# nihalsid/single-view-3d-reconstruction

Hardware: AMD Instinct MI355X
Metric: query-points/sec fwd+bwd (128^3 grid, 50k pts) (higher is better)
Workload: dtype f32

## Files before the change

### include/svr_hip.h

```cpp
#ifndef SVR_HIP_H
#define SVR_HIP_H

#include <stdint.h>

#ifdef __cplusplus
extern "C" {
#endif

#define SVR_OK 0
#define SVR_E_BADARG (-1)
#define SVR_E_BADSHAPE (-2)
#define SVR_E_ALIGN (-3)
#define SVR_E_UNSUPPORTED (-4)
#define SVR_E_IO (-5)
#define SVR_E_NOTFOUND (-6)

#define SVR_MAX_LEVELS 6

int svr_version(void);
const char *svr_last_error(void);

typedef struct svr_pull_plan {
  const uint32_t *keys;
  const void *recs;
// ... 22 lines not shown
  int32_t flags;
} svr_gather_desc;

#define SVR_GATHER_WIDE_OFFSETS 1
#define SVR_GATHER_DETERMINISTIC 2

int64_t svr_sizeof_level(void);
int64_t svr_sizeof_gather_desc(void);

int svr_points_voxel_order(const float *points, int32_t *order, int32_t B, int32_t N, int32_t D, int32_t H,
                           int32_t W, int32_t align_corners, void *workspace, void *stream);
int64_t svr_points_morton_order_workspace(int32_t B, int32_t N);
int svr_points_morton_order(const float *points, int32_t *order, float *sorted_points ,
                            int32_t B, int32_t N, void *workspace, void *stream);

int64_t svr_gather_pull_plan_workspace(int32_t B, int32_t N);
int64_t svr_gather_pull_plan_workspace_cells(int32_t B, int32_t D, int32_t H, int32_t W);
int svr_gather_pull_plan(const float *points, int32_t B, int32_t N, int32_t D, int32_t H, int32_t W, int32_t C,
                         int32_t col, int32_t row_stride, int32_t align_corners, float displacement,
                         uint32_t *keys, void *recs, int32_t *heads, int32_t *items , int32_t *stats ,
                         void *workspace, void *stream);

int svr_gather_item_order(const float *points, int32_t B, int32_t N, int32_t D, int32_t H, int32_t W,
                          int32_t align_corners, float displacement, int32_t with_j ,
                          int32_t *items, void *workspace, void *stream);
int svr_gather_item_order_xblock(const float *points, int32_t B, int32_t N, int32_t D, int32_t H, int32_t W,
                                 int32_t align_corners, float displacement, int32_t block, int32_t *items,
                                 void *workspace, void *stream);
int svr_gather_project_bwd(const float *points, const float *dh, int64_t lddh, int32_t B, int32_t N, int32_t D, int32_t H,
                           int32_t W, int32_t align_corners, float displacement, const int32_t *items, float *dP,
                           void *stream);

int64_t svr_gather_project_plan_workspace(int32_t B, int32_t N);
int64_t svr_gather_project_slots(int32_t B, int32_t N, int32_t D, int32_t H, int32_t W);
int svr_gather_project_plan(const float *points, int32_t B, int32_t N, int32_t D, int32_t H, int32_t W, int32_t align_corners,
                            float displacement, int32_t *items, uint32_t *keys, int32_t *sidx, int32_t *first_slot,
                            void *workspace, void *stream);
int svr_gather_project_bwd2(const float *points, const float *dh, int64_t lddh, int32_t B, int32_t N, int32_t D, int32_t H,
                            int32_t W, int32_t align_corners, float displacement, const int32_t *items, const int32_t *sidx,
                            const int32_t *first_slot, float *partials, float *dP, void *stream);

int svr_gather_trilinear_fwd(const svr_gather_desc *d, const float *points ,
                             float *features, void *stream);
int32_t svr_gather_fc0_supported(const svr_gather_desc *d);
int64_t svr_gather_fc0_workspace(const svr_gather_desc *d, int32_t n_out);
int svr_gather_fc0_fwd(const svr_gather_desc *d, const float *points, const float *W, int64_t ldw, const float *bias, float *Y,
                       int64_t ldy, int32_t n_out, float *features, int64_t ldf, const int32_t *keep_cols, uint32_t keep_levels,
                       int32_t epilogue, void *workspace, void *stream);
int svr_gather_fc0_prepare(const svr_gather_desc *d, const float *W, int64_t ldw, int32_t n_out, float *features, int64_t ldf,
                           const int32_t *keep_cols, uint32_t keep_levels, void *workspace, void *stream);
int svr_gather_fc0_run(const svr_gather_desc *d, const float *points, const float *bias, float *Y, int64_t ldy, int32_t n_out,
                       float *features, int64_t ldf, const int32_t *keep_cols, uint32_t keep_levels, int32_t epilogue,
                       void *workspace, void *stream);
int svr_gather_fc0_bf16_prepare(const svr_gather_desc *d, const float *W, int64_t ldw, int32_t n_out, void *workspace,
                                void *stream);
int svr_gather_fc0_bf16_run(const svr_gather_desc *d, const float *points, const float *bias, uint16_t *Y, int64_t ldy,
                            int32_t n_out, int32_t epilogue, void *workspace, void *stream);
int svr_gather_trilinear_bwd(const svr_gather_desc *d, const float *points, const float *gfeatures,
                             float *gpoints, void *stream);
int svr_gather_corner_indices(const svr_gather_desc *d, int32_t level, const float *points,
                              int32_t *out, void *stream);

int svr_cast_f32_to_bf16(const float *in, uint16_t *out, int64_t n, void *stream);
int svr_gather_trilinear_fwd_bf16(const svr_gather_desc *d, const float *points, uint16_t *features, void *stream);
int svr_linear_fwd_bf16(const uint16_t *X, int64_t ldx, const uint16_t *W, int64_t ldw, const float *bias, uint16_t *Y,
                        int64_t ldy, int64_t M, int64_t N, int64_t K, int epilogue, void *stream);
int svr_fc_out_fwd_bf16(const uint16_t *H, int64_t ldh, const float *w, const float *b, float *logits,
                        const int32_t *row_map, int64_t M, int64_t K, void *stream);

#define SVR_EPI_NONE 0
#define SVR_EPI_BIAS 1
#define SVR_EPI_BIAS_RELU 2
#define SVR_EPI_MASK 3

int svr_linear_fwd(const float *X, int64_t ldx, const float *W, int64_t ldw, const float *bias,
                   float *Y, int64_t ldy, int64_t M, int64_t N, int64_t K, int epilogue,
                   const float *mask, int64_t ldmask, void *stream);
int svr_linear_bwd_data(const float *dY, int64_t lddy, const float *W, int64_t ldw, float *dX,
                        int64_t lddx, int64_t M, int64_t N, int64_t K, int epilogue,
                        const float *mask, int64_t ldmask, void *stream);
int64_t svr_linear_bwd_weight_workspace(int64_t M, int64_t N, int64_t K);
int svr_linear_bwd_weight(const float *dY, int64_t lddy, const float *X, int64_t ldx, float *dW,
                          int64_t lddw, float *db, int64_t M, int64_t N, int64_t K,
                          void *workspace, void *stream);

int64_t svr_linear_fwd_bf16x6_workspace(int64_t N, int64_t K);
int svr_linear_fwd_bf16x6(const float *X, int64_t ldx, const float *W, int64_t ldw, const float *bias,
                          float *Y, int64_t ldy, int64_t M, int64_t N, int64_t K, int epilogue,
                          void *workspace, void *stream);
int64_t svr_linear_fwd_f16x3_workspace(int64_t N, int64_t K);
int svr_linear_fwd_f16x3(const float *X, int64_t ldx, const float *W, int64_t ldw, const float *bias,
                          float *Y, int64_t ldy, int64_t M, int64_t N, int64_t K, int epilogue,
                          void *workspace, void *stream);

int64_t svr_linear_bwd_data_bf16x3_workspace(int64_t N, int64_t K);
int svr_linear_bwd_data_bf16x3(const float *dY, int64_t lddy, const float *W, int64_t ldw, float *dX,
                               int64_t lddx, int64_t M, int64_t N, int64_t K, int epilogue,
                               const float *mask, int64_t ldmask, void *workspace, void *stream);
int64_t svr_linear_bwd_weight_bf16x3_workspace(int64_t M, int64_t N, int64_t K);
int svr_linear_bwd_weight_bf16x3(const float *dY, int64_t lddy, const float *X, int64_t ldx, float *dW,
                                 int64_t lddw, float *db, int64_t M, int64_t N, int64_t K,
                                 void *workspace, void *stream);

int svr_amax_f32(const float *X, int64_t ld, int64_t M, int64_t N, uint32_t *amax, void *stream);
int64_t svr_linear_bwd_data_f16x3_workspace(int64_t N, int64_t K);
int svr_linear_bwd_data_f16x3(const float *dY, int64_t lddy, const float *W, int64_t ldw, float *dX,
                              int64_t lddx, int64_t M, int64_t N, int64_t K, int epilogue,
                              const float *mask, int64_t ldmask, const uint32_t *amax_dy, uint32_t *amax_dx,
                              void *workspace, void *stream);
int64_t svr_linear_bwd_weight_f16x3_workspace(int64_t M, int64_t N, int64_t K);
int svr_linear_bwd_weight_f16x3(const float *dY, int64_t lddy, const float *X, int64_t ldx, float *dW,
                                int64_t lddw, float *db, int64_t M, int64_t N, int64_t K,
                                const uint32_t *amax_dy, void *workspace, void *stream);

#define SVR_LIN_FWD_F32 0
#define SVR_LIN_FWD_F16X3 1
#define SVR_LIN_FWD_BF16X6 2
#define SVR_LIN_BWD_DATA_F32 3
#define SVR_LIN_BWD_DATA_F16X3S 4
#define SVR_LIN_BWD_DATA_BF16X3 5
#define SVR_LIN_BWD_WEIGHT_F32 6
#define SVR_LIN_BWD_WEIGHT_F16X3S 7
#define SVR_LIN_BWD_WEIGHT_BF16X3 8
#define SVR_LIN_K_NT 0
#define SVR_LIN_K_NN 1
#define SVR_LIN_K_TN 2
#define SVR_LIN_K_NT128 3
#define SVR_LIN_K_NT64 4
#define SVR_LIN_K_NT128_BWD 5
#define SVR_LIN_K_NN_X3 6
#define SVR_LIN_K_TN_TR 7
#define SVR_LIN_K_TN_PREPASS 8
#define SVR_LIN_K_NT_X6 9
#define SVR_LIN_BIAS_NONE 0
#define SVR_LIN_BIAS_KERNEL 1
#define SVR_LIN_BIAS_COLSUM_VEC 2
#define SVR_LIN_BIAS_COLSUM_SLOW 3
int svr_linear_variant(int32_t op, int64_t M, int64_t N, int64_t K, int64_t ld_a, int64_t ld_b, int64_t ld_out,
                       int64_t ld_mask, int32_t lo_a, int32_t lo_b, int32_t lo_out, int32_t lo_mask, int32_t epilogue,
                       int32_t want_bias, int32_t *kernel, int32_t *coalesced, int32_t *splits, int64_t *rows_per_split,
                       int32_t *bias_form, int32_t *status);

int svr_fc_out_fwd(const float *H, int64_t ldh, const float *w, const float *b, float *logits,
                   const int32_t *row_map, int64_t M, int64_t K, void *stream);
int64_t svr_fc_out_bwd_workspace(int64_t M, int64_t K);
int svr_fc_out_bwd(const float *H, int64_t ldh, const float *w, const float *dlogits,
                   const int32_t *row_map, float *dH, int64_t lddh, float *dw, float *db, int64_t M,
                   int64_t K, uint32_t *amax_dh, void *workspace, void *stream);

int svr_bce_logits_sum_mean(const float *logits, const float *targets, float *loss, float *dlogits,
                            int64_t B, int64_t N, float gscale, void *workspace, void *stream);
int64_t svr_bce_ordered_workspace(int64_t B);
int svr_bce_logits_sum_mean_ordered(const float *logits, const float *targets, float *loss, float *dlogits,
                                    int64_t B, int64_t N, float gscale, void *workspace, void *stream);

int svr_conv3d_pack_weight(const float *W , float *Wp_fwd, float *Wp_bwd,
                           int32_t Ci, int32_t Co, void *stream);
int svr_conv3d_unpack_wgrad(const float *dWp , float *dW ,
                            int32_t Ci, int32_t Co, void *stream);
int svr_conv3d_k3(const float *in, const float *Wp, const float *bias, float *out, int32_t B,
                  int32_t D, int32_t H, int32_t W, int32_t Ci, int32_t Co, int epilogue,
                  const float *mask, void *stream);
int64_t svr_conv3d_c1_fwd_stats_workspace(int32_t B, int32_t D, int32_t H, int32_t W, int32_t Co);
int svr_conv3d_c1_fwd_stats(const float *in, const float *Wp, const float *bias, float *out, double *stats,
                            int32_t B, int32_t D, int32_t H, int32_t W, int32_t Co, int epilogue,
                            void *workspace, void *stream);
// ... 288 lines not shown
```

### single-view-3d-reconstruction_amd/_lib.py

```python
import ctypes as C
import os

import numpy as np
import torch

_HERE = os.path.dirname(os.path.abspath(__file__))
LIB_PATH = os.path.join(_HERE, "lib", "libsvr_hip.so")

SVR_MAX_LEVELS = 6
EPI_NONE, EPI_BIAS, EPI_BIAS_RELU, EPI_MASK = 0, 1, 2, 3

P = C.c_void_p
I32, I64, F32 = C.c_int32, C.c_int64, C.c_float


class Conv2dDesc(C.Structure):
    _fields_ = [("src0", P), ("src1", P), ("B", I32), ("H", I32), ("W", I32), ("C0", I32), ("C1", I32), ("k", I32),
                ("stride", I32), ("act", I32), ("upsample", I32)]


class PullPlan(C.Structure):
    _fields_ = [("keys", P), ("recs", P), ("heads", P), ("n_items", I64)]


class Level(C.Structure):
    _fields_ = [("vol", P), ("gvol", P), ("C", I32), ("D", I32), ("H", I32), ("W", I32), ("col", I32), ("order", P),
                ("item_order", P), ("plan", C.POINTER(PullPlan))]


class GatherDesc(C.Structure):
    _fields_ = [("n_levels", I32), ("B", I32), ("N", I32), ("row_stride", I32), ("align_corners", I32),
                ("displacement", F32), ("order", P), ("level", Level * SVR_MAX_LEVELS), ("flags", I32)]


GATHER_WIDE_OFFSETS, GATHER_DETERMINISTIC = 1, 2
EVAL_SUMS_WORKSPACE_BYTES = 6144


SIGNATURES = {
    "svr_version": (C.c_int, []),
    "svr_last_error": (C.c_char_p, []),
    "svr_sizeof_level": (I64, []),
    "svr_sizeof_gather_desc": (I64, []),
    "svr_points_morton_order_workspace": (I64, [I32, I32]),
    "svr_points_morton_order": (C.c_int, [P, P, P, I32, I32, P, P]),
    "svr_points_voxel_order": (C.c_int, [P, P, I32, I32, I32, I32, I32, I32, P, P]),
    "svr_gather_item_order": (C.c_int, [P, I32, I32, I32, I32, I32, I32, F32, I32, P, P, P]),
    "svr_gather_item_order_xblock": (C.c_int, [P, I32, I32, I32, I32, I32, I32, F32, I32, P, P, P]),
    "svr_gather_project_bwd": (C.c_int, [P, P, I64, I32, I32, I32, I32, I32, I32, F32, P, P, P]),
    "svr_gather_project_plan_workspace": (C.c_int64, [I32, I32]),
    "svr_gather_project_slots": (C.c_int64, [I32, I32, I32, I32, I32]),
    "svr_gather_project_plan": (C.c_int, [P, I32, I32, I32, I32, I32, I32, F32, P, P, P, P, P, P]),
    "svr_gather_project_bwd2": (C.c_int, [P, P, I64, I32, I32, I32, I32, I32, I32, F32, P, P, P, P, P, P]),
    "svr_gather_pull_plan_workspace": (I64, [I32, I32]),
    "svr_gather_pull_plan_workspace_cells": (I64, [I32, I32, I32, I32]),
    "svr_gather_pull_plan": (C.c_int, [P, I32, I32, I32, I32, I32, I32, I32, I32, I32, F32, P, P, P, P, P, P, P]),
    "svr_gather_trilinear_fwd": (C.c_int, [C.POINTER(GatherDesc), P, P, P]),
    "svr_gather_fc0_supported": (C.c_int32, [C.POINTER(GatherDesc)]),
    "svr_gather_fc0_workspace": (C.c_int64, [C.POINTER(GatherDesc), I32]),
    "svr_gather_fc0_fwd": (C.c_int, [C.POINTER(GatherDesc), P, P, I64, P, P, I64, I32, P, I64, P, C.c_uint32, I32, P, P]),
    "svr_gather_fc0_prepare": (C.c_int, [C.POINTER(GatherDesc), P, I64, I32, P, I64, P, C.c_uint32, P, P]),
    "svr_gather_fc0_run": (C.c_int, [C.POINTER(GatherDesc), P, P, P, I64, I32, P, I64, P, C.c_uint32, I32, P, P]),
    "svr_gather_fc0_bf16_prepare": (C.c_int, [C.POINTER(GatherDesc), P, I64, I32, P, P]),
    "svr_gather_fc0_bf16_run": (C.c_int, [C.POINTER(GatherDesc), P, P, P, I64, I32, I32, P, P]),
    "svr_gather_trilinear_bwd": (C.c_int, [C.POINTER(GatherDesc), P, P, P, P]),
    "svr_gather_corner_indices": (C.c_int, [C.POINTER(GatherDesc), I32, P, P, P]),
    "svr_cast_f32_to_bf16": (C.c_int, [P, P, I64, P]),
    "svr_gather_trilinear_fwd_bf16": (C.c_int, [C.POINTER(GatherDesc), P, P, P]),
    "svr_linear_fwd_bf16": (C.c_int, [P, I64, P, I64, P, P, I64, I64, I64, I64, C.c_int, P]),
    "svr_fc_out_fwd_bf16": (C.c_int, [P, I64, P, P, P, P, I64, I64, P]),
    "svr_linear_fwd": (C.c_int, [P, I64, P, I64, P, P, I64, I64, I64, I64, C.c_int, P, I64, P]),
    "svr_linear_bwd_data": (C.c_int, [P, I64, P, I64, P, I64, I64, I64, I64, C.c_int, P, I64, P]),
    "svr_linear_bwd_weight_workspace": (I64, [I64, I64, I64]),
    "svr_linear_bwd_weight": (C.c_int, [P, I64, P, I64, P, I64, P, I64, I64, I64, P, P]),
    "svr_linear_fwd_bf16x6_workspace": (I64, [I64, I64]),
    "svr_linear_fwd_bf16x6": (C.c_int, [P, I64, P, I64, P, P, I64, I64, I64, I64, C.c_int, P, P]),
    "svr_linear_fwd_f16x3_workspace": (I64, [I64, I64]),
    "svr_linear_fwd_f16x3": (C.c_int, [P, I64, P, I64, P, P, I64, I64, I64, I64, C.c_int, P, P]),
    "svr_linear_bwd_data_bf16x3_workspace": (I64, [I64, I64]),
    "svr_linear_bwd_data_bf16x3": (C.c_int, [P, I64, P, I64, P, I64, I64, I64, I64, C.c_int, P, I64, P, P]),
    "svr_linear_bwd_weight_bf16x3_workspace": (I64, [I64, I64, I64]),
    "svr_linear_bwd_weight_bf16x3": (C.c_int, [P, I64, P, I64, P, I64, P, I64, I64, I64, P, P]),
    "svr_amax_f32": (C.c_int, [P, I64, I64, I64, P, P]),
    "svr_linear_bwd_data_f16x3_workspace": (I64, [I64, I64]),
    "svr_linear_bwd_data_f16x3": (C.c_int, [P, I64, P, I64, P, I64, I64, I64, I64, C.c_int, P, I64, P, P, P, P]),
    "svr_linear_bwd_weight_f16x3_workspace": (I64, [I64, I64, I64]),
    "svr_linear_bwd_weight_f16x3": (C.c_int, [P, I64, P, I64, P, I64, P, I64, I64, I64, P, P, P]),
    "svr_linear_variant": (C.c_int, [I32, I64, I64, I64, I64, I64, I64, I64, I32, I32, I32, I32, I32, I32, P, P, P, P, P, P]),
    "svr_fc_out_fwd": (C.c_int, [P, I64, P, P, P, P, I64, I64, P]),
    "svr_fc_out_bwd_workspace": (I64, [I64, I64]),
    "svr_fc_out_bwd": (C.c_int, [P, I64, P, P, P, P, I64, P, P, I64, I64, P, P, P]),
    "svr_bce_logits_sum_mean": (C.c_int, [P, P, P, P, I64, I64, F32, P, P]),
    "svr_bce_ordered_workspace": (I64, [I64]),
    "svr_bce_logits_sum_mean_ordered": (C.c_int, [P, P, P, P, I64, I64, F32, P, P]),
    "svr_conv3d_pack_weight": (C.c_int, [P, P, P, I32, I32, P]),
    "svr_conv3d_unpack_wgrad": (C.c_int, [P, P, I32, I32, P]),
    "svr_conv3d_k3": (C.c_int, [P, P, P, P, I32, I32, I32, I32, I32, I32, C.c_int, P, P]),
    "svr_conv3d_fwd_bf16x6_workspace": (I64, [I32, I32]),
    "svr_conv3d_k3_fwd_bf16x6": (C.c_int, [P, P, P, P, I32, I32, I32, I32, I32, I32, C.c_int, P, P]),
    "svr_conv3d_fwd_f16x3_workspace": (I64, [I32, I32]),
    "svr_conv3d_k3_fwd_f16x3": (C.c_int, [P, P, P, P, I32, I32, I32, I32, I32, I32, C.c_int, P, P]),
    "svr_conv3d_fwd_f16x3_stats_blocks": (I32, [I32, I32, I32, I32, I32, I32]),
    "svr_conv3d_k3_fwd_f16x3_stats": (C.c_int, [P, P, P, P, P, I32, I32, I32, I32, I32, I32, C.c_int, P, P]),
    "svr_conv3d_bwd_data_bf16x3_workspace": (I64, [I32, I32]),
    "svr_conv3d_k3_bwd_data_bf16x3": (C.c_int, [P, P, P, I32, I32, I32, I32, I32, I32, C.c_int, P, P, P]),
    "svr_conv3d_c1_fwd_stats_workspace": (I64, [I32, I32, I32, I32, I32]),
    "svr_conv3d_c1_fwd_stats": (C.c_int, [P, P, P, P, P, I32, I32, I32, I32, I32, C.c_int, P, P]),
    "svr_conv3d_k3_bwd_weight_workspace": (I64, [I32, I32, I32, I32, I32, I32]),
    "svr_conv3d_k3_bwd_weight": (C.c_int, [P, P, P, P, I32, I32, I32, I32, I32, I32, P, P]),
    "svr_conv3d_k3_bwd_weight_bf16x3_workspace": (I64, [I32, I32, I32, I32, I32, I32]),
    "svr_conv3d_k3_bwd_weight_bf16x3": (C.c_int, [P, P, P, P, I32, I32, I32, I32, I32, I32, P, P]),
    "svr_conv3d_k3_bwd_weight_bf16x3_param": (C.c_int, [P, P, P, P, I32, I32, I32, I32, I32, I32, P, P]),
    "svr_conv3d_bwd_data_f16x3_workspace": (I64, [I32, I32]),
    "svr_conv3d_k3_bwd_data_f16x3": (C.c_int, [P, P, P, I32, I32, I32, I32, I32, I32, C.c_int, P, P, P, P, P]),
    "svr_conv3d_k3_bwd_weight_f16x3": (C.c_int, [P, P, P, P, I32, I32, I32, I32, I32, I32, I32, P, P, P]),
    "svr_conv3d_k3_variant": (C.c_int, [I32, I32, I32, I32, I32, I32, I32, P, P, P, P, P]),
    "svr_bn_stats_workspace": (I64, [I64, I32]),
    "svr_bn_stats": (C.c_int, [P, P, I64, I32, P, P]),
    "svr_bn_stats_finalize": (C.c_int, [P, P, P, P, P, P, P, P, P, I64, I32, F32, F32, P, P]),
    "svr_bn_finalize_parts": (C.c_int, [P, I32, P, P, P, P, P, P, P, P, I64, I32, F32, F32, P]),
    "svr_bn_finalize": (C.c_int, [P, P, P, P, P, P, P, I64, I32, F32, F32, C.c_int, P]),
    "svr_bn_apply_pool": (C.c_int, [P, P, P, P, P, P, P, P, I32, I32, I32, I32, I32, P]),
    "svr_bn_bwd_reduce": (C.c_int, [P, P, P, P, P, P, P, P, I32, I32, I32, I32, I32, P, P]),
    "svr_bn_bwd_apply": (C.c_int, [P, P, P, P, P, P, P, P, P, P, P, P, I32, I32, I32, I32, I32, C.c_int, P, P]),
    "svr_stage1_supported": (I32, [I32, I32, I32, I32, I32]),
    "svr_stage1_workspace": (I64, [I32, I32, I32, I32]),
    "svr_stage1_fwd": (C.c_int, [P, P, P, P, P, P, P, P, P, P, P, P, P, I32, I32, I32, I32, I32, F32, F32, C.c_int, C.c_int, P, P]),
    "svr_stage1_bwd": (C.c_int, [P, P, P, P, P, P, P, P, P, P, P, P, P, P, I32, I32, I32, I32, I32, C.c_int, C.c_int, P, P]),
    "svr_conv2d_im2col": (C.c_int, [C.POINTER(Conv2dDesc), P, P]),
    "svr_conv2d_col2im": (C.c_int, [C.POINTER(Conv2dDesc), P, P, P, P, P]),
    "svr_conv2d_small_supported": (C.c_int, [I32, I32, I32]),
    "svr_conv2d_small_fwd": (C.c_int, [C.POINTER(Conv2dDesc), P, P, P, I32, P]),
    "svr_conv2d_small_bwd_data": (C.c_int, [C.POINTER(Conv2dDesc), P, P, I32, P, P]),
    "svr_conv2d_small_bwd_weight_workspace": (I64, [C.POINTER(Conv2dDesc), I32]),
    "svr_conv2d_small_bwd_weight": (C.c_int, [C.POINTER(Conv2dDesc), P, I32, P, P, P, P]),
    "svr_conv2d_planes_bytes": (I64, [I32, I32, I32]),
    "svr_conv2d_prepare": (C.c_int, [P, I32, I32, I32, I32, I32, P, P, P]),
    "svr_conv2d_prepare_many": (C.c_int, [I32, P, P, P, P, P, P, P, P, P]),
    "svr_conv2d_workspace_bytes": (I64, [C.POINTER(Conv2dDesc), I32]),
    "svr_conv2d_virtual": (C.c_int, [C.POINTER(Conv2dDesc), P, P]),
# ... 145 lines not shown
```

### single-view-3d-reconstruction_amd/build.py

```python
import os
import subprocess
import sys

HERE = os.path.dirname(os.path.abspath(__file__))
CSRC = os.path.join(HERE, "csrc")
INCLUDE = os.path.join(os.path.dirname(HERE), "include")
LIBDIR = os.path.join(HERE, "lib")
LIB = os.path.join(LIBDIR, "libsvr_hip.so")

SOURCES = {
    "capi.cpp": [],
    "gather.hip": ["-ffp-contract=off"],
    "gather_fc0.hip": ["-ffp-contract=off"],
    "sort.hip": [],
    "gemm.hip": [],
    "gemm_bf16x3.hip": [],
    "gemm_bf16x6.hip": [],
    "gemm_f16x3.hip": [],
    "conv3d.hip": [],
    "conv3d_bf16.hip": [],
    "conv3d_bwdw_bf16.hip": [],
    "bn_pool.hip": [],
    "stage1.hip": [],
    "projection.hip": ["-ffp-contract=off"],
    "bf16_path.hip": ["-ffp-contract=off"],
    "mesh_occupancy.hip": ["-ffp-contract=off"],
    "marching_cubes.hip": ["-ffp-contract=off"],
    "sparse_lattice.hip": ["-ffp-contract=off"],
    "voxel_mesh.hip": ["-ffp-contract=off"],
    "mesh_eval.hip": ["-ffp-contract=off"],
    "mesh_df.hip": ["-ffp-contract=off"],
    "raycast.hip": ["-ffp-contract=off"],
    "vertex_color.hip": ["-ffp-contract=off"],
    "mesh_components.hip": ["-ffp-contract=off"],
    "sample_io.hip": [],
    "io_npz.cpp": [],
    "io_df.cpp": [],
    "io_exr.cpp": [],
    "io_mesh.cpp": [],
    "io_png.cpp": [],
    "raw_sample.hip": ["-ffp-contract=off"],
    "conv2d.hip": [],
    "conv2d_igemm.hip": [],
    "depth_head.hip": ["-ffp-contract=off"],
    "rgb_preprocess.hip": ["-ffp-contract=off"],
}
HOST = ("capi.cpp", "io_npz.cpp", "io_df.cpp", "io_exr.cpp", "io_mesh.cpp", "io_png.cpp")
HOST_COMMON = ["-O3", "-fPIC", "-std=c++17", "-ffp-contract=off", "-I" + INCLUDE, "-I" + CSRC]
COMMON = ["-O3", "-fPIC", "--offload-arch=gfx950", "-munsafe-fp-atomics", "-std=c++17", "-I" + INCLUDE, "-I" + CSRC,
          "-Rpass-analysis=kernel-resource-usage"]


def _hipcc():
    for c in (os.environ.get("HIPCC"), "/opt/rocm/bin/hipcc", "hipcc"):
        if c and (os.path.isabs(c) and os.path.exists(c) or not os.path.isabs(c)):
            return c
    return "hipcc"


def _stale(target, deps):
    if not os.path.exists(target):
        return True
    t = os.path.getmtime(target)
    return any(os.path.getmtime(d) > t for d in deps)


def build(force=False, verbose=False):
    os.makedirs(LIBDIR, exist_ok=True)
    objdir = os.path.join(HERE, "build")
    os.makedirs(objdir, exist_ok=True)
    headers = [os.path.join(CSRC, f) for f in os.listdir(CSRC) if f.endswith(".h")]
# ... 61 lines not shown
```

### single-view-3d-reconstruction_amd/csrc/f16x3.h

```cpp
#pragma once
#include <hip/hip_runtime.h>
#include <stdint.h>

namespace {

typedef _Float16 f16x8 __attribute__((ext_vector_type(8)));
typedef _Float16 f16x2 __attribute__((ext_vector_type(2)));
typedef __bf16 bf16x8 __attribute__((ext_vector_type(8)));
typedef __bf16 bf16x2 __attribute__((ext_vector_type(2)));
typedef float f32x2 __attribute__((ext_vector_type(2)));
typedef float f32x4 __attribute__((ext_vector_type(4)));
typedef float f32x16 __attribute__((ext_vector_type(16)));

__device__ __forceinline__ uint32_t pack_f16(float a, float b) {
  f32x2 v = {a, b};
  f16x2 h = __builtin_convertvector(v, f16x2);
  return __builtin_bit_cast(uint32_t, h);
}
__device__ __forceinline__ f32x2 unpack_f16(uint32_t p) {
  return __builtin_convertvector(__builtin_bit_cast(f16x2, p), f32x2);
}

__device__ __forceinline__ void split_x(float x0, float x1, uint32_t &hi, uint32_t &lo) {
  hi = pack_f16(x0, x1);
// ... 3 lines not shown

__device__ __forceinline__ void split_w(float w0, float w1, uint32_t &hi, uint32_t &lo) {
  hi = pack_f16(w0, w1);
  const f32x2 h = unpack_f16(hi);
  lo = pack_f16(w0 - h.x, w1 - h.y);
}
__device__ __forceinline__ void split_w(float w, _Float16 &hi, _Float16 &lo) {
  hi = (_Float16)w;
  lo = (_Float16)(w - (float)hi);
}

__device__ __forceinline__ f16x8 scale_2m11(f16x8 v) {
  return v * (_Float16)(1.f / 2048.f);
}

__device__ __forceinline__ float w_scale(uint32_t amax_bits, bool inverse) {
  const float amax = __uint_as_float(amax_bits);
  int e = 0;
  if (amax > 0.f && amax < 3.0e38f) {
    frexpf(amax, &e);
    e = 14 - e;
    e = e > 100 ? 100 : (e < -100 ? -100 : e);
  }
  return ldexpf(1.f, inverse ? -e : e);
}

__device__ __forceinline__ float bf_lo(uint32_t p) { return __uint_as_float(p << 16); }
__device__ __forceinline__ float bf_hi(uint32_t p) { return __uint_as_float(p & 0xffff0000u); }
__device__ __forceinline__ uint32_t pack_bf16(float a, float b) {
  f32x2 v = {a, b};
  return __builtin_bit_cast(uint32_t, __builtin_convertvector(v, bf16x2));
}

__device__ __forceinline__ void split2(float x0, float x1, uint32_t &hi, uint32_t &mid) {
  hi = pack_bf16(x0, x1);
  mid = pack_bf16(x0 - bf_lo(hi), x1 - bf_hi(hi));
}
__device__ __forceinline__ void split3(float x0, float x1, uint32_t &hi, uint32_t &mid, uint32_t &lo) {
  split2(x0, x1, hi, mid);
  lo = pack_bf16((x0 - bf_lo(hi)) - bf_lo(mid), (x1 - bf_hi(hi)) - bf_hi(mid));
}

template <int SL = 2>
__device__ __forceinline__ int slot_dw(int row, int sub) {
  static_assert(SL == 2 || SL == 4, "16- or 32-value rows");
  const int g = SL == 2 ? (row >> 3) & 1 : (row >> 2) & 3;
  return (row * SL + (sub ^ g)) * 4;
}
__device__ __forceinline__ f16x8 frag_f16(const uint32_t *p) {
  union { uint4 q; f16x8 v; } f;
  f.q = *reinterpret_cast<const uint4 *>(p);
  return f.v;
}
__device__ __forceinline__ bf16x8 frag_bf16(const uint32_t *p) {
  union { uint4 q; bf16x8 v; } f;
  f.q = *reinterpret_cast<const uint4 *>(p);
  return f.v;
}

}
```

### single-view-3d-reconstruction_amd/csrc/gather_fc0.hip

```cpp
#include "common.h"
#include "gather_common.h"
#include "f16x3.h"
#include <algorithm>

using namespace svr;

namespace {

#define GLOBAL_AS __attribute__((address_space(1)))
typedef uint32_t u32x2_t __attribute__((ext_vector_type(2)));

constexpr int FK = 16;
constexpr int FLW = 8;
constexpr int FTM = 64;
constexpr int NPW = 4;
constexpr int NPT = NPW * 64;
constexpr int NTHR = 256 + NPT;
constexpr int RPW = FTM / NPW;
constexpr int FMT = FTM / 32;
constexpr int FTN = 256;
constexpr int FPLANE = FTM * FLW;
constexpr int FKSTEP = 2 * FPLANE + 8;
constexpr int FSLAB_K = 4;
constexpr int FSLAB = FSLAB_K * FKSTEP;
constexpr int FC_MAX_SLABS = 56;
constexpr int FC_STAGE_VOX = 160;
constexpr int FC_STAGE_DW = FC_STAGE_VOX * 64;
constexpr int FC_NSTAGE = 2;
struct FcBox { int nvox, b, z0, y0, x0, by, bx, pad; };
constexpr int FC_LDS_BYTES = 2 * FSLAB * 4 + FC_STAGE_DW * 4;
static_assert(FTM == 64 && NPW == 4 && 2 * FC_LDS_BYTES <= 160 * 1024, "two workgroups per CU");

struct FcLevel {
  const float *vol;
  int C, D, H, W, col;
  int kcol;
};
struct FcSlab {
  int level, j0, nj, lp;
  int k0, nk;
  int c0, keep;
  int stage, geo;
};
struct FcArgs {
  FcLevel L[SVR_MAX_LEVELS];
  FcSlab S[FC_MAX_SLABS];
  int n_slabs, KF;
  int n_stage, stage_level[FC_NSTAGE];
};

__device__ __forceinline__ int fused_col(const FcArgs &A, int kk) {
  for (int s = 0; s < A.n_slabs; ++s) {
    const FcSlab S = A.S[s];
    const int r = kk - S.k0 * FK;
    if (r < 0 || r >= S.nk * FK) continue;
    const FcLevel L = A.L[S.level];
    if (S.lp == 0) return r < 7 ? L.col + r : -1;
    const int nc = S.lp * 4 / S.nj;
    return L.col + (S.j0 + r / nc) * L.C + S.c0 + r % nc;
  }
  return -1;
}

__device__ __forceinline__ int64_t wfrag_index(int kk, int plane, int n, int ntiles, int nplanes = 2) {
  return ((((int64_t)(kk >> 4) * nplanes + plane) * ntiles + (n >> 5)) * 64 + ((kk >> 3) & 1) * 32 + (n & 31)) * 8 + (kk & 7);
}

__global__ void split_w_fused_kernel(FcArgs A, const float *__restrict__ W, int64_t ldw, const uint32_t *__restrict__ amax,
                                     uint16_t *__restrict__ p0, int N) {
  const int kk = blockIdx.x * blockDim.x + threadIdx.x, n = blockIdx.y;
  if (kk >= A.KF || n >= N) return;
  const int src = fused_col(A, kk);
  const float w = src >= 0 ? W[(int64_t)n * ldw + src] * w_scale(amax[0], false) : 0.f;
  _Float16 h, l;
  split_w(w, h, l);
  p0[wfrag_index(kk, 0, n, N / 32)] = __builtin_bit_cast(uint16_t, h);
  p0[wfrag_index(kk, 1, n, N / 32)] = __builtin_bit_cast(uint16_t, l);
}

__global__ void split_w_fused_bf16_kernel(FcArgs A, const float *__restrict__ W, int64_t ldw, uint16_t *__restrict__ p0, int N) {
  const int kk = blockIdx.x * blockDim.x + threadIdx.x, n = blockIdx.y;
  if (kk >= A.KF || n >= N) return;
  const int src = fused_col(A, kk);
  const float w = src >= 0 ? W[(int64_t)n * ldw + src] : 0.f;
  p0[wfrag_index(kk, 0, n, N / 32, 1)] = (uint16_t)(pack_bf16(w, 0.f) & 0xffffu);
}


#define LDS_AS __attribute__((address_space(3)))
constexpr int GEO_N = 14;
constexpr int GEO_IPS = 64 / RPW;
constexpr int GEO_SETS = (7 + GEO_IPS - 1) / GEO_IPS;
struct Geo { int v[GEO_SETS][GEO_N]; };

template <bool BF, bool STAGED>
__device__ __forceinline__ void level_geometry(const FcLevel L, const float *__restrict__ pt0, int rowb, float disp, int ac, int lane,
                                               const FcBox box, Geo &G) {
  constexpr uint32_t EB = BF ? 2u : 4u;
  const int C = L.C;
#pragma unroll
  for (int r = 0; r < GEO_SETS; ++r) {
    const int item = r * 64 + lane, j = min(item / RPW, 6);
    const int row = rowb & 255, b = rowb >> 8;
    const GLOBAL_AS float *pg = (const GLOBAL_AS float *)pt0;
    const uint32_t po = (uint32_t)row * 3u;
    const float pt[3] = {pg[po], pg[po + 1u], pg[po + 2u]};
    const Corner c = sample_corner(pt, j, disp, L.D, L.H, L.W, ac);
    const Weights w = corner_weights(c);
    int xc[2], yc[2], zc[2];
    bool vx[2], vy[2], vz[2];
#pragma unroll
    for (int a = 0; a < 2; ++a) {
      vx[a] = w.x0 + a >= 0 && w.x0 + a < L.W;
      vy[a] = w.y0 + a >= 0 && w.y0 + a < L.H;
      vz[a] = w.z0 + a >= 0 && w.z0 + a < L.D;
      xc[a] = min(max(w.x0 + a, 0), L.W - 1);
      yc[a] = min(max(w.y0 + a, 0), L.H - 1);
      zc[a] = min(max(w.z0 + a, 0), L.D - 1);
    }
#pragma unroll
    for (int k = 0; k < 8; ++k) {
      const float wt = (w.wx[k & 1] * w.wy[(k >> 1) & 1]) * w.wz[k >> 2];
      G.v[r][6 + k] = __float_as_int((vx[k & 1] && vy[(k >> 1) & 1] && vz[k >> 2]) ? wt : 0.f);
    }
    if constexpr (STAGED) {
      (void)b;
#pragma unroll
      for (int i = 0; i < 4; ++i) G.v[r][i] = (((zc[i >> 1] - box.z0) * box.by + (yc[i & 1] - box.y0)) * box.bx) * 256;
#pragma unroll
      for (int a = 0; a < 2; ++a) G.v[r][4 + a] = (xc[a] - box.x0) * 256;
    } else {
#pragma unroll
      for (int i = 0; i < 4; ++i) G.v[r][i] = (int)((uint32_t)(((b * L.D + zc[i >> 1]) * L.H + yc[i & 1]) * L.W * C) * EB);
#pragma unroll
      for (int a = 0; a < 2; ++a) G.v[r][4 + a] = xc[a] * C * (int)EB;
    }
  }
}

template <int LP, int NJ, bool BF, bool STAGED = false>
__device__ __forceinline__ void produce_slab(const FcLevel L, const FcSlab S, uint32_t *__restrict__ buf, int64_t m0, int64_t M,
                                             float *__restrict__ feat, int row_stride, int pw, int lane, const Geo &G,
                                             const uint32_t *stage = nullptr) {
  constexpr int PPW = 64 / LP, NP = RPW / PPW, LPI = LP / NJ, NC = LPI * 4;
  const int C = L.C;
  const GLOBAL_AS char *vol = (const GLOBAL_AS char *)L.vol;
  constexpr uint32_t EB = BF ? 2u : 4u;
  int ge[GEO_N];
#pragma unroll
  for (int k = 0; k < GEO_N; ++k) ge[k] = G.v[0][k];
#pragma unroll
  for (int r = 1; r < GEO_SETS; ++r)
    if (S.j0 / GEO_IPS == r) {
#pragma unroll
      for (int k = 0; k < GEO_N; ++k) ge[k] = G.v[r][k];
    }
  const unsigned ul = (unsigned)lane & 63u;
  const int g = (int)(ul / (unsigned)LP), q = (int)(ul % (unsigned)LP), jj = (int)((unsigned)q / (unsigned)LPI), c4 = (int)((unsigned)q % (unsigned)LPI) * 4;
  const int src0 = (((S.j0 + jj) % GEO_IPS) * RPW + g) << 2;
  const uint32_t xoff = STAGED ? (uint32_t)c4 * 4u : (uint32_t)(S.c0 + c4) * EB;
  const int col = jj * NC + c4;
  static_assert(RPW % 16 == 0 && (PPW == 4 || PPW == 8 || PPW == 16), "swizzle bit of the producer rows");
  static_assert(FKSTEP % 8 == 0 && FLW == 8, "slot bit of the producer's destination");
  const int dsto = ((col >> 4) * FKSTEP + (RPW * pw + g) * FLW + ((col & 15) >> 1)) ^ (PPW == 16 ? ((g >> 3) & 1) * 4 : 0);
  GLOBAL_AS char *featt = (GLOBAL_AS char *)(feat + m0 * row_stride);
  const uint32_t fo0 = (uint32_t)((RPW * pw + g) * row_stride + L.kcol + (S.j0 + jj) * C + S.c0 + c4) * 4u;
  const int live = M - m0 < FTM ? (int)(M - m0) : FTM;
  struct Iter {
    f32x4 v[8];
  };
  auto fetch = [&](Iter &I, int it) {
    const int src = src0 + it * (PPW * 4);
    uint32_t zy[4], x[2];
#pragma unroll
    for (int i = 0; i < 4; ++i) zy[i] = (uint32_t)__builtin_amdgcn_ds_bpermute(src, ge[i]);
#pragma unroll
    for (int a = 0; a < 2; ++a) x[a] = (uint32_t)__builtin_amdgcn_ds_bpermute(src, ge[4 + a]) + xoff;
    if constexpr (BF) {
      u32x2_t raw[8];
#pragma unroll
      for (int k = 0; k < 8; ++k) raw[k] = *reinterpret_cast<const GLOBAL_AS u32x2_t *>(vol + (zy[k >> 1] + x[k & 1]));
#pragma unroll
      for (int k = 0; k < 8; ++k)
        I.v[k] = f32x4{__uint_as_float(raw[k].x << 16), __uint_as_float(raw[k].x & 0xffff0000u), __uint_as_float(raw[k].y << 16),
                       __uint_as_float(raw[k].y & 0xffff0000u)};
    } else if constexpr (STAGED) {
      const LDS_AS char *sb = (const LDS_AS char *)stage;
#pragma unroll
      for (int k = 0; k < 8; ++k) I.v[k] = *reinterpret_cast<const LDS_AS f32x4 *>(sb + (zy[k >> 1] + x[k & 1]));
    } else {
#pragma unroll
      for (int k = 0; k < 8; ++k) I.v[k] = *reinterpret_cast<const GLOBAL_AS f32x4 *>(vol + (zy[k >> 1] + x[k & 1]));
    }
  };
  auto finish = [&](const Iter &I, int it) {
    float w[8];
    const int src = src0 + it * (PPW * 4);
#pragma unroll
    for (int k = 0; k < 8; ++k) w[k] = __int_as_float(__builtin_amdgcn_ds_bpermute(src, ge[6 + k]));
    f32x4 acc = f32x4{0.f, 0.f, 0.f, 0.f};
#pragma unroll
    for (int k = 0; k < 8; ++k) acc = acc + I.v[k] * w[k];
    uint32_t *d = buf + (dsto ^ (PPW == 16 ? 0 : (((it * PPW) >> 3) & 1) * 4)) + it * (PPW * FLW);
    if constexpr (BF) {
      *reinterpret_cast<uint2 *>(d) = make_uint2(pack_bf16(acc.x, acc.y), pack_bf16(acc.z, acc.w));
      return;
    }
    uint32_t h0, l0, h1, l1;
    split_x(acc.x, acc.y, h0, l0);
    split_x(acc.z, acc.w, h1, l1);
    *reinterpret_cast<uint2 *>(d) = make_uint2(h0, h1);
    *reinterpret_cast<uint2 *>(d + FPLANE) = make_uint2(l0, l1);
    if (S.keep && RPW * pw + it * PPW + g < live) {
      __builtin_nontemporal_store(acc, reinterpret_cast<GLOBAL_AS f32x4 *>(featt + (fo0 + (uint32_t)(it * PPW * row_stride * 4))));
    }
  };
  constexpr int DEPTH = 1;
  Iter I[DEPTH];
#pragma unroll
  for (int it = 0; it < DEPTH; ++it) fetch(I[it], it);
#pragma unroll
  for (int it = 0; it < NP; ++it) {
    finish(I[it % DEPTH], it);
    if (it + DEPTH < NP) fetch(I[it % DEPTH], it + DEPTH);
  }
}

template <bool BF>
__device__ __forceinline__ void produce_c1(const FcLevel L, const FcSlab S, uint32_t *__restrict__ buf,
                                           const float *__restrict__ points, int64_t m0, int64_t M, int N, float disp, int ac,
                                           float *__restrict__ feat, int row_stride, int tp) {
  const GLOBAL_AS float *vol = (const GLOBAL_AS float *)L.vol;
  const GLOBAL_AS uint16_t *vol16 = (const GLOBAL_AS uint16_t *)L.vol;
  constexpr int C1R = FTM * 8 / NPT;
  static_assert(C1R >= 1 && FTM * 8 % NPT == 0, "C == 1 level: whole rounds of producer threads");
  float u[C1R][8], wk[C1R][8];
#pragma unroll
  for (int r = 0; r < C1R; ++r) {
    const int item = r * NPT + tp, row = item >> 3, j = item & 7;
    const int64_t pn = min(m0 + row, M - 1);
    const uint32_t vb = (uint32_t)(pn / N) * (uint32_t)(L.D * L.H * L.W);
    const Corner c = sample_corner(points + pn * 3, j < 7 ? j : 0, disp, L.D, L.H, L.W, ac);
    const Weights w = corner_weights(c);
#pragma unroll
    for (int k = 0; k < 8; ++k) {
      const int z = w.z0 + (k >> 2), y = w.y0 + ((k >> 1) & 1), x = w.x0 + (k & 1);
      const bool valid = z >= 0 && z < L.D && y >= 0 && y < L.H && x >= 0 && x < L.W && j < 7;
      const int zc = min(max(z, 0), L.D - 1), yc = min(max(y, 0), L.H - 1), xc = min(max(x, 0), L.W - 1);
      wk[r][k] = valid ? (w.wx[k & 1] * w.wy[(k >> 1) & 1]) * w.wz[k >> 2] : 0.f;
      const uint32_t vo = vb + (uint32_t)((zc * L.H + yc) * L.W + xc);
      u[r][k] = BF ? __uint_as_float((uint32_t)vol16[vo] << 16) : vol[vo];
    }
  }
  uint16_t *b16 = reinterpret_cast<uint16_t *>(buf);
#pragma unroll
  for (int r = 0; r < C1R; ++r) {
    const int item = r * NPT + tp, row = item >> 3, j = item & 7;
    float acc = 0.f;
#pragma unroll
    for (int k = 0; k < 8; ++k) acc = acc + u[r][k] * wk[r][k];
    if (j == 7) acc = 0.f;
    const _Float16 h = (_Float16)acc;
    const _Float16 l = (_Float16)((acc - (float)h) * 2048.f);
    const uint16_t hb = BF ? (uint16_t)(pack_bf16(acc, 0.f) & 0xffffu) : __builtin_bit_cast(uint16_t, h);
    const int s0 = slot_dw(row, 0), s1 = slot_dw(row, 1);
    if (j < 7) {
      b16[s0 * 2 + j] = hb;
      if (!BF) b16[(FPLANE + s0) * 2 + j] = __builtin_bit_cast(uint16_t, l);
      if (!BF && S.keep && m0 + row < M) feat[(m0 + row) * row_stride + L.kcol + j] = acc;
    } else {
      uint32_t z = 0u;
      asm volatile("" : "+v"(z));
      b16[s0 * 2 + 7] = (uint16_t)z;
      if (!BF) b16[(FPLANE + s0) * 2 + 7] = (uint16_t)z;
#pragma unroll
      for (int p = 0; p < 4; ++p) {
        buf[s1 + p] = z;
        if (!BF) buf[FPLANE + s1 + p] = z;
      }
    }
  }
}

__device__ __forceinline__ void stage_box(const FcLevel L, int c0, const FcBox box, uint32_t *__restrict__ stage, int tp) {
  if (box.nvox == 0) return;
  const GLOBAL_AS char *vol = (const GLOBAL_AS char *)L.vol;
  constexpr int R = FC_STAGE_VOX * 16 / NPT;
  static_assert(FC_STAGE_VOX * 16 % NPT == 0, "staging rounds");
  const int n16 = box.nvox * 16, byx = box.by * box.bx;
  const float ibyx = 1.f / (float)byx, ibx = 1.f / (float)box.bx;
  f32x4 reg[R];
#pragma unroll
  for (int i = 0; i < R; ++i) {
    const int idx = min(tp + NPT * i, n16 - 1), v = idx >> 4, q = idx & 15;
    const int vz = (int)(((float)v + 0.5f) * ibyx), r = v - vz * byx;
    const int vy = (int)(((float)r + 0.5f) * ibx), vx = r - vy * box.bx;
    const uint32_t off = (uint32_t)((((box.b * L.D + box.z0 + vz) * L.H + box.y0 + vy) * L.W + box.x0 + vx) * L.C + c0 + q * 4) * 4u;
    reg[i] = *reinterpret_cast<const GLOBAL_AS f32x4 *>(vol + off);
  }
#pragma unroll
  for (int i = 0; i < R; ++i) {
    const int idx = tp + NPT * i;
    if (idx < n16) *reinterpret_cast<f32x4 *>(stage + idx * 4) = reg[i];
  }
}

template <bool BF>
__device__ __forceinline__ void produce(const FcArgs &A, int s, uint32_t *buf, const float *points, int64_t m0, int64_t M,
                                        int N, float disp, int ac, float *feat, int row_stride, int pw, int lane,
                                        uint32_t *stage, const FcBox *__restrict__ boxes, Geo &G, int rowb) {
  const FcSlab S = A.S[s];
  const FcLevel L = A.L[S.level];
  if constexpr (!BF) {
    if (S.stage >= 0) {
      const FcBox box = boxes[S.stage];
      if (S.lp < 0) {
        stage_box(L, S.c0, box, stage, pw * 64 + lane);
        return;
      }
      if (box.nvox > 0) {
        if (S.geo) level_geometry<BF, true>(L, points + m0 * 3, rowb, disp, ac, lane, box, G);
        produce_slab<16, 1, BF, true>(L, S, buf, m0, M, feat, row_stride, pw, lane, G, stage);
        return;
      }
    }
  }
  if (S.lp == 0) {
    produce_c1<BF>(L, S, buf, points, m0, M, N, disp, ac, feat, row_stride, pw * 64 + lane);
    return;
  }
  if (S.geo) level_geometry<BF, false>(L, points + m0 * 3, rowb, disp, ac, lane, FcBox{}, G);
  switch (S.lp * 4 + S.nj) {
    case 16 * 4 + 1: produce_slab<16, 1, BF>(L, S, buf, m0, M, feat, row_stride, pw, lane, G); break;
    case 16 * 4 + 2: produce_slab<16, 2, BF>(L, S, buf, m0, M, feat, row_stride, pw, lane, G); break;
    case 8 * 4 + 1: produce_slab<8, 1, BF>(L, S, buf, m0, M, feat, row_stride, pw, lane, G); break;
    case 8 * 4 + 2: produce_slab<8, 2, BF>(L, S, buf, m0, M, feat, row_stride, pw, lane, G); break;
    case 4 * 4 + 1: produce_slab<4, 1, BF>(L, S, buf, m0, M, feat, row_stride, pw, lane, G); break;
  }
}

__device__ __forceinline__ void slab_barrier() {
  asm volatile("s_waitcnt lgkmcnt(0)\n\ts_barrier" ::: "memory");
}

__global__ void args_store_kernel(FcArgs A, FcArgs *__restrict__ dst) {
  const uint32_t *src = reinterpret_cast<const uint32_t *>(&A);
  for (unsigned i = threadIdx.x; i < sizeof(FcArgs) / 4; i += blockDim.x) reinterpret_cast<uint32_t *>(dst)[i] = src[i];
}

template <bool BF>
__global__ __launch_bounds__(NTHR, 4) void gather_fc0_kernel(const FcArgs *__restrict__ Ap, const float *__restrict__ points,
                                                            const uint16_t *__restrict__ W0,
                                                            const uint32_t *__restrict__ amax, const float *__restrict__ bias,
                                                            float *__restrict__ Y, int64_t ldy, float *__restrict__ feat,
                                                            int row_stride, int pad_start, int64_t M, int N, float disp, int ac,
                                                            int relu, const FcBox *__restrict__ boxes) {
  extern __shared__ __attribute__((aligned(16))) uint32_t lds[];
  const FcArgs &A = *Ap;
  const int t = threadIdx.x, lane = t & 63, wave = t >> 6;
  const int64_t tile = blockIdx.x;
  const int64_t m0 = tile * FTM;
  if (m0 >= M) return;
  const int S = A.n_slabs;
  if (wave >= 4) {
    const int pw = __builtin_amdgcn_readfirstlane(wave) - 4;
    if (pad_start >= 0 && t - 256 < FTM && m0 + (t - 256) < M)
      for (int cc = pad_start; cc < row_stride; ++cc) feat[(m0 + (t - 256)) * row_stride + cc] = 0.f;
    Geo G;
    const int last = (int)min<int64_t>(M - 1 - m0, FTM - 1);
    const int b0 = (int)(m0 / N), rem0 = (int)(m0 - (int64_t)b0 * N);
    static_assert(FTM <= 256, "row in the low byte of rowb");
    const int row = min(RPW * pw + lane % RPW, last);
    int rowb = row | ((b0 + (int)((uint32_t)(rem0 + row) / (uint32_t)N)) << 8);
    asm volatile("" : "+v"(rowb));
    for (int s = -1; s < S; ++s) {
      int lane_s = lane;
      int rowb_s = rowb;
      asm volatile("" : "+v"(lane_s), "+v"(rowb_s));
      if (s + 1 < S)
        produce<BF>(A, s + 1, lds + ((s + 1) & 1) * FSLAB, points, m0, M, N, disp, ac, feat, row_stride, pw, lane_s, lds + 2 * FSLAB,
                    boxes + tile * FC_NSTAGE, G, rowb_s);
      slab_barrier();
    }
    return;
  }
  const int wc = wave, l31 = lane & 31, lh = lane >> 5;
  const int KF = A.KF, nk = KF / FK;
  const uint16_t *wp = W0 + ((2 * wc) * 64 + lane) * 8;
  uint4 b0[2][2], b1[2][2];
  constexpr int NPL = BF ? 1 : 2;
  auto loadb = [&](uint4 (&r)[2][2], int kidx) {
    const uint16_t *q = wp + (kidx < nk ? kidx : nk - 1) * (NPL * (FTN / 32) * 512);
#pragma unroll
    for (int jt = 0; jt < 2; ++jt) {
      r[jt][0] = *reinterpret_cast<const uint4 *>(q + jt * 512);
      if constexpr (!BF) r[jt][1] = *reinterpret_cast<const uint4 *>(q + (FTN / 32) * 512 + jt * 512);
    }
  };
  f32x16 acc[FMT][2];
#pragma unroll
  for (int i = 0; i < FMT; ++i)
#pragma unroll
    for (int j = 0; j < 2; ++j)
#pragma unroll
      for (int r = 0; r < 16; ++r) acc[i][j][r] = 0.f;
  loadb(b0, 0);
  slab_barrier();
  int s = 0, kin = 0, ksl = A.S[0].nk, kidx = 0;
  auto skip_empty = [&]() {
    while (s < S && ksl == 0) {
      slab_barrier();
      ++s;
      ksl = s < S ? A.S[s].nk : 0;
    }
  };
  skip_empty();
  int mma_on = 1;
  asm volatile("" : "+s"(mma_on));
  auto step = [&](const uint4 (&cur)[2][2], uint4 (&fre)[2][2]) {
    if (mma_on) {
      loadb(fre, kidx + 1);
      const uint32_t *pa = lds + (s & 1) * FSLAB + kin * FKSTEP;
      if constexpr (BF) {
#pragma unroll
        for (int i = 0; i < FMT; ++i) {
          union { f16x8 h; bf16x8 b; } ua;
          ua.h = frag_f16(pa + slot_dw(i * 32 + l31, lh));
#pragma unroll
          for (int jt = 0; jt < 2; ++jt) {
            union { uint4 q; bf16x8 b; } ub;
            ub.q = cur[jt][0];
            acc[i][jt] = __builtin_amdgcn_mfma_f32_32x32x16_bf16(ua.b, ub.b, acc[i][jt], 0, 0, 0);
          }
// ... 160 lines not shown
int check_desc(const svr_gather_desc *d, const char *who) {
  SVR_CHECK(d && d->n_levels >= 1 && d->n_levels <= SVR_MAX_LEVELS && d->B > 0 && d->N >= 0, SVR_E_BADARG, "%s: bad descriptor", who);
  SVR_CHECK(d->order == nullptr, SVR_E_UNSUPPORTED, "%s: a processing order is not supported (sort the points instead)", who);
  int n_c1 = 0;
  for (int l = 0; l < d->n_levels; ++l) {
    const svr_level &lv = d->level[l];
    SVR_CHECK(lv.vol && lv.D > 0 && lv.H > 0 && lv.W > 0, SVR_E_BADARG, "%s: level %d: bad volume", who, l);
    SVR_CHECK((int64_t)d->B * lv.D * lv.H * lv.W * lv.C < (1LL << 30), SVR_E_UNSUPPORTED, "%s: level %d has >= 2^30 elements", who, l);
    SVR_CHECK(((uintptr_t)lv.vol & 15) == 0 || lv.C == 1, SVR_E_ALIGN, "%s: level %d: volume must be 16-byte aligned", who, l);
    SVR_CHECK(lv.C == 1 || lv.col % 4 == 0, SVR_E_ALIGN, "%s: level %d: column %d", who, l, lv.col);
    n_c1 += lv.C == 1;
  }
  SVR_CHECK(n_c1 <= 1, SVR_E_UNSUPPORTED, "%s: more than one single-channel level", who);
  return SVR_OK;
}

}

extern "C" int32_t svr_gather_fc0_supported(const svr_gather_desc *d) {
  if (!d || d->n_levels < 1 || d->n_levels > SVR_MAX_LEVELS || d->order) return 0;
  FcArgs A;
  if (!build_slabs(d, 0, A)) return 0;
  for (int l = 0; l < d->n_levels; ++l)
    if ((int64_t)d->B * d->level[l].D * d->level[l].H * d->level[l].W * d->level[l].C >= (1LL << 30)) return 0;
  return 1;
}

extern "C" int64_t svr_gather_fc0_workspace(const svr_gather_desc *d, int32_t n_out) {
  FcArgs A;
  if (!d || !build_slabs(d, 0, A)) return 0;
  const int64_t tiles = cdiv((int64_t)d->B * d->N, FTM);
  return 2 * (int64_t)n_out * A.KF * (int64_t)sizeof(uint16_t) + 1024 + (int64_t)sizeof(FcArgs) + 256 +
         tiles * FC_NSTAGE * (int64_t)sizeof(FcBox);
}

namespace {

struct FcWorkspace {
  uint32_t *amax;
  uint16_t *p0;
  FcArgs *Ad;
  FcBox *boxes;
};
FcWorkspace carve(void *workspace, int32_t n_out, int KF) {
  FcWorkspace w;
  w.amax = align256<uint32_t>(workspace);
  w.p0 = (uint16_t *)(w.amax + 64);
  uint16_t *p1 = w.p0 + (int64_t)n_out * KF;
  w.Ad = align256<FcArgs>(p1 + (int64_t)n_out * KF);
  w.boxes = align256<FcBox>(w.Ad + 1);
  return w;
}

int check_keep(const svr_gather_desc *d, const FcArgs &A, const float *feat, int64_t ldf, uint32_t keep_levels, int64_t *kend) {
  const int64_t M = (int64_t)d->B * d->N;
  SVR_CHECK(keep_levels == 0 || (feat && ldf % 4 == 0 && ((uintptr_t)feat & 15) == 0 && M * ldf < (1LL << 31)),
            SVR_E_BADARG, "gather_fc0: keep_levels needs a 16-byte aligned feature matrix with < 2^31 elements");
  *kend = 0;
  for (int l = 0; l < d->n_levels; ++l) {
    if (!((keep_levels >> l) & 1)) continue;
    const int kc = A.L[l].kcol, w = 7 * d->level[l].C;
    SVR_CHECK(kc >= 0 && kc + w <= ldf && (d->level[l].C == 1 || kc % 4 == 0), SVR_E_BADSHAPE,
              "gather_fc0: kept level %d: columns [%d,%d) in a row of %ld", l, kc, kc + w, (long)ldf);
    for (int m = 0; m < l; ++m)
      if ((keep_levels >> m) & 1)
        SVR_CHECK(kc + w <= A.L[m].kcol || A.L[m].kcol + 7 * d->level[m].C <= kc, SVR_E_BADSHAPE,
                  "gather_fc0: kept levels %d and %d overlap", m, l);
    *kend = std::max<int64_t>(*kend, kc + w);
  }
  return SVR_OK;
}

}

extern "C" int svr_gather_fc0_prepare(const svr_gather_desc *d, const float *W, int64_t ldw, int32_t n_out, float *feat,
                                      int64_t ldf, const int32_t *keep_cols, uint32_t keep_levels, void *workspace,
                                      void *stream) {
  int rc = check_desc(d, "gather_fc0_prepare");
  if (rc != SVR_OK) return rc;
  if ((int64_t)d->B * d->N == 0) return SVR_OK;
  SVR_CHECK(W && workspace, SVR_E_BADARG, "gather_fc0_prepare: null pointer");
  SVR_CHECK(n_out == FTN, SVR_E_UNSUPPORTED, "gather_fc0_prepare: %d output columns (the kernel is built for %d)", n_out, FTN);
  if (ldf <= 0) ldf = d->row_stride;
  FcArgs A;
  SVR_CHECK(build_slabs(d, keep_levels, A, keep_cols, true), SVR_E_UNSUPPORTED,
            "gather_fc0_prepare: a level's channel count has no slab shape (1, 16, 32, 64 k)");
  int64_t kend;
  if ((rc = check_keep(d, A, feat, ldf, keep_levels, &kend)) != SVR_OK) return rc;
  hipStream_t s = (hipStream_t)stream;
  const FcWorkspace ws = carve(workspace, n_out, A.KF);
  int64_t kw = 0;
  for (int l = 0; l < d->n_levels; ++l) kw = std::max<int64_t>(kw, d->level[l].col + 7 * d->level[l].C);
  w_amax_launch(W, ldw, n_out, kw, ws.amax, s);
  hipLaunchKernelGGL(split_w_fused_kernel, dim3((unsigned)cdiv(A.KF, 64), (unsigned)n_out), dim3(64), 0, s, A, W, ldw, ws.amax,
                     ws.p0, (int)n_out);
  hipLaunchKernelGGL(args_store_kernel, dim3(1), dim3(256), 0, s, A, ws.Ad);
  return launch_status("gather_fc0_prepare");
}

extern "C" int svr_gather_fc0_run(const svr_gather_desc *d, const float *points, const float *bias, float *Y, int64_t ldy,
                                  int32_t n_out, float *feat, int64_t ldf, const int32_t *keep_cols, uint32_t keep_levels,
                                  int32_t epilogue, void *workspace, void *stream) {
  int rc = check_desc(d, "gather_fc0_run");
  if (rc != SVR_OK) return rc;
  const int64_t M = (int64_t)d->B * d->N;
  if (M == 0) return SVR_OK;
  SVR_CHECK(points && Y && workspace, SVR_E_BADARG, "gather_fc0_run: null pointer");
  SVR_CHECK(n_out == FTN, SVR_E_UNSUPPORTED, "gather_fc0_run: %d output columns (the kernel is built for %d)", n_out, FTN);
  SVR_CHECK(epilogue == SVR_EPI_NONE || ((epilogue == SVR_EPI_BIAS || epilogue == SVR_EPI_BIAS_RELU) && bias), SVR_E_BADARG,
            "gather_fc0_run: epilogue %d", epilogue);
  if (ldf <= 0) ldf = d->row_stride;
  FcArgs A;
  SVR_CHECK(build_slabs(d, keep_levels, A, keep_cols, true), SVR_E_UNSUPPORTED,
            "gather_fc0_run: a level's channel count has no slab shape (1, 16, 32, 64 k)");
  int64_t kend;
  if ((rc = check_keep(d, A, feat, ldf, keep_levels, &kend)) != SVR_OK) return rc;
  int64_t kw = 0;
  for (int l = 0; l < d->n_levels; ++l) kw = std::max<int64_t>(kw, d->level[l].col + 7 * d->level[l].C);
  const int64_t pad_start = keep_cols ? kend : kw;
  const FcWorkspace ws = carve(workspace, n_out, A.KF);
  static const hipError_t lds_attr =
      hipFuncSetAttribute((const void *)gather_fc0_kernel<false>, hipFuncAttributeMaxDynamicSharedMemorySize, FC_LDS_BYTES);
  SVR_CHECK(lds_attr == hipSuccess, (int)lds_attr, "gather_fc0_run: cannot reserve %d bytes of LDS: %s", FC_LDS_BYTES,
            hipGetErrorString(lds_attr));
  const float *eb = epilogue == SVR_EPI_NONE ? nullptr : bias;
  const int relu = epilogue == SVR_EPI_BIAS_RELU ? 1 : 0;
  if (A.n_stage > 0)
    hipLaunchKernelGGL(fc0_boxes_kernel, dim3((unsigned)cdiv(M, FTM)), dim3(64), 0, (hipStream_t)stream, ws.Ad, points, M, d->N,
                       d->displacement, d->align_corners, ws.boxes);
  hipLaunchKernelGGL(gather_fc0_kernel<false>, dim3((unsigned)cdiv(M, FTM)), dim3(NTHR), FC_LDS_BYTES, (hipStream_t)stream, ws.Ad, points,
                     ws.p0, ws.amax, eb, Y, ldy, feat, (int)ldf, keep_levels ? (int)pad_start : -1, M, d->N, d->displacement,
                     d->align_corners, relu, ws.boxes);
  return launch_status("gather_fc0_run");
}

extern "C" int svr_gather_fc0_fwd(const svr_gather_desc *d, const float *points, const float *W, int64_t ldw, const float *bias,
                                  float *Y, int64_t ldy, int32_t n_out, float *feat, int64_t ldf, const int32_t *keep_cols,
                                  uint32_t keep_levels, int32_t epilogue, void *workspace, void *stream) {
  int rc = svr_gather_fc0_prepare(d, W, ldw, n_out, feat, ldf, keep_cols, keep_levels, workspace, stream);
  if (rc != SVR_OK) return rc;
  return svr_gather_fc0_run(d, points, bias, Y, ldy, n_out, feat, ldf, keep_cols, keep_levels, epilogue, workspace, stream);
}

extern "C" int svr_gather_fc0_bf16_prepare(const svr_gather_desc *d, const float *W, int64_t ldw, int32_t n_out, void *workspace,
                                           void *stream) {
  int rc = check_desc(d, "gather_fc0_bf16_prepare");
  if (rc != SVR_OK) return rc;
  if ((int64_t)d->B * d->N == 0) return SVR_OK;
  SVR_CHECK(W && workspace, SVR_E_BADARG, "gather_fc0_bf16_prepare: null pointer");
  SVR_CHECK(n_out == FTN, SVR_E_UNSUPPORTED, "gather_fc0_bf16_prepare: %d output columns (the kernel is built for %d)", n_out, FTN);
  FcArgs A;
  SVR_CHECK(build_slabs(d, 0, A), SVR_E_UNSUPPORTED, "gather_fc0_bf16_prepare: a level's channel count has no slab shape (1, 16, 32, 64 k)");
  for (int l = 0; l < d->n_levels; ++l)
    SVR_CHECK(((uintptr_t)d->level[l].vol & 7) == 0 || d->level[l].C == 1, SVR_E_ALIGN, "gather_fc0_bf16_prepare: level %d: 8-byte alignment", l);
  hipStream_t s = (hipStream_t)stream;
  const FcWorkspace ws = carve(workspace, n_out, A.KF);
  hipLaunchKernelGGL(split_w_fused_bf16_kernel, dim3((unsigned)cdiv(A.KF, 64), (unsigned)n_out), dim3(64), 0, s, A, W, ldw, ws.p0, (int)n_out);
  hipLaunchKernelGGL(args_store_kernel, dim3(1), dim3(256), 0, s, A, ws.Ad);
  return launch_status("gather_fc0_bf16_prepare");
}

extern "C" int svr_gather_fc0_bf16_run(const svr_gather_desc *d, const float *points, const float *bias, uint16_t *Y, int64_t ldy,
                                       int32_t n_out, int32_t epilogue, void *workspace, void *stream) {
  int rc = check_desc(d, "gather_fc0_bf16_run");
  if (rc != SVR_OK) return rc;
  const int64_t M = (int64_t)d->B * d->N;
  if (M == 0) return SVR_OK;
  SVR_CHECK(points && Y && workspace, SVR_E_BADARG, "gather_fc0_bf16_run: null pointer");
  SVR_CHECK(n_out == FTN, SVR_E_UNSUPPORTED, "gather_fc0_bf16_run: %d output columns (the kernel is built for %d)", n_out, FTN);
  SVR_CHECK(epilogue == SVR_EPI_NONE || ((epilogue == SVR_EPI_BIAS || epilogue == SVR_EPI_BIAS_RELU) && bias), SVR_E_BADARG,
            "gather_fc0_bf16_run: epilogue %d", epilogue);
  FcArgs A;
  SVR_CHECK(build_slabs(d, 0, A), SVR_E_UNSUPPORTED, "gather_fc0_bf16_run: a level's channel count has no slab shape (1, 16, 32, 64 k)");
  const FcWorkspace ws = carve(workspace, n_out, A.KF);
  static const hipError_t lds_attr =
      hipFuncSetAttribute((const void *)gather_fc0_kernel<true>, hipFuncAttributeMaxDynamicSharedMemorySize, FC_LDS_BYTES);
  SVR_CHECK(lds_attr == hipSuccess, (int)lds_attr, "gather_fc0_bf16_run: cannot reserve %d bytes of LDS: %s", FC_LDS_BYTES,
            hipGetErrorString(lds_attr));
  const float *eb = epilogue == SVR_EPI_NONE ? nullptr : bias;
  const int relu = epilogue == SVR_EPI_BIAS_RELU ? 1 : 0;
  hipLaunchKernelGGL(gather_fc0_kernel<true>, dim3((unsigned)cdiv(M, FTM)), dim3(NTHR), FC_LDS_BYTES, (hipStream_t)stream, ws.Ad, points,
                     ws.p0, ws.amax, eb, reinterpret_cast<float *>(Y), ldy, (float *)nullptr, 0, -1, M, d->N, d->displacement,
                     d->align_corners, relu, (const FcBox *)nullptr);
  return launch_status("gather_fc0_bf16_run");
}
```

### single-view-3d-reconstruction_amd/csrc/gemm_bf16x3.hip

```cpp
#include "common.h"
#define SVR_GEMM_PLAN_ONLY
#include "gemm_core.h"
#include "conv2d_virt.h"
#include "f16x3.h"

using namespace svr;

namespace {

constexpr int XK = 32;
constexpr int XLD = 40;
constexpr int XLW = XLD / 2;

template <int ROWS, int NT, bool F16 = false>
struct RowKLoader {
  static constexpr int R = ROWS * 8 / NT;
  const float *rowp[R];
  float4 v[R];
  float sy = 1.f;
  __device__ __forceinline__ RowKLoader(const float *src, int64_t ld, int64_t row0, int64_t nrows) {
    const int t = threadIdx.x;
#pragma unroll
    for (int i = 0; i < R; ++i) {
      int64_t r = row0 + (t >> 3) + (NT / 8) * i;
      r = r < nrows ? r : nrows - 1;
      rowp[i] = src + r * ld + (t & 7) * 4;
    }
  }
  __device__ __forceinline__ void load(int64_t k0, int64_t) {
#pragma unroll
    for (int i = 0; i < R; ++i) v[i] = *reinterpret_cast<const float4 *>(rowp[i] + k0);
  }
  __device__ __forceinline__ void store(uint32_t *planes) const {
    const int t = threadIdx.x;
#pragma unroll
    for (int i = 0; i < R; ++i) {
      uint32_t h0, m0, h1, m1;
      if constexpr (F16) {
        split_x(v[i].x * sy, v[i].y * sy, h0, m0);
        split_x(v[i].z * sy, v[i].w * sy, h1, m1);
      } else {
        split2(v[i].x, v[i].y, h0, m0);
        split2(v[i].z, v[i].w, h1, m1);
      }
      const int off = ((t >> 3) + (NT / 8) * i) * XLW + (t & 7) * 2;
      *reinterpret_cast<uint2 *>(planes + off) = make_uint2(h0, h1);
      *reinterpret_cast<uint2 *>(planes + ROWS * XLW + off) = make_uint2(m0, m1);
    }
  }
};

template <int ROWS, int NT>
struct PlaneLoader {
  static constexpr int R = ROWS * 4 / NT;
  const uint16_t *ph[R], *pm[R];
  uint2 vh[R][2], vm[R][2];
  __device__ __forceinline__ PlaneLoader(const uint16_t *hi, const uint16_t *mid, int64_t ld, int64_t row0, int64_t nrows) {
    const int t = threadIdx.x;
#pragma unroll
    for (int i = 0; i < R; ++i) {
      int64_t r = row0 + (t >> 2) + (NT / 4) * i;
      r = r < nrows ? r : nrows - 1;
      ph[i] = hi + r * ld + (t & 3) * 8;
      pm[i] = mid + r * ld + (t & 3) * 8;
    }
  }
  __device__ __forceinline__ void load(int64_t k0, int64_t) {
#pragma unroll
    for (int i = 0; i < R; ++i) {
      const uint2 *qh = reinterpret_cast<const uint2 *>(ph[i] + k0);
      const uint2 *qm = reinterpret_cast<const uint2 *>(pm[i] + k0);
      vh[i][0] = qh[0]; vh[i][1] = qh[1];
      vm[i][0] = qm[0]; vm[i][1] = qm[1];
    }
  }
  __device__ __forceinline__ void store(uint32_t *planes) const {
    const int t = threadIdx.x;
#pragma unroll
    for (int i = 0; i < R; ++i) {
      const int off = ((t >> 2) + (NT / 4) * i) * XLW + (t & 3) * 4;
      *reinterpret_cast<uint2 *>(planes + off) = vh[i][0];
      *reinterpret_cast<uint2 *>(planes + off + 2) = vh[i][1];
      *reinterpret_cast<uint2 *>(planes + ROWS * XLW + off) = vm[i][0];
      *reinterpret_cast<uint2 *>(planes + ROWS * XLW + off + 2) = vm[i][1];
    }
  }
};

template <int ROWS, int NT>
struct TransLoader {
  static constexpr int KG = NT / ROWS;
  static constexpr int P = 16 / KG;
  const float *colp;
  int64_t ld;
  int kfirst;
  float v[2 * P];
  __device__ __forceinline__ TransLoader(const float *src, int64_t ld_, int64_t col0, int64_t ncols) : ld(ld_) {
    const int t = threadIdx.x;
    int64_t c = col0 + (t % ROWS);
    c = c < ncols ? c : ncols - 1;
    kfirst = 2 * (t / ROWS) * P;
    colp = src + (int64_t)kfirst * ld + c;
  }
  __device__ __forceinline__ void load(int64_t k0, int64_t kend) {
    const float *q = colp + k0 * ld;
    if (k0 + XK <= kend) {
#pragma unroll
      for (int p = 0; p < 2 * P; ++p) v[p] = q[p * ld];
    } else {
#pragma unroll
      for (int p = 0; p < 2 * P; ++p) v[p] = (k0 + kfirst + p < kend) ? q[p * ld] : 0.f;
    }
  }
  __device__ __forceinline__ void store(uint32_t *planes) const {
    const int t = threadIdx.x;
    uint32_t h[P], m[P];
#pragma unroll
    for (int p = 0; p < P; ++p) split2(v[2 * p], v[2 * p + 1], h[p], m[p]);
    const int off = (t % ROWS) * XLW + (t / ROWS) * P;
#pragma unroll
    for (int p = 0; p < P; p += 4) {
      *reinterpret_cast<uint4 *>(planes + off + p) = make_uint4(h[p], h[p + 1], h[p + 2], h[p + 3]);
      *reinterpret_cast<uint4 *>(planes + ROWS * XLW + off + p) = make_uint4(m[p], m[p + 1], m[p + 2], m[p + 3]);
    }
  }
};

__device__ __forceinline__ bf16x8 read_frag(const uint32_t *plane, int row, int kword) {
  union { uint4 q; bf16x8 v; } f;
  f.q = *reinterpret_cast<const uint4 *>(plane + row * XLW + kword);
  return f.v;
}

template <int WR, int WC>
struct Geo {
  static constexpr int NT = WR * WC * 64, TM = WR * 64, TN = WC * 64;
  static constexpr int STAGE = 2 * (TM + TN) * XLW;
  static constexpr int LDS_DWORDS = STAGE;
};

template <int WR, int WC, bool F16 = false>
__device__ __forceinline__ void compute_step(const uint32_t *pa, f32x16 (&acc)[2][2]) {
  using G = Geo<WR, WC>;
  const int lane = threadIdx.x & 63, wave = threadIdx.x >> 6;
  const int wr = wave / WC, wc = wave % WC;
  const int l31 = lane & 31, lh = lane >> 5;
  const uint32_t *pb = pa + 2 * G::TM * XLW;
#pragma unroll
  for (int ks = 0; ks < 2; ++ks) {
    bf16x8 ah[2], am[2], bh[2], bm[2];
    const int kw = ks * 8 + lh * 4;
#pragma unroll
    for (int i = 0; i < 2; ++i) {
      const int row = wr * 64 + i * 32 + l31;
      ah[i] = read_frag(pa, row, kw);
      am[i] = read_frag(pa + G::TM * XLW, row, kw);
    }
#pragma unroll
    for (int j = 0; j < 2; ++j) {
      const int row = wc * 64 + j * 32 + l31;
      bh[j] = read_frag(pb, row, kw);
      bm[j] = read_frag(pb + G::TN * XLW, row, kw);
    }
    if constexpr (F16) {
      f16x8 fah[2], fal[2], fbh[2], fbl[2], fbq[2];
#pragma unroll
      for (int i = 0; i < 2; ++i) {
        fah[i] = __builtin_bit_cast(f16x8, ah[i]);
        fal[i] = __builtin_bit_cast(f16x8, am[i]);
        fbh[i] = __builtin_bit_cast(f16x8, bh[i]);
        fbl[i] = __builtin_bit_cast(f16x8, bm[i]);
        fbq[i] = scale_2m11(fbh[i]);
      }
#pragma unroll
      for (int i = 0; i < 2; ++i)
#pragma unroll
        for (int j = 0; j < 2; ++j) {
          acc[i][j] = __builtin_amdgcn_mfma_f32_32x32x16_f16(fal[i], fbq[j], acc[i][j], 0, 0, 0);
          acc[i][j] = __builtin_amdgcn_mfma_f32_32x32x16_f16(fah[i], fbl[j], acc[i][j], 0, 0, 0);
          acc[i][j] = __builtin_amdgcn_mfma_f32_32x32x16_f16(fah[i], fbh[j], acc[i][j], 0, 0, 0);
        }
    } else {
#pragma unroll
    for (int i = 0; i < 2; ++i)
#pragma unroll
      for (int j = 0; j < 2; ++j) {
        acc[i][j] = __builtin_amdgcn_mfma_f32_32x32x16_bf16(am[i], bh[j], acc[i][j], 0, 0, 0);
        acc[i][j] = __builtin_amdgcn_mfma_f32_32x32x16_bf16(ah[i], bm[j], acc[i][j], 0, 0, 0);
        acc[i][j] = __builtin_amdgcn_mfma_f32_32x32x16_bf16(ah[i], bh[j], acc[i][j], 0, 0, 0);
      }
    }
  }
}

template <int WR, int WC, class AL, class BL, bool F16 = false>
__device__ __forceinline__ void mainloop(AL &al, BL &bl, uint32_t *lds, int64_t kbeg, int64_t kend, f32x16 (&acc)[2][2]) {
  using G = Geo<WR, WC>;
#pragma unroll
  for (int i = 0; i < 2; ++i)
#pragma unroll
    for (int j = 0; j < 2; ++j)
#pragma unroll
      for (int r = 0; r < 16; ++r) acc[i][j][r] = 0.f;
  if (kbeg >= kend) return;
  al.load(kbeg, kend);
  bl.load(kbeg, kend);
  al.store(lds);
  bl.store(lds + 2 * G::TM * XLW);
  __syncthreads();
  for (int64_t k0 = kbeg; k0 < kend; k0 += XK) {
    const bool more = k0 + XK < kend;
    if (more) {
      al.load(k0 + XK, kend);
      bl.load(k0 + XK, kend);
    }
    __builtin_amdgcn_sched_barrier(0);
    compute_step<WR, WC, F16>(lds, acc);
    __syncthreads();
    if (more) {
      al.store(lds);
      bl.store(lds + 2 * G::TM * XLW);
    }
    __syncthreads();
  }
}

template <int WR, int WC, class F>
__device__ __forceinline__ void foreach_acc(f32x16 (&acc)[2][2], F f) {
  const int lane = threadIdx.x & 63, wave = threadIdx.x >> 6;
  const int wr = wave / WC, wc = wave % WC;
#pragma unroll
  for (int i = 0; i < 2; ++i)
#pragma unroll
    for (int j = 0; j < 2; ++j) {
      const int col = wc * 64 + j * 32 + (lane & 31);
#pragma unroll
      for (int r = 0; r < 16; ++r) f(wr * 64 + i * 32 + (r & 3) + 8 * (r >> 2) + 4 * (lane >> 5), col, acc[i][j][r]);
    }
}

__global__ void pack_planes_kernel(const float *__restrict__ W, int64_t ldw, uint16_t *__restrict__ hi,
                                   uint16_t *__restrict__ mid, int64_t N, int64_t K) {
  int64_t idx = (int64_t)blockIdx.x * blockDim.x + threadIdx.x;
  if (idx >= K * (N / 2)) return;
  int64_t k = idx / (N / 2), n = (idx % (N / 2)) * 2;
  uint32_t h, m;
  split2(W[n * ldw + k], W[(n + 1) * ldw + k], h, m);
  *reinterpret_cast<uint32_t *>(hi + k * N + n) = h;
  *reinterpret_cast<uint32_t *>(mid + k * N + n) = m;
}

constexpr int NN_TM = 128, NN_TN = 128, NN_CLD = NN_TN + 4;
template <bool F16>
__global__ __launch_bounds__(256, 3) void linear_nn_x3_kernel(const float *__restrict__ dY, int64_t lddy,
                                                           const uint16_t *__restrict__ Wh,
                                                           const uint16_t *__restrict__ Wm, float *__restrict__ dX,
                                                           int64_t lddx, const float *__restrict__ mask, int64_t ldmask,
                                                           int64_t M, int64_t N, int64_t K, const uint32_t *__restrict__ amax_w,
                                                           const uint32_t *__restrict__ amax_dy, uint32_t *__restrict__ amax_dx) {
  using G = Geo<2, 2>;
  static_assert(G::LDS_DWORDS >= (NN_TM / 2) * NN_CLD, "half the epilogue tile must fit the staging buffer");
  __shared__ __attribute__((aligned(16))) uint32_t lds[G::LDS_DWORDS];
  const int64_t nct = cdiv(K, NN_TN), lidx = xcd_logical(blockIdx.x, gridDim.x);
  if (lidx >= nct * cdiv(M, NN_TM)) return;
  const int64_t c0 = (lidx % nct) * NN_TN, m0 = (lidx / nct) * NN_TM;
  RowKLoader<NN_TM, 256, F16> al(dY, lddy, m0, M);
  PlaneLoader<NN_TN, 256> bl(Wh, Wm, N, c0, K);
  float inv = 1.f, vmax = 0.f;
  if constexpr (F16) {
    al.sy = amax_dy ? w_scale(amax_dy[0], false) : 1.f;
    inv = w_scale(amax_w[0], true) * (amax_dy ? w_scale(amax_dy[0], true) : 1.f);
  }
  f32x16 acc[2][2];
  mainloop<2, 2, RowKLoader<NN_TM, 256, F16>, PlaneLoader<NN_TN, 256>, F16>(al, bl, lds, 0, N, acc);
  float *ct = reinterpret_cast<float *>(lds);
  const int t = threadIdx.x;
  const int wave = t >> 6;
#pragma unroll
  for (int pass = 0; pass < 2; ++pass) {
    float4 k4[8];
    if (mask) {
#pragma unroll
      for (int i = 0; i < 8; ++i) {
        const int64_t m = m0 + 64 * pass + (t >> 5) + 8 * i, c = c0 + (t & 31) * 4;
        k4[i] = *reinterpret_cast<const float4 *>(mask + (m < M ? m : M - 1) * ldmask + (c < K ? c : K - 4));
      }
    }
    if ((wave >> 1) == pass)
      foreach_acc<2, 2>(acc, [&](int row, int col, float v) { ct[(row - 64 * pass) * NN_CLD + col] = v; });
    __syncthreads();
#pragma unroll
    for (int i = 0; i < 8; ++i) {
      const int row = (t >> 5) + 8 * i, c4 = (t & 31) * 4;
      const int64_t m = m0 + 64 * pass + row, c = c0 + c4;
      if (m < M && c < K) {
        float4 v = *reinterpret_cast<const float4 *>(ct + row * NN_CLD + c4);
        if constexpr (F16) { v.x *= inv; v.y *= inv; v.z *= inv; v.w *= inv; }
        if (mask) {
          v.x = k4[i].x > 0.f ? v.x : 0.f;
          v.y = k4[i].y > 0.f ? v.y : 0.f;
          v.z = k4[i].z > 0.f ? v.z : 0.f;
          v.w = k4[i].w > 0.f ? v.w : 0.f;
        }
        if constexpr (F16) vmax = fmaxf(fmaxf(vmax, fmaxf(fabsf(v.x), fabsf(v.y))), fmaxf(fabsf(v.z), fabsf(v.w)));
        if constexpr (F16) {
          typedef float nt4 __attribute__((ext_vector_type(4)));
          __builtin_nontemporal_store(nt4{v.x, v.y, v.z, v.w}, reinterpret_cast<nt4 *>(dX + m * lddx + c));
        } else {
          *reinterpret_cast<float4 *>(dX + m * lddx + c) = v;
        }
      }
    }
    __syncthreads();
  }
  if constexpr (F16) {
    if (amax_dx) svr_amax_publish(amax_dx, vmax);
  }
}

__global__ void pack_planes_f16_kernel(const float *__restrict__ W, int64_t ldw, const uint32_t *__restrict__ amax,
                                       uint16_t *__restrict__ hi, uint16_t *__restrict__ lo, int64_t N, int64_t K) {
  int64_t idx = (int64_t)blockIdx.x * blockDim.x + threadIdx.x;
  if (idx >= K * (N / 2)) return;
  const int64_t k = idx / (N / 2), n = (idx % (N / 2)) * 2;
  const float sc = w_scale(amax[0], false);
  const float w0 = W[n * ldw + k] * sc, w1 = W[(n + 1) * ldw + k] * sc;
  uint32_t h, l;
  split_w(w0, w1, h, l);
  *reinterpret_cast<uint32_t *>(hi + k * N + n) = h;
  *reinterpret_cast<uint32_t *>(lo + k * N + n) = l;
}

constexpr int TN_TM = 128, TN_TN = 128;
__global__ __launch_bounds__(256) void linear_tn_x3_kernel(const uint16_t *__restrict__ dYh,
                                                           const uint16_t *__restrict__ dYm, int64_t Mpad,
                                                           const float *__restrict__ X, int64_t ldx,
                                                           float *__restrict__ slab, int64_t M, int64_t N, int64_t K,
                                                           int64_t rows_per_split, int splits) {
  using G = Geo<2, 2>;
  __shared__ __attribute__((aligned(16))) uint32_t lds[G::LDS_DWORDS];
  const int64_t tk = cdiv(K, TN_TN), tiles = tk * cdiv(N, TN_TM), lidx = xcd_logical(blockIdx.x, gridDim.x);
  if (lidx >= tiles * splits) return;
  const int64_t split = lidx / tiles, tile = lidx % tiles;
  const int64_t tn = cdiv(N, TN_TM);
  const int64_t i0 = (tile % tn) * TN_TM, j0 = (tile / tn) * TN_TN;
  const int64_t kbeg = split * rows_per_split;
  const int64_t kend = min(M, kbeg + rows_per_split);
  PlaneLoader<TN_TM, 256> al(dYh, dYm, Mpad, i0, N);
  TransLoader<TN_TN, 256> bl(X, ldx, j0, K);
  f32x16 acc[2][2];
  mainloop<2, 2>(al, bl, lds, kbeg, kend, acc);
  float *out = slab + split * N * K;
  foreach_acc<2, 2>(acc, [&](int row, int col, float v) {
    int64_t i = i0 + row, j = j0 + col;
    if (i < N && j < K) out[i * K + j] = v;
  });
}

typedef __bf16 bf16x4 __attribute__((ext_vector_type(4)));
constexpr int TR_XPLANE = 32 * 64;

__device__ __forceinline__ int tr_off(int r, int ch) { return 256 * r + 16 * (ch ^ (((r & 3) << 2) | ((r >> 2) & 3))); }

__device__ __forceinline__ bf16x8 tr_frag(const uint32_t *plane, int byte0, int byte1) {
  typedef __attribute__((address_space(3))) bf16x4 lds_bf16x4;
  const char *b = reinterpret_cast<const char *>(plane);
  const bf16x4 lo = __builtin_amdgcn_ds_read_tr16_b64_v4bf16((lds_bf16x4 *)(b + byte0));
  const bf16x4 hi = __builtin_amdgcn_ds_read_tr16_b64_v4bf16((lds_bf16x4 *)(b + byte1));
  return __builtin_shufflevector(lo, hi, 0, 1, 2, 3, 4, 5, 6, 7);
}

struct CwGeom {
  CvSrc S;
  int Wo, HoWo;
  float rWo, rHoWo;
  int k, stride, pad, Cpad;
};
template <bool F16 = false, bool CONV = false, bool VEC4 = true>
__global__ __launch_bounds__(256, 2) void linear_tn_x3_tr_kernel(const float *__restrict__ dY, int64_t lddy,
                                                              const float *__restrict__ X, int64_t ldx,
                                                              float *__restrict__ slab, float *__restrict__ dbpart,
                                                              int64_t M, int64_t N, int64_t K, int64_t rows_per_split,
                                                              int splits, const uint32_t *__restrict__ amax_dy, const CwGeom G) {
  __shared__ __attribute__((aligned(16))) uint32_t lds[4 * TR_XPLANE];
  uint32_t *la = lds, *lx = lds + 2 * TR_XPLANE;
  const int t = threadIdx.x, lane = t & 63, wave = t >> 6;
  const int wr = wave >> 1, wc = wave & 1, lh = lane >> 5;
  const int64_t tk = cdiv(K, TN_TN), tiles = tk * cdiv(N, TN_TM), lidx = xcd_logical(blockIdx.x, gridDim.x);
  if (lidx >= tiles * splits) return;
  const int64_t split = lidx / tiles, tile = lidx % tiles;
  const int64_t tn = cdiv(N, TN_TM);
  const int64_t i0 = (tile % tn) * TN_TM, j0 = (tile / tn) * TN_TN;
  const int64_t kbeg = split * rows_per_split;
  const int64_t kend = min(M, kbeg + rows_per_split);
  float4 av[4], xv[4];
  const int64_t acol = CONV ? i0 + 4 * (int64_t)(t & 31) : min(i0 + 4 * (int64_t)(t & 31), N - 4), xcol = min(j0 + 4 * (int64_t)(t & 31), K - 4);
  int ctap_y = 0, ctap_x = 0, cch = 0;
  if constexpr (CONV) {
    const int tap = (int)(xcol / G.Cpad);
    cch = (int)(xcol % G.Cpad);
    ctap_y = tap / G.k - G.pad;
    ctap_x = tap % G.k - G.pad;
  }
  auto gload = [&](int64_t k0) {
#pragma unroll
    for (int i = 0; i < 4; ++i) {
      const int64_t m = min(k0 + (t >> 5) + 8 * i, kend - 1);
      if constexpr (CONV) {
        if (VEC4 && (N & 3) == 0 && acol + 4 <= N) {
          av[i] = *reinterpret_cast<const float4 *>(dY + m * lddy + acol);
        } else {
          float e[4];
#pragma unroll
          for (int u = 0; u < 4; ++u) e[u] = acol + u < N ? dY[m * lddy + acol + u] : 0.f;
          av[i] = make_float4(e[0], e[1], e[2], e[3]);
        }
        int b, rem, oy, ox;
        cv_divmod((int)m, G.HoWo, G.rHoWo, b, rem);
        cv_divmod(rem, G.Wo, G.rWo, oy, ox);
        xv[i] = cv_load4<VEC4>(G.S, b * G.S.H * G.S.W, oy * G.stride + ctap_y, ox * G.stride + ctap_x, cch);
      } else {
        av[i] = *reinterpret_cast<const float4 *>(dY + m * lddy + acol);
        xv[i] = *reinterpret_cast<const float4 *>(X + m * ldx + xcol);
      }
    }
  };
  const bool want_db = dbpart != nullptr && j0 == 0;
  float4 dbs = make_float4(0.f, 0.f, 0.f, 0.f);
  float sy = 1.f;
  if constexpr (F16) sy = amax_dy ? w_scale(amax_dy[0], false) : 1.f;
  auto lstore = [&](int64_t k0) {
#pragma unroll
    for (int i = 0; i < 4; ++i) {
      const int r = (t >> 5) + 8 * i;
      const bool ok = k0 + r < kend;
      const int off = (tr_off(r, (t & 31) >> 1) + 8 * (t & 1)) >> 2;
      const float4 a = ok ? av[i] : make_float4(0.f, 0.f, 0.f, 0.f);
      float4 x = ok ? xv[i] : make_float4(0.f, 0.f, 0.f, 0.f);
      if constexpr (CONV) x = cv_act4(x, G.S.act);
      if (want_db) { dbs.x += a.x; dbs.y += a.y; dbs.z += a.z; dbs.w += a.w; }
      uint32_t h0, m0, h1, m1;
      if constexpr (F16) {
        split_x(a.x * sy, a.y * sy, h0, m0);
        split_x(a.z * sy, a.w * sy, h1, m1);
      } else {
        split2(a.x, a.y, h0, m0);
        split2(a.z, a.w, h1, m1);
      }
      *reinterpret_cast<uint2 *>(la + off) = make_uint2(h0, h1);
      *reinterpret_cast<uint2 *>(la + TR_XPLANE + off) = make_uint2(m0, m1);
      if constexpr (F16) {
        split_x(x.x, x.y, h0, m0);
        split_x(x.z, x.w, h1, m1);
      } else {
        split2(x.x, x.y, h0, m0);
        split2(x.z, x.w, h1, m1);
      }
      *reinterpret_cast<uint2 *>(lx + off) = make_uint2(h0, h1);
      *reinterpret_cast<uint2 *>(lx + TR_XPLANE + off) = make_uint2(m0, m1);
    }
  };
  const int g = (lane >> 4) & 1, q = (lane & 15) >> 2, p = lane & 3;
  int aoff[2][2][2], boff[2][2][2];
#pragma unroll
  for (int ks = 0; ks < 2; ++ks)
#pragma unroll
    for (int j = 0; j < 2; ++j)
#pragma unroll
      for (int rr = 0; rr < 2; ++rr) {
        const int row = ks * 16 + lh * 8 + rr * 4 + q;
        aoff[ks][j][rr] = tr_off(row, wr * 8 + j * 4 + 2 * g + (p >> 1)) + 8 * (p & 1);
        boff[ks][j][rr] = tr_off(row, wc * 8 + j * 4 + 2 * g + (p >> 1)) + 8 * (p & 1);
      }

  f32x16 acc[2][2];
#pragma unroll
  for (int i = 0; i < 2; ++i)
#pragma unroll
    for (int j = 0; j < 2; ++j)
#pragma unroll
      for (int r = 0; r < 16; ++r) acc[i][j][r] = 0.f;
  const int nrows_valid = CONV ? (int)min<int64_t>(N - i0, (int64_t)TN_TM) - wr * 64 : 64;
  auto mma = [&]() {
    if constexpr (CONV) {
      if (nrows_valid <= 0) return;
    }
#pragma unroll
    for (int ks = 0; ks < 2; ++ks) {
      bf16x8 ah[2], am[2], bh[2], bm[2];
#pragma unroll
      for (int j = 0; j < 2; ++j) {
        ah[j] = tr_frag(la, aoff[ks][j][0], aoff[ks][j][1]);
        am[j] = tr_frag(la + TR_XPLANE, aoff[ks][j][0], aoff[ks][j][1]);
        bh[j] = tr_frag(lx, boff[ks][j][0], boff[ks][j][1]);
        bm[j] = tr_frag(lx + TR_XPLANE, boff[ks][j][0], boff[ks][j][1]);
      }
      if constexpr (F16) {
        f16x8 fah[2], fam[2], fbh[2], fbm[2], fahs[2], fams[2];
#pragma unroll
        for (int j = 0; j < 2; ++j) {
          fah[j] = __builtin_bit_cast(f16x8, ah[j]);
          fam[j] = __builtin_bit_cast(f16x8, am[j]);
          fbh[j] = __builtin_bit_cast(f16x8, bh[j]);
          fbm[j] = __builtin_bit_cast(f16x8, bm[j]);
          fahs[j] = scale_2m11(fah[j]);
          fams[j] = scale_2m11(fam[j]);
        }
#pragma unroll
        for (int i = 0; i < 2; ++i) {
          if constexpr (CONV) {
            if (i * 32 >= nrows_valid) continue;
          }
#pragma unroll
          for (int j = 0; j < 2; ++j) {
            acc[i][j] = __builtin_amdgcn_mfma_f32_32x32x16_f16(fams[i], fbh[j], acc[i][j], 0, 0, 0);
            acc[i][j] = __builtin_amdgcn_mfma_f32_32x32x16_f16(fahs[i], fbm[j], acc[i][j], 0, 0, 0);
            acc[i][j] = __builtin_amdgcn_mfma_f32_32x32x16_f16(fah[i], fbh[j], acc[i][j], 0, 0, 0);
          }
        }
      } else {
#pragma unroll
      for (int i = 0; i < 2; ++i)
#pragma unroll
        for (int j = 0; j < 2; ++j) {
          acc[i][j] = __builtin_amdgcn_mfma_f32_32x32x16_bf16(am[i], bh[j], acc[i][j], 0, 0, 0);
          acc[i][j] = __builtin_amdgcn_mfma_f32_32x32x16_bf16(ah[i], bm[j], acc[i][j], 0, 0, 0);
          acc[i][j] = __builtin_amdgcn_mfma_f32_32x32x16_bf16(ah[i], bh[j], acc[i][j], 0, 0, 0);
        }
      }
    }
  };
  if (kbeg < kend) {
    gload(kbeg);
    lstore(kbeg);
    __syncthreads();
    for (int64_t k0 = kbeg; k0 < kend; k0 += XK) {
      const bool more = k0 + XK < kend;
      if (more) gload(k0 + XK);
      __builtin_amdgcn_sched_barrier(0);
// ... 137 lines not shown
                     epilogue == SVR_EPI_MASK ? mask : nullptr, ldmask, M, N, K, (const uint32_t *)amax, amax_dy, amax_dx);
  return launch_status("linear_bwd_data_f16x3");
}
}

namespace {
int64_t tn_mpad(int64_t M) { return cdiv(M, 64) * 64; }
}

extern "C" int64_t svr_linear_bwd_weight_bf16x3_workspace(int64_t M, int64_t N, int64_t K) {
  int64_t rps;
  int splits = tn_splits_x3(M, N, K, &rps);
  const int64_t dbparts = cdiv(M, 64) > splits ? cdiv(M, 64) : splits;
  return align256((int64_t)splits * N * K * 4) + 2 * align256(N * tn_mpad(M) * 2) + align256(dbparts * N * 4) + 256;
}

extern "C" int svr_linear_bwd_weight_bf16x3(const float *dY, int64_t lddy, const float *X, int64_t ldx, float *dW,
                                            int64_t lddw, float *db, int64_t M, int64_t N, int64_t K, void *workspace,
                                            void *stream) {
  SVR_CHECK(dY && X && dW && workspace, SVR_E_BADARG, "linear_bwd_weight_bf16x3: null pointer");
  LinPlan plan;
  if (int rc = lin_plan(LinQuery{SVR_LIN_BWD_WEIGHT_BF16X3, M, N, K, lddy, ldx, lddw, 0, lo4(dY), lo4(X), lo4(dW), 0, SVR_EPI_NONE, db != nullptr, 1}, plan)) return rc;
  hipStream_t s = (hipStream_t)stream;
  const int64_t rps = plan.rows_per_split;
  const int splits = plan.splits;
  const int64_t Mpad = tn_mpad(M), parts = cdiv(M, 64);
  char *w = align256(workspace);
  float *slab = (float *)w;
  w += align256((int64_t)splits * N * K * 4);
  uint16_t *ph = (uint16_t *)w;
  w += align256(N * Mpad * 2);
  uint16_t *pm = (uint16_t *)w;
  w += align256(N * Mpad * 2);
  float *dbpart = (float *)w;
  dim3 grid(xcd_grid(cdiv(K, TN_TN) * cdiv(N, TN_TM) * splits));
  if (plan.kernel == SVR_LIN_K_TN_TR) {
    hipLaunchKernelGGL(linear_tn_x3_tr_kernel<>, grid, dim3(256), 0, s, dY, lddy, X, ldx, slab, db ? dbpart : nullptr, M, N, K,
                       rps, splits, (const uint32_t *)nullptr, CwGeom{});
    hipLaunchKernelGGL(slab_reduce_x3_kernel, dim3((unsigned)cdiv(N * K, 64)), dim3(256), 0, s, slab, dW, N, K, lddw, splits);
    if (db) col_parts_sum_launch(dbpart, db, N, splits, s);
    return launch_status("linear_bwd_weight_bf16x3");
  }
  hipLaunchKernelGGL(dy_planes_kernel, dim3((unsigned)parts), dim3(256), 0, s, dY, lddy, ph, pm, Mpad, M, N, db ? dbpart : nullptr);
  hipLaunchKernelGGL(linear_tn_x3_kernel, grid, dim3(256), 0, s, ph, pm, Mpad, X, ldx, slab, M, N, K, rps, splits);
  hipLaunchKernelGGL(slab_reduce_x3_kernel, dim3((unsigned)cdiv(N * K, 64)), dim3(256), 0, s, slab, dW, N, K, lddw, splits);
  if (db) col_parts_sum_launch(dbpart, db, N, (int)parts, s);
  return launch_status("linear_bwd_weight_bf16x3");
}

extern "C" int64_t svr_linear_bwd_weight_f16x3_workspace(int64_t M, int64_t N, int64_t K) {
  return svr_linear_bwd_weight_bf16x3_workspace(M, N, K);
}

extern "C" int svr_linear_bwd_weight_f16x3(const float *dY, int64_t lddy, const float *X, int64_t ldx, float *dW, int64_t lddw,
                                           float *db, int64_t M, int64_t N, int64_t K, const uint32_t *amax_dy, void *workspace,
                                           void *stream) {
  SVR_CHECK(dY && X && dW && workspace, SVR_E_BADARG, "linear_bwd_weight_f16x3: null pointer");
  LinPlan plan;
  if (int rc = lin_plan(LinQuery{SVR_LIN_BWD_WEIGHT_F16X3S, M, N, K, lddy, ldx, lddw, 0, lo4(dY), lo4(X), lo4(dW), 0, SVR_EPI_NONE, db != nullptr, 1}, plan)) return rc;
  hipStream_t s = (hipStream_t)stream;
  const int64_t rps = plan.rows_per_split;
  const int splits = plan.splits;
  const int64_t Mpad = tn_mpad(M);
  char *w = align256(workspace);
  float *slab = (float *)w;
  w += align256((int64_t)splits * N * K * 4) + 2 * align256(N * Mpad * 2);
  float *dbpart = (float *)w;
  dim3 grid(xcd_grid(cdiv(K, TN_TN) * cdiv(N, TN_TM) * splits));
  hipLaunchKernelGGL((linear_tn_x3_tr_kernel<true>), grid, dim3(256), 0, s, dY, lddy, X, ldx, slab, db ? dbpart : nullptr, M, N, K,
                     rps, splits, amax_dy, CwGeom{});
  hipLaunchKernelGGL(slab_reduce_x3_kernel, dim3((unsigned)cdiv(N * K, 64)), dim3(256), 0, s, slab, dW, N, K, lddw, splits);
  if (db) col_parts_sum_launch(dbpart, db, N, splits, s);
  return launch_status("linear_bwd_weight_f16x3");
}

namespace {
__global__ __launch_bounds__(256) void conv_wgrad_reduce_kernel(const float *__restrict__ slab, float *__restrict__ dW, int Cout, int C,
                                                                int kk, int Cpad, int splits) {
  __shared__ float red[256];
  const int64_t total = (int64_t)Cout * C * kk, idx = (int64_t)blockIdx.x * 64 + (threadIdx.x & 63);
  const int g = threadIdx.x >> 6;
  float s = 0.f;
  if (idx < total) {
    const int tap = (int)(idx % kk), c = (int)((idx / kk) % C), co = (int)(idx / ((int64_t)kk * C));
    const int64_t K = (int64_t)kk * Cpad, st = (int64_t)Cout * K, at = (int64_t)co * K + (int64_t)tap * Cpad + c;
    for (int z = g; z < splits; z += 4) s += slab[z * st + at];
  }
  red[threadIdx.x] = s;
  __syncthreads();
  if (g == 0 && idx < total) dW[idx] = ((red[threadIdx.x] + red[threadIdx.x + 64]) + red[threadIdx.x + 128]) + red[threadIdx.x + 192];
}
int conv_wgrad_splits(int64_t M, int64_t N, int64_t K, int64_t *rows_per_split) {
  const int64_t tiles = cdiv(N, TN_TM) * cdiv(K, TN_TN);
  const int64_t want = std::max<int64_t>(1, 384 / tiles);
  int64_t rps = cdiv(cdiv(M, want), XK) * XK;
  rps = std::max<int64_t>(rps, 4 * XK);
  *rows_per_split = rps;
  return (int)cdiv(M, rps);
}
}

extern "C" int64_t svr_conv2d_bwd_weight_workspace(const svr_conv2d_desc *d, int32_t Cout) {
  if (!d) return 0;
  const int C = d->C0 + d->C1, Cpad = (C + 15) / 16 * 16;
  const int Ho = (d->H + 2 - d->k) / d->stride + 1, Wo = (d->W + 2 - d->k) / d->stride + 1;
  int64_t rps;
  const int64_t K = (int64_t)d->k * d->k * Cpad;
  const int splits = conv_wgrad_splits((int64_t)d->B * Ho * Wo, Cout, K, &rps);
  return align256((int64_t)splits * Cout * K * 4) + align256((int64_t)splits * Cout * 4) + 256;
}

extern "C" int svr_conv2d_bwd_weight(const svr_conv2d_desc *d, const float *dY, const uint32_t *amax_dy, int32_t Cout, float *dW,
                                     float *db, void *workspace, void *stream) {
  SVR_CHECK(d && d->src0 && dY && dW && workspace && Cout > 0, SVR_E_BADARG, "conv2d_bwd_weight: null pointer");
  SVR_CHECK((d->k == 4 && d->stride == 2) || (d->k == 3 && d->stride == 1), SVR_E_UNSUPPORTED, "conv2d_bwd_weight: k=%d stride=%d", d->k, d->stride);
  SVR_CHECK(!d->upsample, SVR_E_UNSUPPORTED, "conv2d_bwd_weight: the x2 upsample is materialised first (svr_conv2d_virtual)");
  SVR_CHECK(d->C1 == 0 || d->src1, SVR_E_BADARG, "conv2d_bwd_weight: C1 = %d without a second source", d->C1);
  const int C = d->C0 + d->C1, Cpad = (C + 15) / 16 * 16;
  const int Ho = (d->H + 2 - d->k) / d->stride + 1, Wo = (d->W + 2 - d->k) / d->stride + 1;
  const int64_t M = (int64_t)d->B * Ho * Wo, K = (int64_t)d->k * d->k * Cpad, N = Cout;
  SVR_CHECK(M > 0 && M < (1 << 24) && (int64_t)d->B * d->H * d->W < (1 << 24), SVR_E_UNSUPPORTED, "conv2d_bwd_weight: %ld output pixels (row decode limit 2^24)", (long)M);
  hipStream_t s = (hipStream_t)stream;
  int64_t rps;
  const int splits = conv_wgrad_splits(M, N, K, &rps);
  char *w = align256(workspace);
  float *slab = (float *)w;
// ... 17 lines not shown
```

### single-view-3d-reconstruction_amd/model/ifnet.py

```python
import contextlib
import copy
import os

import torch
import torch.nn as nn

from .. import ops
from ..arena import StepArena

_ARCH = {
    128: dict(stages=[(("conv_in",), "conv_in_bn"), (("conv_0", "conv_0_1"), "conv0_1_bn"),
                      (("conv_1", "conv_1_1"), "conv1_1_bn"), (("conv_2", "conv_2_1"), "conv2_1_bn"),
                      (("conv_3", "conv_3_1"), "conv3_1_bn")],
              disp=0.0722, align_corners=False),
    32: dict(stages=[(("conv_1", "conv_1_1"), "conv1_1_bn"), (("conv_2", "conv_2_1"), "conv2_1_bn"),
                     (("conv_3", "conv_3_1"), "conv3_1_bn")],
             disp=0.035, align_corners=True),
}


def _displacements(d):
    rows = [[0.0, 0.0, 0.0]]
    for axis in range(3):
        for sign in (-1, 1):
# ... 70 lines not shown
            launched = True
        for l in range(1, n_levels):
            dhw = _level_dims(D, H, W, l)
            C = layout.channels[l] if layout is not None else 0
            tag = f"L{l}."
            if l in proj_levels:
                if DETERMINISTIC:
                    orders[l] = ops.project_plan(pts, dhw, disp, align)
                    orders[l].record_stream(main)
                else:
                    orders[l] = ops.item_order(pts, dhw, disp, align, arena=arena, tag=tag, x_block=ops.proj_x_block(N, dhw))
                    if arena is None:
                        orders[l].record_stream(main)
                launched = True
            elif form in ("auto", "pull") and fits32 and ops.pull_plan_supported(B, N, dhw, C, layout.row_stride):
                plan = ops.pull_plan(pts, dhw, C, layout.col[l], layout.row_stride, disp, align, arena=arena, tag=tag)
                plan.record_stream(main)
                if form == "pull" or _pull_decision((pts.device.index, l, dhw, C, B, N), plan, side):
                    plans[l] = plan
                else:
                    orders[l] = plan.items
                launched = True
            elif DETERMINISTIC and N > 0:
                raise RuntimeError(f"IF-Net HIP path, DETERMINISTIC: level {l} ({C} channels, {dhw}) has no atomic-free scatter "
                                   "(pull plans cover 16 / 32 / 64 channels, the projection the 128-channel levels of the "
                                   "128-architecture)")
            elif form in ("auto", "pull", "items") and fits32:
                orders[l] = ops.item_order(pts, dhw, disp, align, arena=arena, tag=tag)
                if arena is None:
                    orders[l].record_stream(main)
                launched = True
            elif N >= 0.15 * dhw[0] * dhw[1] * dhw[2] and N > 64:
                orders[l] = ops.voxel_order(pts, dhw, align)
                orders[l].record_stream(main)
                launched = True
        ready = None
        if launched:
            ready = torch.cuda.Event()
            ready.record(side)
    return orders, plans, ready


PROJECT_WIDE_LEVELS = os.environ.get("SVR_NO_PROJECTION") is None
FUSE_FC0 = os.environ.get("SVR_NO_FUSED_FC0") is None
FUSE_FC0_BF16 = os.environ.get("SVR_NO_FUSED_FC0_BF16") is None
OVERLAP_BACKWARD = os.environ.get("SVR_NO_BWD_OVERLAP") is None
STAGE1_RECOMPUTE = os.environ.get("SVR_NO_STAGE1") is None
SORT_ON_SIDE_STREAM = os.environ.get("SVR_SORT_ON_MAIN") is None
PREPARE_WEIGHTS_AHEAD = os.environ.get("SVR_NO_WEIGHT_PREP") is None
FORK_SPLIT_LEVEL = 3
FORK_PIPELINED = os.environ.get("SVR_NO_FORK_PIPELINE") is None
STATS_IN_CONV_EPILOGUE = os.environ.get("SVR_NO_CONV_STATS") is None
USE_ARENA = os.environ.get("SVR_NO_ARENA") is None


def _fc0_fusable(channels, B, dims, n_out):
    if n_out != 256 or sum(1 for c in channels if c == 1) > 1:
        return False
    D, H, W = dims
    for l, c in enumerate(channels):
        if not (c in (1, 16, 32) or c % 64 == 0):
            return False
        d, h, w = _level_dims(D, H, W, l)
        if B * d * h * w * c >= 2 ** 30:
            return False
    return True


def _stage1_applies(si, convs, inp):
    return (STAGE1_RECOMPUTE and si == 0 and len(convs) == 1 and inp.is_cuda and tuple(convs[0].weight.shape[:2]) == (16, 1)
            and min(inp.shape[1:4]) >= 1 and ops.stage1_supported(inp, 16))


class _ProjLink:

    def __init__(self, levels, layout):
        self.levels = tuple(levels)
        self.dh0 = None
        self.need_level0 = False
        cols = sorted((layout.col[l], layout.col[l] + 7 * layout.channels[l]) for l in levels)
        keep, start = [], 0
        for a, b in cols:
            if a > start:
                keep.append((start, a))
            start = b
        if start < layout.row_stride:
            keep.append((start, layout.row_stride))
        raw = [(layout.col[l], layout.col[l] + 7) for l, c in enumerate(layout.channels) if c == 1 and l not in levels]
        split = []
        for a, b in keep:
            cuts = sorted({a, b} | {c for r in raw for c in r if a < c < b})
            split += list(zip(cuts[:-1], cuts[1:]))
        self.keep = split
        self.raw = set(raw)


def _run_stages(ext, inp, training, for_backward):
    levels, saved = [inp], []
    nst = len(ext._stages)
    for si, (convs, bn) in enumerate(ext._stages):
        bn_args = (bn.weight.detach(), bn.bias.detach(), bn.running_mean, bn.running_var, training)
        bn_kw = dict(eps=bn.eps, momentum=bn.momentum, want_pool=(si + 1 < nst))
        if _stage1_applies(si, convs, inp):
            conv = convs[0]
            y, pooled, argmax, ss, mean, wp = ops.stage1_fwd(inp, conv.weight.detach(), conv.bias.detach(), *bn_args, **bn_kw)
            acts = ("stage1", wp)
# ... 50 lines not shown


class _Fork:

    def __init__(self, on, main, device, arena, need_pts, skip, proj, n_levels):
        self.on = on
        self.main = main
        self.keep = _get_side_stream(device) if on else main
        self.w = _get_side_stream(device, 1) if on else main
        self.p = None
        s = FORK_SPLIT_LEVEL
        self.split = s if (on and arena is not None and not need_pts and s not in skip and s not in proj
                           and 0 < s < n_levels) else None
        self.pipelined = FORK_PIPELINED and self.split is not None
        self.dx0_done = self.keep_done = None
        self.level_done = {}

    def stream(self, s):
        return torch.cuda.stream(s) if self.on else contextlib.nullcontext()

    def start(self, *held):
        self.held = held
        if self.on:
            self.keep.wait_stream(self.main)
            self.w.wait_stream(self.main)

    def mark_level(self, l):
        self.level_done[l] = torch.cuda.current_stream().record_event()

    def wait_level(self, l):
        if self.pipelined and l in self.level_done:
            self.main.wait_event(self.level_done[l])

    def join(self):
        self.main.wait_event(self.keep_done)
        self.main.wait_stream(self.w)
        if self.p is not None:
            self.main.wait_stream(self.p)


def _scatter_state(orders, plans, ready, gvols, ext, levels, pts, layout, proj, arena, need_x):
    if orders is None:
        orders, plans, ready = _level_orders_async(pts, *levels[0].shape[1:4], len(levels), ext._align, layout, ext._disp,
                                                   proj_levels=proj, arena=arena, need_level0=need_x)
    if ops.GATHER_FLAGS & ops._lib.GATHER_DETERMINISTIC:
        plans = [None] * len(levels)
        gvols = None
    g0 = (torch.empty_like(levels[0]) if plans[0] is not None else torch.zeros_like(levels[0])) if need_x else None
    if gvols is None:
        gvols = _gvols(arena, levels, plans, proj)
    return orders, plans, ready, [g0] + gvols[1:]


def _fc0_kept_bwd(fork, dh0, feat, w0p, klay, arena):
    cols = klay.full_cols_on(w0p.device)
    w0k = w0p[:, cols]
    dw0_keep = torch.zeros_like(w0p)
    fork.start(w0k)
    with fork.stream(fork.w):
        dwk, db0 = ops.linear_bwd_weight(dh0, feat, want_bias=True)
        dw0_keep[:, cols[:klay.width]] = dwk[:, :klay.width]
        if fork.on:
            db0.record_stream(fork.main)
    with fork.stream(fork.keep):
        gfeat = arena.get("kept_grad", tuple(feat.shape), torch.float32, feat.device) if arena is not None else torch.empty_like(feat)
        ops.linear_bwd_data(dh0, w0k, out=gfeat)
        if fork.on:
            fork.dx0_done = torch.cuda.Event()
            fork.dx0_done.record(fork.keep)
    return dw0_keep, db0, gfeat


def _scatter_kept(fork, ext, levels, gvols, pts, gfeat, layout, orders, plans, ready, skip, proj, need_pts):
    n = len(levels)
    lo = [None if l in proj else o for l, o in enumerate(orders)]

    def scatter(want_gpoints, skip_levels):
        return ops.gather_bwd(levels, gvols, pts, gfeat, layout, ext._disp, ext._align, want_gpoints=want_gpoints,
                              level_orders=lo, level_plans=plans, skip_levels=skip_levels)

    def scatter_level(l):
        scatter(False, tuple(k for k in range(n) if k != l))
        fork.mark_level(l)

    gpts = None
    with fork.stream(fork.keep):
        if ready is not None:
            torch.cuda.current_stream().wait_event(ready)
        if fork.pipelined:
            for l in range(n - 1, -1, -1):
                if l != fork.split and l not in skip and l not in proj and gvols[l] is not None:
                    scatter_level(l)
        else:
            gpts = scatter(need_pts, skip if fork.split is None else tuple(skip) + (fork.split,))
        if fork.on:
            fork.keep_done = torch.cuda.Event()
            fork.keep_done.record(fork.keep)
    if fork.split is not None:
        with torch.cuda.stream(fork.w):
            fork.w.wait_event(fork.dx0_done)
            if ready is not None:
                fork.w.wait_event(ready)
            scatter_level(fork.split)
    return gpts


def _project_wide(fork, ext, levels, gvols, pts, dh0, w0p, orders, ready, proj, dPs, dw0p):
    if fork.on and ready is not None:
        fork.main.wait_event(ready)
    if dw0p is None:
        dw0p = torch.zeros_like(w0p)

    def project_level(l):
        v = levels[l]
        B_, Dl, Hl, Wl, Cl = v.shape
        c0 = ext._layout.col[l]
        dP = ops.gather_project_bwd(pts, dh0, (Dl, Hl, Wl), orders[l], ext._disp, ext._align, out=dPs.get(l))
        dP2 = dP.view(B_ * Dl * Hl * Wl, 7 * 256)
        wl = w0p[:, c0:c0 + 7 * Cl].reshape(256, 7, Cl).permute(1, 0, 2).reshape(7 * 256, Cl).contiguous()
# ... 33 lines not shown
            continue
        dout, grads[bn.weight], grads[bn.bias] = ops.bn_backward(
            acts[-1], gvols[si + 1], dpooled, argmax if dpooled is not None else None, mean, ss, relu_mask=True, training=training)
        for k in range(len(convs) - 1, -1, -1):
            conv = convs[k]
            cin = acts[k - 1] if k > 0 else inp
            grads[conv.weight], grads[conv.bias] = ops.conv3d_k3_bwd_weight(cin, dout, param_layout=True)
            if k > 0:
                dout = ops.conv3d_k3_bwd_data(dout, conv.weight.detach(), mask=acts[k - 1])
            elif si > 0:
                dpooled = ops.conv3d_k3_bwd_data(dout, conv.weight.detach())
            elif need_x:
                gx = ops.conv3d_k3_bwd_data(dout, conv.weight.detach())
    return grads, gx


class _EncoderGatherFn(torch.autograd.Function):

    @staticmethod
    def forward(ctx, ext, grad_mode, link, lease, w0p, b0, x, points, *params):
        B, _, D, H, W = x.shape
        training = ext.training
        x_cl = x.contiguous().view(B, D, H, W, 1)
        pts = points.contiguous()
        nlev = len(ext._stages) + 1
        will_backward = bool(grad_mode) and any(ctx.needs_input_grad)
        ctx.link = link if (will_backward and link is not None) else None
        if ctx.link is not None:
            ctx.link.need_level0 = bool(ctx.needs_input_grad[6])
        proj = ctx.link.levels if ctx.link is not None else ()
        if lease is not None and not (will_backward and x.is_cuda):
            lease.release()
            lease = None
        ctx.lease = lease
        arena = lease.arena if lease is not None else None
        ctx.fused = b0 is not None
        keep = [l for l in range(nlev) if l not in proj] if (ctx.fused and will_backward) else []
        ctx.klay = ext._layout.subset(keep) if keep else None
        ctx.level_orders, ctx.level_plans, ctx.orders_ready = None, None, None
        if will_backward and x.is_cuda:
            ctx.level_orders, ctx.level_plans, ctx.orders_ready = _level_orders_async(
                pts, D, H, W, nlev, ext._align, ctx.klay if ctx.klay is not None else ext._layout, ext._disp,
                proj_levels=proj, arena=arena, need_level0=bool(ctx.needs_input_grad[6]))
        levels, saved = _run_stages(ext, x_cl, training, for_backward=True)
        if training:
            torch._foreach_add_([bn.num_batches_tracked for _, bn in ext._stages], 1)
        ready, ext._points_ready = getattr(ext, "_points_ready", None), None
        if ready is not None:
            torch.cuda.current_stream().wait_event(ready)
        if ctx.fused:
            rows_out = None
            if keep and arena is not None:
                rows_out = arena.get("kept_rows", (B * pts.shape[1], ctx.klay.row_stride), torch.float32, x.device)
            out, feat = ops.gather_fc0_fwd(levels, pts, ext._layout, ext._disp, ext._align, w0p.detach(), b0.detach(), relu=True,
                                           keep_levels=keep, keep_layout=ctx.klay, rows_out=rows_out, arena=arena)
            ctx.feat = feat
        else:
            out = feat = ops.gather_fwd(levels, pts, ext._layout, ext._disp, ext._align)
        ctx.gvols, ctx.dP = None, {}
        if will_backward and x.is_cuda:
            ctx.gvols, ctx.dP, ctx.orders_ready = _zero_fill_async(levels, ctx.level_orders, ctx.level_plans, proj, arena)
        ctx.ext, ctx.saved, ctx.levels, ctx.pts = ext, saved, levels, pts
        ctx.w0p = w0p.detach() if (ctx.link is not None or ctx.fused) else None
        ctx.x_shape, ctx.training = x.shape, training
        return out

    @staticmethod
    def backward(ctx, gfeat):
        if ctx.saved is None:
            raise RuntimeError("IF-Net HIP path: second backward through the same forward pass (the saved pyramid and "
                               "activations are released by the first one; retain_graph is not supported)")
        ext, saved, levels, pts = ctx.ext, ctx.saved, ctx.levels, ctx.pts
        ctx.saved = ctx.levels = ctx.pts = None
        need_x, need_pts = ctx.needs_input_grad[6], ctx.needs_input_grad[7]
        gfeat = gfeat.contiguous()
        link = ctx.link
        proj = link.levels if link is not None else ()
        lease, ctx.lease = ctx.lease, None
        arena = lease.arena if lease is not None else None
        klay = ctx.klay if ctx.fused else None
        scatter_layout = klay if klay is not None else ext._layout
        skip = tuple(l for l in range(len(levels)) if klay.col[l] < 0) if ctx.fused else ()
        dPs, ctx.dP = ctx.dP, None
        gvols, ctx.gvols = ctx.gvols, None
        orders, plans, ready, gvols = _scatter_state(ctx.level_orders, ctx.level_plans, ctx.orders_ready, gvols, ext, levels,
                                                     pts, scatter_layout, proj, arena, need_x)
        main = torch.cuda.current_stream() if gfeat.is_cuda else None
        fork = _Fork(ctx.fused and link is not None and main is not None and OVERLAP_BACKWARD
                     and not torch.cuda.is_current_stream_capturing(),
                     main, gfeat.device, arena, need_pts, skip, proj, len(levels))
        dw0 = db0 = None
        if ctx.fused:
            dh0, feat, ctx.feat = gfeat, ctx.feat, None
            dw0, db0, gfeat = _fc0_kept_bwd(fork, dh0, feat, ctx.w0p, klay, arena)
            if link is not None:
                link.dh0 = dh0
        if link is not None and link.dh0 is None:
            raise RuntimeError("IF-Net HIP path: the projected backward needs dh0 from the point MLP's backward")
        gpts = _scatter_kept(fork, ext, levels, gvols, pts, gfeat, scatter_layout, orders, plans, ready, skip, proj, need_pts)
        if proj:
            dh0, link.dh0 = link.dh0, None
            dw0 = _project_wide(fork, ext, levels, gvols, pts, dh0, ctx.w0p, orders, ready, proj, dPs, dw0)
        if fork.on and not fork.pipelined:
            fork.join()
            feat = None
        grads, gx = _stages_bwd(fork, ext, saved, gvols, ctx.training, need_x)
        if need_x:
            fork.wait_level(0)
            gx = (gx + gvols[0]).view(ctx.x_shape)
        if fork.pipelined:
            fork.join()
        if lease is not None:
            lease.release()
        return (None, None, None, None, dw0, db0, gx, gpts) + tuple(grads.get(p) for p in ext._param_list)


class _PointMLPFn(torch.autograd.Function):

    @staticmethod
    def forward(ctx, feat, row_map, w0p, b0, w1, b1, w2, b2, wo, bo, link=None):
        ctx.headless = w0p is None
        h0 = feat if ctx.headless else ops.linear_fwd(feat, w0p, b0, relu=True)
        h1 = ops.linear_fwd(h0, w1, b1, relu=True)
        h2 = ops.linear_fwd(h1, w2, b2, relu=True)
        logits = ops.fc_out_fwd(h2, wo, bo, row_map)
        ctx.save_for_backward(*(() if ctx.headless else (feat, w0p)), w1, w2, wo, h0, h1, h2)
        ctx.row_map = row_map
        ctx.link = link
        return logits

    @staticmethod
    def backward(ctx, dlogits):
        *head, w1, w2, wo, h0, h1, h2 = ctx.saved_tensors
        dh2, dwo, dbo = ops.fc_out_bwd(h2, wo, dlogits.contiguous(), ctx.row_map)
        dw2, db2 = ops.linear_bwd_weight(dh2, h1)
        dh1 = ops.linear_bwd_data(dh2, w2, mask=h1)
        dw1, db1 = ops.linear_bwd_weight(dh1, h0)
        dh0 = ops.linear_bwd_data(dh1, w1, mask=h0)
        tail = (dw1, db1, dw2, db2, dwo, dbo, None)
        if ctx.headless:
            return (dh0, None, None, None) + tail
        (feat, w0p), link = head, ctx.link
        if link is None:
            dw0, db0 = ops.linear_bwd_weight(dh0, feat)
            dfeat = ops.linear_bwd_data(dh0, w0p) if ctx.needs_input_grad[0] else None
            return (dfeat, None, dw0, db0) + tail
        link.dh0 = dh0
# ... 384 lines not shown
```

### single-view-3d-reconstruction_amd/ops.py

```python
import ctypes as C
import os

import torch

from . import _lib
from .arena import alloc as _alloc
from ._lib import EPI_BIAS, EPI_BIAS_RELU, EPI_MASK, EPI_NONE, GatherDesc, check
from ._lib import ptr as _p, stream as _stream


def _rp(t):
    if t is None:
        return None
    if not t.is_cuda:
        raise RuntimeError("svr_amd ops need GPU tensors (the HIP path has no CPU fallback)")
    return t.data_ptr()


def _f32(*ts):
    for t in ts:
        if t is not None and t.dtype != torch.float32:
            raise RuntimeError(f"expected float32, got {t.dtype}")


# ... 229 lines not shown
            raise RuntimeError(f"level {l} has no columns in this layout (list it in skip_levels)")
        L.vol, L.gvol = _p(v), _p(g)
        L.col = layout.col[l]
        o = level_orders[l] if level_orders is not None else None
        if o is not None and B * N > 0 and o.numel() == 7 * B * N:
            L.item_order, L.order = _p(o), C.c_void_p(0)
        else:
            L.item_order, L.order = C.c_void_p(0), _p(o)
        if level_plans is not None and level_plans[l] is not None:
            L.plan = C.pointer(level_plans[l].c)
    return d


GATHER_FLAGS = 0


def gather_fwd(vols, points, layout, displacement, align_corners, out=None, order=None, flags=0):
    B, N, _ = points.shape
    _f32(points)
    d = make_gather_desc(vols, None, layout, B, N, displacement, align_corners, order, flags=flags | GATHER_FLAGS)
    if out is None:
        out = torch.empty(B * N, layout.row_stride, device=points.device, dtype=torch.float32)
    amax_forget(out)
    check(_lib.lib().svr_gather_trilinear_fwd(C.byref(d), _p(points), _p(out), _stream()), "gather_fwd")
    return out


def gather_fc0_supported(vols, points, layout, displacement, align_corners, n_out=256):
    B, N, _ = points.shape
    if n_out != 256 or not points.is_cuda:
        return False
    d = make_gather_desc(vols, None, layout, B, N, displacement, align_corners)
    return bool(_lib.lib().svr_gather_fc0_supported(C.byref(d)))


class Fc0Prepared:

    def __init__(self, vols, layout, displacement, align_corners, n_out, ws, keep_levels, keep_layout, B=None, N=None):
        self.vols, self.layout, self.displacement, self.align_corners = list(vols), layout, displacement, align_corners
        self.B, self.N = B, N
        self.n_out, self.ws, self.keep_levels, self.keep_layout = n_out, ws, tuple(keep_levels), keep_layout
        self.mask = 0
        for lv in self.keep_levels:
            self.mask |= 1 << lv
        self.kc = None
        self.stride = layout.row_stride
        if self.mask and keep_layout is not None:
            if set(keep_layout.levels) != set(self.keep_levels):
                raise RuntimeError("gather_fc0: keep_layout does not hold exactly keep_levels")
            self.stride = keep_layout.row_stride
            self.kc = (C.c_int32 * len(self.vols))(*[int(c) for c in keep_layout.col])


def gather_fc0_prepare(vols, layout, displacement, align_corners, w, B, N, keep_levels=(), keep_layout=None, arena=None):
    _f32(w)
    d = make_gather_desc(vols, None, layout, B, N, displacement, align_corners)
    l = _lib.lib()
    n_out = w.shape[0]
    assert w.stride(1) == 1 and w.shape[1] >= layout.width
    ws_bytes = l.svr_gather_fc0_workspace(C.byref(d), n_out)
    if ws_bytes <= 0:
        raise RuntimeError("gather_fc0: unsupported level shapes (see svr_gather_fc0_supported)")
    ws = _alloc(arena, "fc0_ws", (ws_bytes,), torch.uint8, w.device)
    prep = Fc0Prepared(vols, layout, displacement, align_corners, n_out, ws, keep_levels, keep_layout, B, N)
    check(l.svr_gather_fc0_prepare(C.byref(d), _rp(w), w.stride(0), n_out, C.c_void_p(256) if prep.mask else None,
                                   prep.stride if prep.mask else 0, prep.kc, prep.mask, _p(ws), _stream()), "gather_fc0_prepare")
    return prep


def gather_fc0_run(prep, points, bias, relu=True, rows_out=None):
    B, N, _ = points.shape
    _f32(points, bias)
    if prep.B is not None and (B != prep.B or N > prep.N):
        raise RuntimeError(f"gather_fc0: points ({B}, {N}, 3) exceed the prepared capacity (B = {prep.B}, N <= {prep.N}): "
                           "prepare again for the larger point set")
    d = make_gather_desc(prep.vols, None, prep.layout, B, N, prep.displacement, prep.align_corners)
    out = torch.empty(B * N, prep.n_out, device=points.device, dtype=torch.float32)
    rows, ldf = None, 0
    if prep.mask:
        if rows_out is not None:
            if tuple(rows_out.shape) != (B * N, prep.stride) or not rows_out.is_contiguous():
                raise RuntimeError(f"gather_fc0: rows_out must be contiguous ({B * N}, {prep.stride})")
            _f32(rows_out)
            amax_forget(rows_out)
            rows = rows_out
        else:
            rows = torch.empty(B * N, prep.stride, device=points.device, dtype=torch.float32)
        ldf = prep.stride
    epi = EPI_NONE if bias is None else (EPI_BIAS_RELU if relu else EPI_BIAS)
    check(_lib.lib().svr_gather_fc0_run(C.byref(d), _p(points), _p(bias), _p(out), out.stride(0), prep.n_out, _p(rows), ldf,
                                        prep.kc, prep.mask, epi, _p(prep.ws), _stream()), "gather_fc0_run")
    return out, rows


def gather_fc0_fwd(vols, points, layout, displacement, align_corners, w, bias, relu=True, keep_levels=(), keep_layout=None,
                   rows_out=None, arena=None):
    B, N, _ = points.shape
    prep = gather_fc0_prepare(vols, layout, displacement, align_corners, w, B, N, keep_levels, keep_layout, arena)
    return gather_fc0_run(prep, points, bias, relu, rows_out)


def gather_bwd(vols, gvols, points, gfeat, layout, displacement, align_corners, want_gpoints=False, order=None,
               level_orders=None, flags=0, level_plans=None, skip_levels=()):
    B, N, _ = points.shape
    if gfeat.numel() != B * N * layout.row_stride:
        raise RuntimeError(f"gather_bwd: gfeat {tuple(gfeat.shape)} does not match the layout's ({B * N}, {layout.row_stride})")
    d = make_gather_desc(vols, gvols, layout, B, N, displacement, align_corners, order, level_orders,
                         flags=flags | GATHER_FLAGS, level_plans=level_plans, skip_levels=skip_levels)
    gp = torch.empty_like(points) if want_gpoints else None
    for g in gvols or ():
        amax_forget(g)
    check(_lib.lib().svr_gather_trilinear_bwd(C.byref(d), _p(points), _p(gfeat), _p(gp), _stream()), "gather_bwd")
    return gp


def corner_indices(vols, points, layout, level, displacement, align_corners):
    B, N, _ = points.shape
    d = make_gather_desc(vols, None, layout, B, N, displacement, align_corners)
    out = torch.empty(B, 7, N, 3, device=points.device, dtype=torch.int32)
    check(_lib.lib().svr_gather_corner_indices(C.byref(d), level, _p(points), _p(out), _stream()), "corner_indices")
    return out


def cast_bf16(t):
    _f32(t)
    out = torch.empty(t.shape, device=t.device, dtype=torch.bfloat16)
    check(_lib.lib().svr_cast_f32_to_bf16(_p(t), _p(out), t.numel(), _stream()), "cast_bf16")
    return out


def _bf16(*ts):
    for t in ts:
        if t is not None and t.dtype != torch.bfloat16:
            raise RuntimeError(f"expected bfloat16, got {t.dtype}")


def gather_fwd_bf16(vols, points, layout, displacement, align_corners, order=None):
    B, N, _ = points.shape
    _f32(points)
    _bf16(*vols)
    d = GatherDesc()
    d.order = _p(order)
    d.n_levels, d.B, d.N, d.row_stride = len(vols), B, N, layout.row_stride
    d.align_corners, d.displacement = int(align_corners), displacement
    for l, v in enumerate(vols):
        if v.dim() != 5 or v.shape[0] != B or v.shape[4] != layout.channels[l]:
            raise RuntimeError(f"level {l}: expected (B,D,H,W,{layout.channels[l]}) channels-last, got {tuple(v.shape)}")
        L = d.level[l]
        L.vol, L.C, L.D, L.H, L.W, L.col = _p(v), v.shape[4], v.shape[1], v.shape[2], v.shape[3], layout.col[l]
    out = torch.empty(B * N, layout.row_stride, device=points.device, dtype=torch.bfloat16)
    check(_lib.lib().svr_gather_trilinear_fwd_bf16(C.byref(d), _p(points), _p(out), _stream()), "gather_fwd_bf16")
# ... 304 lines not shown


def amax_slot(device):
    return _amax_slots.take(device)


def _amax_stamp(t):
    try:
        return (t._version, t.data_ptr())
    except RuntimeError:
        return None


def amax_remember(t, a):
    t._svr_amax = a
    t._svr_amax_stamp = _amax_stamp(t)


def amax_forget(t):
    if t is not None and getattr(t, "_svr_amax", None) is not None:
        t.__dict__.pop("_svr_amax", None)
        t.__dict__.pop("_svr_amax_stamp", None)


def amax_cached(t, force=False):
    a = getattr(t, "_svr_amax", None)
    if a is None or force:
        return None
    stamp = getattr(t, "_svr_amax_stamp", None)
    if stamp is None or stamp != _amax_stamp(t) or not _AmaxSlots.fresh(a):
        return None
    return a


def amax_of(t, force=False):
    a = amax_cached(t, force)
    if a is not None:
        return a
    _f32(t)
    a = amax_slot(t.device)
    if t.dim() == 2 and t.stride(1) == 1 and t.shape[1] % 4 == 0 and t.stride(0) % 4 == 0 and t.data_ptr() % 16 == 0:
        M, N, ld, src = t.shape[0], t.shape[1], t.stride(0), t
    else:
        src = t if t.is_contiguous() else t.contiguous()
        n = src.numel()
        if n % 4 or src.data_ptr() % 16:
            raise RuntimeError("amax_of: tensor must have a multiple of 4 elements and be 16-byte aligned")
        M, N, ld = n // 4, 4, 4
    check(_lib.lib().svr_amax_f32(C.c_void_p(src.data_ptr()), ld, M, N, _p(a), _stream()), "amax_f32")
    amax_remember(t, a)
    return a


def linear_bwd_data(dy, w, mask=None, out=None, mode=None):
    _f32(dy, w, mask)
    M, N = dy.shape
    K = w.shape[1]
    if out is None:
        out = torch.empty(M, K, device=dy.device, dtype=torch.float32)
    epi = EPI_MASK if mask is not None else EPI_NONE
    op = _linear_bwd_data_op(mode, N, operand_layout(dy), operand_layout(out), operand_layout(mask))
    amax_forget(out)
    if op == "bwd_data_f16x3s":
        l = _lib.lib()
        ws = _lookup("lbh", w, mode, "f16x3s") if (w.stride(0) == K and w.stride(1) == 1) else None
        wptr = C.c_void_p(0) if ws is not None else C.c_void_p(w.data_ptr())
        if ws is None:
            assert w.stride(1) == 1
            ws = torch.empty(l.svr_linear_bwd_data_f16x3_workspace(N, K), device=dy.device, dtype=torch.uint8)
        amax_dy = amax_of(dy)
        amax_dx = amax_slot(dy.device)
        check(l.svr_linear_bwd_data_f16x3(C.c_void_p(dy.data_ptr()), dy.stride(0), wptr, w.stride(0),
                                          C.c_void_p(out.data_ptr()), out.stride(0), M, N, K, epi,
                                          _rp(mask), mask.stride(0) if mask is not None else 0, _p(amax_dy), _p(amax_dx), _p(ws), _stream()),
              "linear_bwd_data_f16x3")
        amax_remember(out, amax_dx)
        return out
    if op == "bwd_data_bf16x3":
        l = _lib.lib()
        ws = _lookup("lb", w, mode, "bf16x3") if (w.stride(0) == K and w.stride(1) == 1) else None
        wptr = C.c_void_p(0) if ws is not None else C.c_void_p(w.data_ptr())
        if ws is None:
            ws = torch.empty(l.svr_linear_bwd_data_bf16x3_workspace(N, K), device=dy.device, dtype=torch.uint8)
        check(l.svr_linear_bwd_data_bf16x3(C.c_void_p(dy.data_ptr()), dy.stride(0), wptr, w.stride(0),
                                           C.c_void_p(out.data_ptr()), out.stride(0), M, N, K, epi,
                                           _rp(mask), mask.stride(0) if mask is not None else 0, _p(ws), _stream()),
              "linear_bwd_data_bf16x3")
        return out
    check(_lib.lib().svr_linear_bwd_data(C.c_void_p(dy.data_ptr()), dy.stride(0), C.c_void_p(w.data_ptr()), w.stride(0),
                                         C.c_void_p(out.data_ptr()), out.stride(0), M, N, K, epi,
                                         _rp(mask), mask.stride(0) if mask is not None else 0, _stream()), "linear_bwd_data")
    return out


def linear_bwd_weight(dy, x, want_bias=True, mode=None):
    _f32(dy, x)
    M, N = dy.shape
    K = x.shape[1]
    l = _lib.lib()
    dw = torch.empty(N, K, device=dy.device, dtype=torch.float32)
    db = torch.empty(N, device=dy.device, dtype=torch.float32) if want_bias else None
    op = _linear_bwd_weight_op(mode, M, N, K, operand_layout(dy), operand_layout(x))
    if op == "bwd_weight_f16x3s":
        ws = torch.empty(l.svr_linear_bwd_weight_f16x3_workspace(M, N, K), device=dy.device, dtype=torch.uint8)
        check(l.svr_linear_bwd_weight_f16x3(C.c_void_p(dy.data_ptr()), dy.stride(0), C.c_void_p(x.data_ptr()), x.stride(0),
                                            _p(dw), dw.stride(0), _p(db), M, N, K, _p(amax_of(dy)), _p(ws), _stream()),
              "linear_bwd_weight_f16x3")
        return dw, db
    if op == "bwd_weight_bf16x3":
        ws = torch.empty(l.svr_linear_bwd_weight_bf16x3_workspace(M, N, K), device=dy.device, dtype=torch.uint8)
        check(l.svr_linear_bwd_weight_bf16x3(C.c_void_p(dy.data_ptr()), dy.stride(0), C.c_void_p(x.data_ptr()), x.stride(0),
                                             _p(dw), dw.stride(0), _p(db), M, N, K, _p(ws), _stream()),
              "linear_bwd_weight_bf16x3")
        return dw, db
    ws = torch.empty(l.svr_linear_bwd_weight_workspace(M, N, K), device=dy.device, dtype=torch.uint8)
    check(l.svr_linear_bwd_weight(C.c_void_p(dy.data_ptr()), dy.stride(0), C.c_void_p(x.data_ptr()), x.stride(0),
                                  _p(dw), dw.stride(0), _p(db), M, N, K, _p(ws), _stream()), "linear_bwd_weight")
    return dw, db


def fc_out_fwd(h, w, b, row_map=None):
    _f32(h, w, b)
    M, K = h.shape
    out = torch.empty(M, device=h.device, dtype=torch.float32)
    check(_lib.lib().svr_fc_out_fwd(_p(h), h.stride(0), _p(w), _p(b), _p(out), _p(row_map), M, K, _stream()), "fc_out_fwd")
    return out


def fc_out_bwd(h, w, dlogits, row_map=None):
    _f32(h, w, dlogits)
    M, K = h.shape
    l = _lib.lib()
    ws = torch.empty(l.svr_fc_out_bwd_workspace(M, K), device=h.device, dtype=torch.uint8)
    dh = torch.empty(M, K, device=h.device, dtype=torch.float32)
    dw = torch.empty(K, device=h.device, dtype=torch.float32)
    db = torch.empty(1, device=h.device, dtype=torch.float32)
    amax = amax_slot(h.device) if BACKWARD_GEMM == "f16x3s" else None
    check(l.svr_fc_out_bwd(_p(h), h.stride(0), _p(w), _p(dlogits), _p(row_map), _p(dh), dh.stride(0), _p(dw), _p(db), M, K,
                           _p(amax), _p(ws), _stream()), "fc_out_bwd")
    if amax is not None:
        amax_remember(dh, amax)
    return dh, dw, db


def bce_logits_sum_mean(logits, targets, want_grad=True, gscale=1.0, ordered=False):
    _f32(logits, targets)
    B, N = logits.shape
    loss = torch.empty(1, device=logits.device, dtype=torch.float32)
    dz = torch.empty_like(logits) if want_grad else None
    if ordered:
        l = _lib.lib()
        ws = torch.empty(int(l.svr_bce_ordered_workspace(B)) // 8, device=logits.device, dtype=torch.float64)
        check(l.svr_bce_logits_sum_mean_ordered(_p(logits), _p(targets), _p(loss), _p(dz), B, N, gscale, _p(ws), _stream()),
              "bce_ordered")
        return loss, dz
    ws = torch.empty(B, device=logits.device, dtype=torch.float64)
    check(_lib.lib().svr_bce_logits_sum_mean(_p(logits), _p(targets), _p(loss), _p(dz), B, N, gscale, _p(ws), _stream()),
          "bce")
# ... 739 lines not shown
```

Baseline: 26.34 million.

## Store fc0 kept features pre-split to fp16 hi/lo and add panel dX GEMM

The fused gather+fc0 forward kernel gains a variant that writes kept feature rows already split into fp16 high/low halves. The backward weight GEMM can then read these directly instead of re-splitting fp32 activations. A new panel-style f16x3 bwd-data kernel is added for the narrow fc0 dX GEMM (N<=256). Both are enabled by default through environment flags. The split layout changes the width of C=1 level columns and requires the f16x3s backward mode.

```diff
diff --git a/include/svr_hip.h b/include/svr_hip.h
--- a/include/svr_hip.h
+++ b/include/svr_hip.h
@@ -98,6 +98,9 @@
 int svr_gather_fc0_run(const svr_gather_desc *d, const float *points, const float *bias, float *Y, int64_t ldy, int32_t n_out,
                        float *features, int64_t ldf, const int32_t *keep_cols, uint32_t keep_levels, int32_t epilogue,
                        void *workspace, void *stream);
+int svr_gather_fc0_run_split(const svr_gather_desc *d, const float *points, const float *bias, float *Y, int64_t ldy,
+                             int32_t n_out, void *features, int64_t ldf, const int32_t *keep_cols, uint32_t keep_levels,
+                             int32_t epilogue, void *workspace, void *stream);
 int svr_gather_fc0_bf16_prepare(const svr_gather_desc *d, const float *W, int64_t ldw, int32_t n_out, void *workspace,
                                 void *stream);
 int svr_gather_fc0_bf16_run(const svr_gather_desc *d, const float *points, const float *bias, uint16_t *Y, int64_t ldy,
@@ -154,10 +157,18 @@
                               int64_t lddx, int64_t M, int64_t N, int64_t K, int epilogue,
                               const float *mask, int64_t ldmask, const uint32_t *amax_dy, uint32_t *amax_dx,
                               void *workspace, void *stream);
+int64_t svr_linear_bwd_data_f16x3_panel_workspace(int64_t N, int64_t K);
+int svr_linear_bwd_data_f16x3_panel(const float *dY, int64_t lddy, const float *W, int64_t ldw, float *dX,
+                                    int64_t lddx, int64_t M, int64_t N, int64_t K, int epilogue,
+                                    const float *mask, int64_t ldmask, const uint32_t *amax_dy, uint32_t *amax_dx,
+                                    void *workspace, void *stream);
 int64_t svr_linear_bwd_weight_f16x3_workspace(int64_t M, int64_t N, int64_t K);
 int svr_linear_bwd_weight_f16x3(const float *dY, int64_t lddy, const float *X, int64_t ldx, float *dW,
                                 int64_t lddw, float *db, int64_t M, int64_t N, int64_t K,
                                 const uint32_t *amax_dy, void *workspace, void *stream);
+int svr_linear_bwd_weight_f16x3_xsplit(const float *dY, int64_t lddy, const void *Xsplit, int64_t ldx, float *dW,
+                                       int64_t lddw, float *db, int64_t M, int64_t N, int64_t K,
+                                       const uint32_t *amax_dy, void *workspace, void *stream);
 
 #define SVR_LIN_FWD_F32 0
 #define SVR_LIN_FWD_F16X3 1
diff --git a/single-view-3d-reconstruction_amd/_lib.py b/single-view-3d-reconstruction_amd/_lib.py
--- a/single-view-3d-reconstruction_amd/_lib.py
+++ b/single-view-3d-reconstruction_amd/_lib.py
@@ -61,6 +61,7 @@
     "svr_gather_fc0_fwd": (C.c_int, [C.POINTER(GatherDesc), P, P, I64, P, P, I64, I32, P, I64, P, C.c_uint32, I32, P, P]),
     "svr_gather_fc0_prepare": (C.c_int, [C.POINTER(GatherDesc), P, I64, I32, P, I64, P, C.c_uint32, P, P]),
     "svr_gather_fc0_run": (C.c_int, [C.POINTER(GatherDesc), P, P, P, I64, I32, P, I64, P, C.c_uint32, I32, P, P]),
+    "svr_gather_fc0_run_split": (C.c_int, [C.POINTER(GatherDesc), P, P, P, I64, I32, P, I64, P, C.c_uint32, I32, P, P]),
     "svr_gather_fc0_bf16_prepare": (C.c_int, [C.POINTER(GatherDesc), P, I64, I32, P, P]),
     "svr_gather_fc0_bf16_run": (C.c_int, [C.POINTER(GatherDesc), P, P, P, I64, I32, I32, P, P]),
     "svr_gather_trilinear_bwd": (C.c_int, [C.POINTER(GatherDesc), P, P, P, P]),
@@ -84,8 +85,11 @@
     "svr_amax_f32": (C.c_int, [P, I64, I64, I64, P, P]),
     "svr_linear_bwd_data_f16x3_workspace": (I64, [I64, I64]),
     "svr_linear_bwd_data_f16x3": (C.c_int, [P, I64, P, I64, P, I64, I64, I64, I64, C.c_int, P, I64, P, P, P, P]),
+    "svr_linear_bwd_data_f16x3_panel": (C.c_int, [P, I64, P, I64, P, I64, I64, I64, I64, C.c_int, P, I64, P, P, P, P]),
+    "svr_linear_bwd_data_f16x3_panel_workspace": (I64, [I64, I64]),
     "svr_linear_bwd_weight_f16x3_workspace": (I64, [I64, I64, I64]),
     "svr_linear_bwd_weight_f16x3": (C.c_int, [P, I64, P, I64, P, I64, P, I64, I64, I64, P, P, P]),
+    "svr_linear_bwd_weight_f16x3_xsplit": (C.c_int, [P, I64, P, I64, P, I64, P, I64, I64, I64, P, P, P]),
     "svr_linear_variant": (C.c_int, [I32, I64, I64, I64, I64, I64, I64, I64, I32, I32, I32, I32, I32, I32, P, P, P, P, P, P]),
     "svr_fc_out_fwd": (C.c_int, [P, I64, P, P, P, P, I64, I64, P]),
     "svr_fc_out_bwd_workspace": (I64, [I64, I64]),
diff --git a/single-view-3d-reconstruction_amd/build.py b/single-view-3d-reconstruction_amd/build.py
--- a/single-view-3d-reconstruction_amd/build.py
+++ b/single-view-3d-reconstruction_amd/build.py
@@ -17,6 +17,7 @@
     "gemm_bf16x3.hip": [],
     "gemm_bf16x6.hip": [],
     "gemm_f16x3.hip": [],
+    "gemm_f16x3_panel.hip": [],
     "conv3d.hip": [],
     "conv3d_bf16.hip": [],
     "conv3d_bwdw_bf16.hip": [],
diff --git a/single-view-3d-reconstruction_amd/csrc/f16x3.h b/single-view-3d-reconstruction_amd/csrc/f16x3.h
--- a/single-view-3d-reconstruction_amd/csrc/f16x3.h
+++ b/single-view-3d-reconstruction_amd/csrc/f16x3.h
@@ -79,6 +79,9 @@
   f.q = *reinterpret_cast<const uint4 *>(p);
   return f.v;
 }
+__host__ __device__ __forceinline__ int64_t wfrag_index(int kk, int plane, int n, int ntiles, int nplanes = 2) {
+  return ((((int64_t)(kk >> 4) * nplanes + plane) * ntiles + (n >> 5)) * 64 + ((kk >> 3) & 1) * 32 + (n & 31)) * 8 + (kk & 7);
+}
 __device__ __forceinline__ bf16x8 frag_bf16(const uint32_t *p) {
   union { uint4 q; bf16x8 v; } f;
   f.q = *reinterpret_cast<const uint4 *>(p);
diff --git a/single-view-3d-reconstruction_amd/csrc/gather_fc0.hip b/single-view-3d-reconstruction_amd/csrc/gather_fc0.hip
--- a/single-view-3d-reconstruction_amd/csrc/gather_fc0.hip
+++ b/single-view-3d-reconstruction_amd/csrc/gather_fc0.hip
@@ -62,10 +62,6 @@
   return -1;
 }
 
-__device__ __forceinline__ int64_t wfrag_index(int kk, int plane, int n, int ntiles, int nplanes = 2) {
-  return ((((int64_t)(kk >> 4) * nplanes + plane) * ntiles + (n >> 5)) * 64 + ((kk >> 3) & 1) * 32 + (n & 31)) * 8 + (kk & 7);
-}
-
 __global__ void split_w_fused_kernel(FcArgs A, const float *__restrict__ W, int64_t ldw, const uint32_t *__restrict__ amax,
                                      uint16_t *__restrict__ p0, int N) {
   const int kk = blockIdx.x * blockDim.x + threadIdx.x, n = blockIdx.y;
@@ -138,7 +134,7 @@
   }
 }
 
-template <int LP, int NJ, bool BF, bool STAGED = false>
+template <int LP, int NJ, bool BF, bool STAGED = false, bool KS = false>
 __device__ __forceinline__ void produce_slab(const FcLevel L, const FcSlab S, uint32_t *__restrict__ buf, int64_t m0, int64_t M,
                                              float *__restrict__ feat, int row_stride, int pw, int lane, const Geo &G,
                                              const uint32_t *stage = nullptr) {
@@ -212,7 +208,13 @@
     *reinterpret_cast<uint2 *>(d) = make_uint2(h0, h1);
     *reinterpret_cast<uint2 *>(d + FPLANE) = make_uint2(l0, l1);
     if (S.keep && RPW * pw + it * PPW + g < live) {
-      __builtin_nontemporal_store(acc, reinterpret_cast<GLOBAL_AS f32x4 *>(featt + (fo0 + (uint32_t)(it * PPW * row_stride * 4))));
+      if constexpr (KS) {
+        typedef uint32_t u32x4_t __attribute__((ext_vector_type(4)));
+        __builtin_nontemporal_store(u32x4_t{h0, h1, l0, l1},
+                                    reinterpret_cast<GLOBAL_AS u32x4_t *>(featt + (fo0 + (uint32_t)(it * PPW * row_stride * 4))));
+      } else {
+        __builtin_nontemporal_store(acc, reinterpret_cast<GLOBAL_AS f32x4 *>(featt + (fo0 + (uint32_t)(it * PPW * row_stride * 4))));
+      }
     }
   };
   constexpr int DEPTH = 1;
@@ -226,7 +228,7 @@
   }
 }
 
-template <bool BF>
+template <bool BF, bool KS = false>
 __device__ __forceinline__ void produce_c1(const FcLevel L, const FcSlab S, uint32_t *__restrict__ buf,
                                            const float *__restrict__ points, int64_t m0, int64_t M, int N, float disp, int ac,
                                            float *__restrict__ feat, int row_stride, int tp) {
@@ -267,10 +269,25 @@
     if (j < 7) {
       b16[s0 * 2 + j] = hb;
       if (!BF) b16[(FPLANE + s0) * 2 + j] = __builtin_bit_cast(uint16_t, l);
-      if (!BF && S.keep && m0 + row < M) feat[(m0 + row) * row_stride + L.kcol + j] = acc;
+      if (!BF && S.keep && m0 + row < M) {
+        if constexpr (KS) {
+          uint16_t *g16 = reinterpret_cast<uint16_t *>(feat + (m0 + row) * row_stride + L.kcol) + (j >> 2) * 8 + (j & 3);
+          g16[0] = hb;
+          g16[4] = __builtin_bit_cast(uint16_t, l);
+        } else {
+          feat[(m0 + row) * row_stride + L.kcol + j] = acc;
+        }
+      }
     } else {
       uint32_t z = 0u;
       asm volatile("" : "+v"(z));
+      if constexpr (KS && !BF) {
+        if (S.keep && m0 + row < M) {
+          uint16_t *g16 = reinterpret_cast<uint16_t *>(feat + (m0 + row) * row_stride + L.kcol) + 8 + 3;
+          g16[0] = (uint16_t)z;
+          g16[4] = (uint16_t)z;
+        }
+      }
       b16[s0 * 2 + 7] = (uint16_t)z;
       if (!BF) b16[(FPLANE + s0) * 2 + 7] = (uint16_t)z;
 #pragma unroll
@@ -305,7 +322,7 @@
   }
 }
 
-template <bool BF>
+template <bool BF, bool KS>
 __device__ __forceinline__ void produce(const FcArgs &A, int s, uint32_t *buf, const float *points, int64_t m0, int64_t M,
                                         int N, float disp, int ac, float *feat, int row_stride, int pw, int lane,
                                         uint32_t *stage, const FcBox *__restrict__ boxes, Geo &G, int rowb) {
@@ -320,22 +337,22 @@
       }
       if (box.nvox > 0) {
         if (S.geo) level_geometry<BF, true>(L, points + m0 * 3, rowb, disp, ac, lane, box, G);
-        produce_slab<16, 1, BF, true>(L, S, buf, m0, M, feat, row_stride, pw, lane, G, stage);
+        produce_slab<16, 1, BF, true, KS>(L, S, buf, m0, M, feat, row_stride, pw, lane, G, stage);
         return;
       }
     }
   }
   if (S.lp == 0) {
-    produce_c1<BF>(L, S, buf, points, m0, M, N, disp, ac, feat, row_stride, pw * 64 + lane);
+    produce_c1<BF, KS>(L, S, buf, points, m0, M, N, disp, ac, feat, row_stride, pw * 64 + lane);
     return;
   }
   if (S.geo) level_geometry<BF, false>(L, points + m0 * 3, rowb, disp, ac, lane, FcBox{}, G);
   switch (S.lp * 4 + S.nj) {
-    case 16 * 4 + 1: produce_slab<16, 1, BF>(L, S, buf, m0, M, feat, row_stride, pw, lane, G); break;
-    case 16 * 4 + 2: produce_slab<16, 2, BF>(L, S, buf, m0, M, feat, row_stride, pw, lane, G); break;
-    case 8 * 4 + 1: produce_slab<8, 1, BF>(L, S, buf, m0, M, feat, row_stride, pw, lane, G); break;
-    case 8 * 4 + 2: produce_slab<8, 2, BF>(L, S, buf, m0, M, feat, row_stride, pw, lane, G); break;
-    case 4 * 4 + 1: produce_slab<4, 1, BF>(L, S, buf, m0, M, feat, row_stride, pw, lane, G); break;
+    case 16 * 4 + 1: produce_slab<16, 1, BF, false, KS>(L, S, buf, m0, M, feat, row_stride, pw, lane, G); break;
+    case 16 * 4 + 2: produce_slab<16, 2, BF, false, KS>(L, S, buf, m0, M, feat, row_stride, pw, lane, G); break;
+    case 8 * 4 + 1: produce_slab<8, 1, BF, false, KS>(L, S, buf, m0, M, feat, row_stride, pw, lane, G); break;
+    case 8 * 4 + 2: produce_slab<8, 2, BF, false, KS>(L, S, buf, m0, M, feat, row_stride, pw, lane, G); break;
+    case 4 * 4 + 1: produce_slab<4, 1, BF, false, KS>(L, S, buf, m0, M, feat, row_stride, pw, lane, G); break;
   }
 }
 
@@ -348,7 +365,7 @@
   for (unsigned i = threadIdx.x; i < sizeof(FcArgs) / 4; i += blockDim.x) reinterpret_cast<uint32_t *>(dst)[i] = src[i];
 }
 
-template <bool BF>
+template <bool BF, bool KS = false>
 __global__ __launch_bounds__(NTHR, 4) void gather_fc0_kernel(const FcArgs *__restrict__ Ap, const float *__restrict__ points,
                                                             const uint16_t *__restrict__ W0,
                                                             const uint32_t *__restrict__ amax, const float *__restrict__ bias,
@@ -378,7 +395,7 @@
       int rowb_s = rowb;
       asm volatile("" : "+v"(lane_s), "+v"(rowb_s));
       if (s + 1 < S)
-        produce<BF>(A, s + 1, lds + ((s + 1) & 1) * FSLAB, points, m0, M, N, disp, ac, feat, row_stride, pw, lane_s, lds + 2 * FSLAB,
+        produce<BF, KS>(A, s + 1, lds + ((s + 1) & 1) * FSLAB, points, m0, M, N, disp, ac, feat, row_stride, pw, lane_s, lds + 2 * FSLAB,
                     boxes + tile * FC_NSTAGE, G, rowb_s);
       slab_barrier();
     }
@@ -645,19 +662,21 @@
   return w;
 }
 
-int check_keep(const svr_gather_desc *d, const FcArgs &A, const float *feat, int64_t ldf, uint32_t keep_levels, int64_t *kend) {
+int check_keep(const svr_gather_desc *d, const FcArgs &A, const float *feat, int64_t ldf, uint32_t keep_levels, int64_t *kend,
+               bool split = false) {
   const int64_t M = (int64_t)d->B * d->N;
   SVR_CHECK(keep_levels == 0 || (feat && ldf % 4 == 0 && ((uintptr_t)feat & 15) == 0 && M * ldf < (1LL << 31)),
             SVR_E_BADARG, "gather_fc0: keep_levels needs a 16-byte aligned feature matrix with < 2^31 elements");
   *kend = 0;
   for (int l = 0; l < d->n_levels; ++l) {
     if (!((keep_levels >> l) & 1)) continue;
-    const int kc = A.L[l].kcol, w = 7 * d->level[l].C;
-    SVR_CHECK(kc >= 0 && kc + w <= ldf && (d->level[l].C == 1 || kc % 4 == 0), SVR_E_BADSHAPE,
+    auto width = [&](int lv) { return (split && d->level[lv].C == 1) ? 8 : 7 * d->level[lv].C; };
+    const int kc = A.L[l].kcol, w = width(l);
+    SVR_CHECK(kc >= 0 && kc + w <= ldf && ((d->level[l].C == 1 && !split) || kc % 4 == 0), SVR_E_BADSHAPE,
               "gather_fc0: kept level %d: columns [%d,%d) in a row of %ld", l, kc, kc + w, (long)ldf);
     for (int m = 0; m < l; ++m)
       if ((keep_levels >> m) & 1)
-        SVR_CHECK(kc + w <= A.L[m].kcol || A.L[m].kcol + 7 * d->level[m].C <= kc, SVR_E_BADSHAPE,
+        SVR_CHECK(kc + w <= A.L[m].kcol || A.L[m].kcol + width(m) <= kc, SVR_E_BADSHAPE,
                   "gather_fc0: kept levels %d and %d overlap", m, l);
     *kend = std::max<int64_t>(*kend, kc + w);
   }
@@ -691,9 +710,10 @@
   return launch_status("gather_fc0_prepare");
 }
 
-extern "C" int svr_gather_fc0_run(const svr_gather_desc *d, const float *points, const float *bias, float *Y, int64_t ldy,
-                                  int32_t n_out, float *feat, int64_t ldf, const int32_t *keep_cols, uint32_t keep_levels,
-                                  int32_t epilogue, void *workspace, void *stream) {
+namespace {
+template <bool KS>
+int fc0_run(const svr_gather_desc *d, const float *points, const float *bias, float *Y, int64_t ldy, int32_t n_out, float *feat,
+            int64_t ldf, const int32_t *keep_cols, uint32_t keep_levels, int32_t epilogue, void *workspace, void *stream) {
   int rc = check_desc(d, "gather_fc0_run");
   if (rc != SVR_OK) return rc;
   const int64_t M = (int64_t)d->B * d->N;
@@ -706,14 +726,15 @@
   FcArgs A;
   SVR_CHECK(build_slabs(d, keep_levels, A, keep_cols, true), SVR_E_UNSUPPORTED,
             "gather_fc0_run: a level's channel count has no slab shape (1, 16, 32, 64 k)");
+  SVR_CHECK(!KS || keep_levels == 0 || keep_cols, SVR_E_UNSUPPORTED, "gather_fc0_run_split: split rows need the compact kept matrix (keep_cols)");
   int64_t kend;
-  if ((rc = check_keep(d, A, feat, ldf, keep_levels, &kend)) != SVR_OK) return rc;
+  if ((rc = check_keep(d, A, feat, ldf, keep_levels, &kend, KS)) != SVR_OK) return rc;
   int64_t kw = 0;
   for (int l = 0; l < d->n_levels; ++l) kw = std::max<int64_t>(kw, d->level[l].col + 7 * d->level[l].C);
   const int64_t pad_start = keep_cols ? kend : kw;
   const FcWorkspace ws = carve(workspace, n_out, A.KF);
   static const hipError_t lds_attr =
-      hipFuncSetAttribute((const void *)gather_fc0_kernel<false>, hipFuncAttributeMaxDynamicSharedMemorySize, FC_LDS_BYTES);
+      hipFuncSetAttribute((const void *)gather_fc0_kernel<false, KS>, hipFuncAttributeMaxDynamicSharedMemorySize, FC_LDS_BYTES);
   SVR_CHECK(lds_attr == hipSuccess, (int)lds_attr, "gather_fc0_run: cannot reserve %d bytes of LDS: %s", FC_LDS_BYTES,
             hipGetErrorString(lds_attr));
   const float *eb = epilogue == SVR_EPI_NONE ? nullptr : bias;
@@ -721,10 +742,23 @@
   if (A.n_stage > 0)
     hipLaunchKernelGGL(fc0_boxes_kernel, dim3((unsigned)cdiv(M, FTM)), dim3(64), 0, (hipStream_t)stream, ws.Ad, points, M, d->N,
                        d->displacement, d->align_corners, ws.boxes);
-  hipLaunchKernelGGL(gather_fc0_kernel<false>, dim3((unsigned)cdiv(M, FTM)), dim3(NTHR), FC_LDS_BYTES, (hipStream_t)stream, ws.Ad, points,
+  hipLaunchKernelGGL((gather_fc0_kernel<false, KS>), dim3((unsigned)cdiv(M, FTM)), dim3(NTHR), FC_LDS_BYTES, (hipStream_t)stream, ws.Ad, points,
                      ws.p0, ws.amax, eb, Y, ldy, feat, (int)ldf, keep_levels ? (int)pad_start : -1, M, d->N, d->displacement,
                      d->align_corners, relu, ws.boxes);
   return launch_status("gather_fc0_run");
+}
+}
+
+extern "C" int svr_gather_fc0_run(const svr_gather_desc *d, const float *points, const float *bias, float *Y, int64_t ldy,
+                                  int32_t n_out, float *feat, int64_t ldf, const int32_t *keep_cols, uint32_t keep_levels,
+                                  int32_t epilogue, void *workspace, void *stream) {
+  return fc0_run<false>(d, points, bias, Y, ldy, n_out, feat, ldf, keep_cols, keep_levels, epilogue, workspace, stream);
+}
+
+extern "C" int svr_gather_fc0_run_split(const svr_gather_desc *d, const float *points, const float *bias, float *Y, int64_t ldy,
+                                        int32_t n_out, void *feat, int64_t ldf, const int32_t *keep_cols, uint32_t keep_levels,
+                                        int32_t epilogue, void *workspace, void *stream) {
+  return fc0_run<true>(d, points, bias, Y, ldy, n_out, (float *)feat, ldf, keep_cols, keep_levels, epilogue, workspace, stream);
 }
 
 extern "C" int svr_gather_fc0_fwd(const svr_gather_desc *d, const float *points, const float *W, int64_t ldw, const float *bias,
diff --git a/single-view-3d-reconstruction_amd/csrc/gemm_bf16x3.hip b/single-view-3d-reconstruction_amd/csrc/gemm_bf16x3.hip
--- a/single-view-3d-reconstruction_amd/csrc/gemm_bf16x3.hip
+++ b/single-view-3d-reconstruction_amd/csrc/gemm_bf16x3.hip
@@ -3,6 +3,7 @@
 #include "gemm_core.h"
 #include "conv2d_virt.h"
 #include "f16x3.h"
+#include <type_traits>
 
 using namespace svr;
 
@@ -50,13 +51,15 @@
   }
 };
 
-template <int ROWS, int NT>
+template <int ROWS, int NT, bool RAG = false>
 struct PlaneLoader {
   static constexpr int R = ROWS * 4 / NT;
   const uint16_t *ph[R], *pm[R];
   uint2 vh[R][2], vm[R][2];
+  int live = ROWS;
   __device__ __forceinline__ PlaneLoader(const uint16_t *hi, const uint16_t *mid, int64_t ld, int64_t row0, int64_t nrows) {
     const int t = threadIdx.x;
+    if constexpr (RAG) live = (int)min<int64_t>(ROWS, (nrows - row0 + 31) / 32 * 32);
 #pragma unroll
     for (int i = 0; i < R; ++i) {
       int64_t r = row0 + (t >> 2) + (NT / 4) * i;
@@ -68,6 +71,7 @@
   __device__ __forceinline__ void load(int64_t k0, int64_t) {
 #pragma unroll
     for (int i = 0; i < R; ++i) {
+      if (RAG && (threadIdx.x >> 2) + (NT / 4) * i >= live) continue;
       const uint2 *qh = reinterpret_cast<const uint2 *>(ph[i] + k0);
       const uint2 *qm = reinterpret_cast<const uint2 *>(pm[i] + k0);
       vh[i][0] = qh[0]; vh[i][1] = qh[1];
@@ -78,6 +82,7 @@
     const int t = threadIdx.x;
 #pragma unroll
     for (int i = 0; i < R; ++i) {
+      if (RAG && (t >> 2) + (NT / 4) * i >= live) continue;
       const int off = ((t >> 2) + (NT / 4) * i) * XLW + (t & 3) * 4;
       *reinterpret_cast<uint2 *>(planes + off) = vh[i][0];
       *reinterpret_cast<uint2 *>(planes + off + 2) = vh[i][1];
@@ -139,13 +144,48 @@
   static constexpr int LDS_DWORDS = STAGE;
 };
 
-template <int WR, int WC, bool F16 = false>
-__device__ __forceinline__ void compute_step(const uint32_t *pa, f32x16 (&acc)[2][2]) {
+template <int WR, int WC, bool F16 = false, bool RAG = false>
+__device__ __forceinline__ void compute_step(const uint32_t *pa, f32x16 (&acc)[2][2], int ncv = WC * 64) {
   using G = Geo<WR, WC>;
   const int lane = threadIdx.x & 63, wave = threadIdx.x >> 6;
   const int wr = wave / WC, wc = wave % WC;
   const int l31 = lane & 31, lh = lane >> 5;
   const uint32_t *pb = pa + 2 * G::TM * XLW;
+  if constexpr (RAG) {
+    const int nv = __builtin_amdgcn_readfirstlane(ncv - wc * 64);
+    if (nv <= 0) return;
+#pragma unroll
+    for (int ks = 0; ks < 2; ++ks) {
+      bf16x8 ah[2], am[2];
+      const int kw = ks * 8 + lh * 4;
+#pragma unroll
+      for (int i = 0; i < 2; ++i) {
+        const int row = wr * 64 + i * 32 + l31;
+        ah[i] = read_frag(pa, row, kw);
+        am[i] = read_frag(pa + G::TM * XLW, row, kw);
+      }
+#pragma unroll
+      for (int j = 0; j < 2; ++j) {
+        if (j == 1 && nv <= 32) continue;
+        const int row = wc * 64 + j * 32 + l31;
+        const bf16x8 bh = read_frag(pb, row, kw), bm = read_frag(pb + G::TN * XLW, row, kw);
+#pragma unroll
+        for (int i = 0; i < 2; ++i) {
+          if constexpr (F16) {
+            const f16x8 fbh = __builtin_bit_cast(f16x8, bh);
+            acc[i][j] = __builtin_amdgcn_mfma_f32_32x32x16_f16(__builtin_bit_cast(f16x8, am[i]), scale_2m11(fbh), acc[i][j], 0, 0, 0);
+            acc[i][j] = __builtin_amdgcn_mfma_f32_32x32x16_f16(__builtin_bit_cast(f16x8, ah[i]), __builtin_bit_cast(f16x8, bm), acc[i][j], 0, 0, 0);
+            acc[i][j] = __builtin_amdgcn_mfma_f32_32x32x16_f16(__builtin_bit_cast(f16x8, ah[i]), fbh, acc[i][j], 0, 0, 0);
+          } else {
+            acc[i][j] = __builtin_amdgcn_mfma_f32_32x32x16_bf16(am[i], bh, acc[i][j], 0, 0, 0);
+            acc[i][j] = __builtin_amdgcn_mfma_f32_32x32x16_bf16(ah[i], bm, acc[i][j], 0, 0, 0);
+            acc[i][j] = __builtin_amdgcn_mfma_f32_32x32x16_bf16(ah[i], bh, acc[i][j], 0, 0, 0);
+          }
+        }
+      }
+    }
+    return;
+  }
 #pragma unroll
   for (int ks = 0; ks < 2; ++ks) {
     bf16x8 ah[2], am[2], bh[2], bm[2];
@@ -193,8 +233,9 @@
   }
 }
 
-template <int WR, int WC, class AL, class BL, bool F16 = false>
-__device__ __forceinline__ void mainloop(AL &al, BL &bl, uint32_t *lds, int64_t kbeg, int64_t kend, f32x16 (&acc)[2][2]) {
+template <int WR, int WC, class AL, class BL, bool F16 = false, bool RAG = false>
+__device__ __forceinline__ void mainloop(AL &al, BL &bl, uint32_t *lds, int64_t kbeg, int64_t kend, f32x16 (&acc)[2][2],
+                                         int ncv = WC * 64) {
   using G = Geo<WR, WC>;
 #pragma unroll
   for (int i = 0; i < 2; ++i)
@@ -215,7 +256,7 @@
       bl.load(k0 + XK, kend);
     }
     __builtin_amdgcn_sched_barrier(0);
-    compute_step<WR, WC, F16>(lds, acc);
+    compute_step<WR, WC, F16, RAG>(lds, acc, ncv);
     __syncthreads();
     if (more) {
       al.store(lds);
@@ -265,14 +306,15 @@
   if (lidx >= nct * cdiv(M, NN_TM)) return;
   const int64_t c0 = (lidx % nct) * NN_TN, m0 = (lidx / nct) * NN_TM;
   RowKLoader<NN_TM, 256, F16> al(dY, lddy, m0, M);
-  PlaneLoader<NN_TN, 256> bl(Wh, Wm, N, c0, K);
   float inv = 1.f, vmax = 0.f;
   if constexpr (F16) {
     al.sy = amax_dy ? w_scale(amax_dy[0], false) : 1.f;
     inv = w_scale(amax_w[0], true) * (amax_dy ? w_scale(amax_dy[0], true) : 1.f);
   }
   f32x16 acc[2][2];
-  mainloop<2, 2, RowKLoader<NN_TM, 256, F16>, PlaneLoader<NN_TN, 256>, F16>(al, bl, lds, 0, N, acc);
+  PlaneLoader<NN_TN, 256, true> bl(Wh, Wm, N, c0, K);
+  mainloop<2, 2, RowKLoader<NN_TM, 256, F16>, PlaneLoader<NN_TN, 256, true>, F16, true>(al, bl, lds, 0, N, acc,
+                                                                                       (int)min<int64_t>(K - c0, (int64_t)NN_TN));
   float *ct = reinterpret_cast<float *>(lds);
   const int t = threadIdx.x;
   const int wave = t >> 6;
@@ -376,12 +418,13 @@
   float rWo, rHoWo;
   int k, stride, pad, Cpad;
 };
-template <bool F16 = false, bool CONV = false, bool VEC4 = true>
+template <bool F16 = false, bool CONV = false, bool VEC4 = true, bool XSPLIT = false>
 __global__ __launch_bounds__(256, 2) void linear_tn_x3_tr_kernel(const float *__restrict__ dY, int64_t lddy,
                                                               const float *__restrict__ X, int64_t ldx,
                                                               float *__restrict__ slab, float *__restrict__ dbpart,
                                                               int64_t M, int64_t N, int64_t K, int64_t rows_per_split,
                                                               int splits, const uint32_t *__restrict__ amax_dy, const CwGeom G) {
+  static_assert(!XSPLIT || (F16 && !CONV), "pre-split X: the f16 split of a matrix in memory");
   __shared__ __attribute__((aligned(16))) uint32_t lds[4 * TR_XPLANE];
   uint32_t *la = lds, *lx = lds + 2 * TR_XPLANE;
   const int t = threadIdx.x, lane = t & 63, wave = t >> 6;
@@ -402,6 +445,8 @@
     ctap_y = tap / G.k - G.pad;
     ctap_x = tap % G.k - G.pad;
   }
+  const int xlive = (int)min<int64_t>(TN_TN, (K - j0 + 31) / 32 * 32);
+  const bool xon = 4 * (t & 31) < xlive;
   auto gload = [&](int64_t k0) {
 #pragma unroll
     for (int i = 0; i < 4; ++i) {
@@ -421,7 +466,7 @@
         xv[i] = cv_load4<VEC4>(G.S, b * G.S.H * G.S.W, oy * G.stride + ctap_y, ox * G.stride + ctap_x, cch);
       } else {
         av[i] = *reinterpret_cast<const float4 *>(dY + m * lddy + acol);
-        xv[i] = *reinterpret_cast<const float4 *>(X + m * ldx + xcol);
+        if (xon) xv[i] = *reinterpret_cast<const float4 *>(X + m * ldx + xcol);
       }
     }
   };
@@ -449,7 +494,11 @@
       }
       *reinterpret_cast<uint2 *>(la + off) = make_uint2(h0, h1);
       *reinterpret_cast<uint2 *>(la + TR_XPLANE + off) = make_uint2(m0, m1);
-      if constexpr (F16) {
+      if (!CONV && !xon) continue;
+      if constexpr (XSPLIT) {
+        h0 = __float_as_uint(x.x); h1 = __float_as_uint(x.y);
+        m0 = __float_as_uint(x.z); m1 = __float_as_uint(x.w);
+      } else if constexpr (F16) {
         split_x(x.x, x.y, h0, m0);
         split_x(x.z, x.w, h1, m1);
       } else {
@@ -481,10 +530,49 @@
 #pragma unroll
       for (int r = 0; r < 16; ++r) acc[i][j][r] = 0.f;
   const int nrows_valid = CONV ? (int)min<int64_t>(N - i0, (int64_t)TN_TM) - wr * 64 : 64;
+  const int ncols_valid = __builtin_amdgcn_readfirstlane((int)min<int64_t>(K - j0, (int64_t)TN_TN) - wc * 64);
   auto mma = [&]() {
-    if constexpr (CONV) {
-      if (nrows_valid <= 0) return;
-    }
+    if constexpr (!CONV) {
+      if (ncols_valid <= 0) return;
+#pragma unroll
+      for (int ks = 0; ks < 2; ++ks) {
+        bf16x8 ah[2], am[2];
+#pragma unroll
+        for (int i = 0; i < 2; ++i) {
+          ah[i] = tr_frag(la, aoff[ks][i][0], aoff[ks][i][1]);
+          am[i] = tr_frag(la + TR_XPLANE, aoff[ks][i][0], aoff[ks][i][1]);
+        }
+        f16x8 fah[2], fahs[2], fams[2];
+        if constexpr (F16) {
+#pragma unroll
+          for (int i = 0; i < 2; ++i) {
+            fah[i] = __builtin_bit_cast(f16x8, ah[i]);
+            fahs[i] = scale_2m11(fah[i]);
+            fams[i] = scale_2m11(__builtin_bit_cast(f16x8, am[i]));
+          }
+        }
+#pragma unroll
+        for (int j = 0; j < 2; ++j) {
+          if (j == 1 && ncols_valid <= 32) continue;
+          const bf16x8 bh = tr_frag(lx, boff[ks][j][0], boff[ks][j][1]), bm = tr_frag(lx + TR_XPLANE, boff[ks][j][0], boff[ks][j][1]);
+#pragma unroll
+          for (int i = 0; i < 2; ++i) {
+            if constexpr (F16) {
+              const f16x8 fbh = __builtin_bit_cast(f16x8, bh), fbm = __builtin_bit_cast(f16x8, bm);
+              acc[i][j] = __builtin_amdgcn_mfma_f32_32x32x16_f16(fams[i], fbh, acc[i][j], 0, 0, 0);
+              acc[i][j] = __builtin_amdgcn_mfma_f32_32x32x16_f16(fahs[i], fbm, acc[i][j], 0, 0, 0);
+              acc[i][j] = __builtin_amdgcn_mfma_f32_32x32x16_f16(fah[i], fbh, acc[i][j], 0, 0, 0);
+            } else {
+              acc[i][j] = __builtin_amdgcn_mfma_f32_32x32x16_bf16(am[i], bh, acc[i][j], 0, 0, 0);
+              acc[i][j] = __builtin_amdgcn_mfma_f32_32x32x16_bf16(ah[i], bm, acc[i][j], 0, 0, 0);
+              acc[i][j] = __builtin_amdgcn_mfma_f32_32x32x16_bf16(ah[i], bh, acc[i][j], 0, 0, 0);
+            }
+          }
+        }
+      }
+      return;
+    }
+    if (nrows_valid <= 0) return;
 #pragma unroll
     for (int ks = 0; ks < 2; ++ks) {
       bf16x8 ah[2], am[2], bh[2], bm[2];
@@ -728,9 +816,10 @@
   return svr_linear_bwd_weight_bf16x3_workspace(M, N, K);
 }
 
-extern "C" int svr_linear_bwd_weight_f16x3(const float *dY, int64_t lddy, const float *X, int64_t ldx, float *dW, int64_t lddw,
-                                           float *db, int64_t M, int64_t N, int64_t K, const uint32_t *amax_dy, void *workspace,
-                                           void *stream) {
+namespace {
+template <bool XSPLIT>
+int bwd_weight_f16x3(const float *dY, int64_t lddy, const float *X, int64_t ldx, float *dW, int64_t lddw, float *db, int64_t M,
+                     int64_t N, int64_t K, const uint32_t *amax_dy, void *workspace, void *stream) {
   SVR_CHECK(dY && X && dW && workspace, SVR_E_BADARG, "linear_bwd_weight_f16x3: null pointer");
   LinPlan plan;
   if (int rc = lin_plan(LinQuery{SVR_LIN_BWD_WEIGHT_F16X3S, M, N, K, lddy, ldx, lddw, 0, lo4(dY), lo4(X), lo4(dW), 0, SVR_EPI_NONE, db != nullptr, 1}, plan)) return rc;
@@ -743,11 +832,24 @@
   w += align256((int64_t)splits * N * K * 4) + 2 * align256(N * Mpad * 2);
   float *dbpart = (float *)w;
   dim3 grid(xcd_grid(cdiv(K, TN_TN) * cdiv(N, TN_TM) * splits));
-  hipLaunchKernelGGL((linear_tn_x3_tr_kernel<true>), grid, dim3(256), 0, s, dY, lddy, X, ldx, slab, db ? dbpart : nullptr, M, N, K,
-                     rps, splits, amax_dy, CwGeom{});
+  hipLaunchKernelGGL((linear_tn_x3_tr_kernel<true, false, true, XSPLIT>), grid, dim3(256), 0, s, dY, lddy, X, ldx, slab,
+                     db ? dbpart : nullptr, M, N, K, rps, splits, amax_dy, CwGeom{});
   hipLaunchKernelGGL(slab_reduce_x3_kernel, dim3((unsigned)cdiv(N * K, 64)), dim3(256), 0, s, slab, dW, N, K, lddw, splits);
   if (db) col_parts_sum_launch(dbpart, db, N, splits, s);
   return launch_status("linear_bwd_weight_f16x3");
+}
+}
+
+extern "C" int svr_linear_bwd_weight_f16x3(const float *dY, int64_t lddy, const float *X, int64_t ldx, float *dW, int64_t lddw,
+                                           float *db, int64_t M, int64_t N, int64_t K, const uint32_t *amax_dy, void *workspace,
+                                           void *stream) {
+  return bwd_weight_f16x3<false>(dY, lddy, X, ldx, dW, lddw, db, M, N, K, amax_dy, workspace, stream);
+}
+
+extern "C" int svr_linear_bwd_weight_f16x3_xsplit(const float *dY, int64_t lddy, const void *Xsplit, int64_t ldx, float *dW,
+                                                  int64_t lddw, float *db, int64_t M, int64_t N, int64_t K, const uint32_t *amax_dy,
+                                                  void *workspace, void *stream) {
+  return bwd_weight_f16x3<true>(dY, lddy, (const float *)Xsplit, ldx, dW, lddw, db, M, N, K, amax_dy, workspace, stream);
 }
 
 namespace {
diff --git a/single-view-3d-reconstruction_amd/csrc/gemm_f16x3_panel.hip b/single-view-3d-reconstruction_amd/csrc/gemm_f16x3_panel.hip
--- /dev/null
+++ b/single-view-3d-reconstruction_amd/csrc/gemm_f16x3_panel.hip
@@ -0,0 +1,186 @@
+#include "common.h"
+#include "f16x3.h"
+
+using namespace svr;
+
+namespace {
+
+constexpr int PR = 64;
+constexpr int PLW = 8;
+constexpr int PPLANE = PR * PLW;
+constexpr int PKSTEP = 2 * PPLANE + 8;
+constexpr int PSTG_LD = 68;
+constexpr int PSTG = 8 * PSTG_LD;
+constexpr int PN_MAX = 256;
+
+int panel_lds_bytes(int64_t N) { return (int)((N / 16) * PKSTEP + 4 * PSTG) * 4; }
+
+__global__ void pack_wfrag_f16_kernel(const float *__restrict__ W, int64_t ldw, const uint32_t *__restrict__ amax,
+                                      uint16_t *__restrict__ p, int N, int K, int KT) {
+  const int k = blockIdx.x * blockDim.x + threadIdx.x, n = blockIdx.y;
+  if (k >= KT * 32 || n >= N) return;
+  const float w = k < K ? W[(int64_t)n * ldw + k] * w_scale(amax[0], false) : 0.f;
+  _Float16 h, l;
+  split_w(w, h, l);
+  p[wfrag_index(n, 0, k, KT)] = __builtin_bit_cast(uint16_t, h);
+  p[wfrag_index(n, 1, k, KT)] = __builtin_bit_cast(uint16_t, l);
+}
+
+__device__ __forceinline__ void lds_wave_sync() {
+  asm volatile("s_waitcnt lgkmcnt(0)" ::: "memory");
+}
+
+__global__ __launch_bounds__(256, 2) void linear_nn_x3_panel_kernel(const float *__restrict__ dY, int64_t lddy,
+                                                                   const uint16_t *__restrict__ Wf, float *__restrict__ dX,
+                                                                   int64_t lddx, int64_t M, int N, int K, int KT,
+                                                                   const uint32_t *__restrict__ amax_w,
+                                                                   const uint32_t *__restrict__ amax_dy,
+                                                                   uint32_t *__restrict__ amax_dx) {
+  extern __shared__ __attribute__((aligned(16))) uint32_t lds[];
+  const int t = threadIdx.x, lane = t & 63, wave = __builtin_amdgcn_readfirstlane(t >> 6);
+  const int l31 = lane & 31, lh = lane >> 5;
+  const int64_t m0 = (int64_t)blockIdx.x * PR;
+  const int nk = N / 16;
+  const float sy = amax_dy ? w_scale(amax_dy[0], false) : 1.f;
+  const float inv = w_scale(amax_w[0], true) * (amax_dy ? w_scale(amax_dy[0], true) : 1.f);
+  {
+    const int q = N / 4, total = PR * q;
+    for (int u0 = 0; u0 < total; u0 += 8 * 256) {
+      float4 v[8];
+#pragma unroll
+      for (int i = 0; i < 8; ++i) {
+        const int u = min(u0 + 256 * i + t, total - 1), row = u / q, c4 = u - row * q;
+        const int64_t m = min(m0 + row, M - 1);
+        v[i] = *reinterpret_cast<const float4 *>(dY + m * lddy + 4 * c4);
+      }
+#pragma unroll
+      for (int i = 0; i < 8; ++i) {
+        const int u = u0 + 256 * i + t;
+        if (u >= total) continue;
+        const int row = u / q, col = 4 * (u - row * q);
+        uint32_t h0, l0, h1, l1;
+        split_x(v[i].x * sy, v[i].y * sy, h0, l0);
+        split_x(v[i].z * sy, v[i].w * sy, h1, l1);
+        uint32_t *d = lds + (col >> 4) * PKSTEP + row * PLW + (((col & 15) >> 1) ^ (((row >> 3) & 1) * 4));
+        *reinterpret_cast<uint2 *>(d) = make_uint2(h0, h1);
+        *reinterpret_cast<uint2 *>(d + PPLANE) = make_uint2(l0, l1);
+      }
+    }
+  }
+  __syncthreads();
+  float *stg = reinterpret_cast<float *>(lds + nk * PKSTEP) + wave * PSTG;
+  float vmax = 0.f;
+  const int npairs = (KT + 1) / 2;
+  for (int p = wave; p < npairs; p += 4) {
+    const bool has1 = 2 * p + 1 < KT;
+    const uint16_t *wp = Wf + ((int64_t)(2 * p) * 64 + lane) * 8;
+    const int t1 = has1 ? 512 : 0;
+    uint4 b0[2][2], b1[2][2];
+    auto loadb = [&](uint4 (&r)[2][2], int kc) {
+      const uint16_t *qp = wp + (int64_t)(kc < nk ? kc : nk - 1) * (2 * KT * 512);
+      r[0][0] = *reinterpret_cast<const uint4 *>(qp);
+      r[0][1] = *reinterpret_cast<const uint4 *>(qp + KT * 512);
+      r[1][0] = *reinterpret_cast<const uint4 *>(qp + t1);
+      r[1][1] = *reinterpret_cast<const uint4 *>(qp + KT * 512 + t1);
+    };
+    f32x16 acc[2][2];
+#pragma unroll
+    for (int i = 0; i < 2; ++i)
+#pragma unroll
+      for (int j = 0; j < 2; ++j)
+#pragma unroll
+        for (int r = 0; r < 16; ++r) acc[i][j][r] = 0.f;
+    auto step = [&](const uint4 (&cur)[2][2], uint4 (&fre)[2][2], int kc) {
+      loadb(fre, kc + 1);
+      const uint32_t *pa = lds + kc * PKSTEP;
+      f16x8 b[3][2];
+#pragma unroll
+      for (int jt = 0; jt < 2; ++jt) {
+        union { uint4 q; f16x8 v; } u0, u1;
+        u0.q = cur[jt][0];
+        u1.q = cur[jt][1];
+        b[0][jt] = u0.v;
+        b[1][jt] = u1.v;
+        b[2][jt] = scale_2m11(u0.v);
+      }
+#pragma unroll
+      for (int jt = 0; jt < 2; ++jt) {
+        if (jt == 1 && !has1) continue;
+#pragma unroll
+        for (int i = 0; i < 2; ++i) {
+          const f16x8 ah = frag_f16(pa + slot_dw(i * 32 + l31, lh)), al = frag_f16(pa + PPLANE + slot_dw(i * 32 + l31, lh));
+          acc[i][jt] = __builtin_amdgcn_mfma_f32_32x32x16_f16(al, b[2][jt], acc[i][jt], 0, 0, 0);
+          acc[i][jt] = __builtin_amdgcn_mfma_f32_32x32x16_f16(ah, b[1][jt], acc[i][jt], 0, 0, 0);
+          acc[i][jt] = __builtin_amdgcn_mfma_f32_32x32x16_f16(ah, b[0][jt], acc[i][jt], 0, 0, 0);
+        }
+      }
+    };
+    loadb(b0, 0);
+    for (int kc = 0; kc < nk; kc += 2) {
+      step(b0, b1, kc);
+      step(b1, b0, kc + 1);
+    }
+#pragma unroll
+    for (int i = 0; i < 2; ++i)
+#pragma unroll
+      for (int g = 0; g < 4; ++g) {
+#pragma unroll
+        for (int jt = 0; jt < 2; ++jt)
+#pragma unroll
+          for (int rr = 0; rr < 4; ++rr) stg[(4 * lh + rr) * PSTG_LD + jt * 32 + l31] = acc[i][jt][4 * g + rr];
+        lds_wave_sync();
+#pragma unroll
+        for (int u = 0; u < 2; ++u) {
+          const int row = (lane >> 4) + 4 * u, c4 = (lane & 15) * 4;
+          float4 v = *reinterpret_cast<const float4 *>(stg + row * PSTG_LD + c4);
+          const int64_t m = m0 + i * 32 + 8 * g + row;
+          const int c = p * 64 + c4;
+          if (m < M && c < K) {
+            v.x *= inv; v.y *= inv; v.z *= inv; v.w *= inv;
+            vmax = fmaxf(fmaxf(vmax, fmaxf(fabsf(v.x), fabsf(v.y))), fmaxf(fabsf(v.z), fabsf(v.w)));
+            typedef float nt4 __attribute__((ext_vector_type(4)));
+            __builtin_nontemporal_store(nt4{v.x, v.y, v.z, v.w}, reinterpret_cast<nt4 *>(dX + m * lddx + c));
+          }
+        }
+        lds_wave_sync();
+      }
+  }
+  if (amax_dx) svr_amax_publish(amax_dx, vmax);
+}
+
+}
+
+extern "C" int64_t svr_linear_bwd_data_f16x3_panel_workspace(int64_t N, int64_t K) {
+  return 2 * N * cdiv(K, 32) * 32 * (int64_t)sizeof(uint16_t) + 512;
+}
+
+extern "C" int svr_linear_bwd_data_f16x3_panel(const float *dY, int64_t lddy, const float *W, int64_t ldw, float *dX, int64_t lddx,
+                                               int64_t M, int64_t N, int64_t K, int epilogue, const float *mask, int64_t ldmask,
+                                               const uint32_t *amax_dy, uint32_t *amax_dx, void *workspace, void *stream) {
+  (void)ldmask;
+  SVR_CHECK(dY && W && dX && workspace, SVR_E_BADARG, "linear_bwd_data_f16x3_panel: null pointer");
+  SVR_CHECK(epilogue == SVR_EPI_NONE && !mask, SVR_E_UNSUPPORTED, "linear_bwd_data_f16x3_panel: no mask epilogue (epilogue %d)", epilogue);
+  SVR_CHECK(M >= 0 && N > 0 && K > 0 && N % 32 == 0 && K % 4 == 0, SVR_E_BADSHAPE,
+            "linear_bwd_data_f16x3_panel: M=%ld N=%ld K=%ld (need N %% 32 == 0, K %% 4 == 0)", (long)M, (long)N, (long)K);
+  SVR_CHECK(N <= PN_MAX, SVR_E_UNSUPPORTED, "linear_bwd_data_f16x3_panel: N=%ld (the resident panel holds at most %d columns)", (long)N, PN_MAX);
+  SVR_CHECK(K <= (1 << 20) && M < (1LL << 31) * PR, SVR_E_UNSUPPORTED, "linear_bwd_data_f16x3_panel: M=%ld K=%ld", (long)M, (long)K);
+  SVR_CHECK(lddy % 4 == 0 && ((uintptr_t)dY & 15) == 0, SVR_E_ALIGN, "linear_bwd_data_f16x3_panel: dY must be 16-byte aligned");
+  SVR_CHECK(lddx % 4 == 0 && ((uintptr_t)dX & 15) == 0, SVR_E_ALIGN,
+            "linear_bwd_data_f16x3_panel: dX must be 16-byte aligned with a leading dimension that is a multiple of 4");
+  if (M == 0) return SVR_OK;
+  hipStream_t s = (hipStream_t)stream;
+  const int KT = (int)cdiv(K, 32);
+  uint32_t *amax = align256<uint32_t>(workspace);
+  uint16_t *planes = (uint16_t *)(amax + 64);
+  w_amax_launch(W, ldw, N, K, amax, s);
+  hipLaunchKernelGGL(pack_wfrag_f16_kernel, dim3((unsigned)cdiv(KT * 32, 64), (unsigned)N), dim3(64), 0, s, W, ldw, amax, planes, (int)N,
+                     (int)K, KT);
+  const int lds_bytes = panel_lds_bytes(N);
+  static const hipError_t lds_attr =
+      hipFuncSetAttribute((const void *)linear_nn_x3_panel_kernel, hipFuncAttributeMaxDynamicSharedMemorySize, panel_lds_bytes(PN_MAX));
+  SVR_CHECK(lds_attr == hipSuccess, (int)lds_attr, "linear_bwd_data_f16x3_panel: cannot reserve %d bytes of LDS: %s",
+            panel_lds_bytes(PN_MAX), hipGetErrorString(lds_attr));
+  hipLaunchKernelGGL(linear_nn_x3_panel_kernel, dim3((unsigned)cdiv(M, PR)), dim3(256), lds_bytes, s, dY, lddy, planes, dX, lddx, M,
+                     (int)N, (int)K, KT, (const uint32_t *)amax, amax_dy, amax_dx);
+  return launch_status("linear_bwd_data_f16x3_panel");
+}
diff --git a/single-view-3d-reconstruction_amd/model/ifnet.py b/single-view-3d-reconstruction_amd/model/ifnet.py
--- a/single-view-3d-reconstruction_amd/model/ifnet.py
+++ b/single-view-3d-reconstruction_amd/model/ifnet.py
@@ -146,6 +146,8 @@
 FORK_PIPELINED = os.environ.get("SVR_NO_FORK_PIPELINE") is None
 STATS_IN_CONV_EPILOGUE = os.environ.get("SVR_NO_CONV_STATS") is None
 USE_ARENA = os.environ.get("SVR_NO_ARENA") is None
+FC0_ROWS_SPLIT = os.environ.get("SVR_NO_FC0_ROWS_SPLIT") is None
+FC0_DX_PANEL = os.environ.get("SVR_NO_FC0_DX_PANEL") is None
 
 
 def _fc0_fusable(channels, B, dims, n_out):
@@ -302,19 +304,19 @@
     return orders, plans, ready, [g0] + gvols[1:]
 
 
-def _fc0_kept_bwd(fork, dh0, feat, w0p, klay, arena):
+def _fc0_kept_bwd(fork, dh0, feat, w0p, klay, arena, feat_split=False):
     cols = klay.full_cols_on(w0p.device)
     w0k = w0p[:, cols]
     dw0_keep = torch.zeros_like(w0p)
     fork.start(w0k)
     with fork.stream(fork.w):
-        dwk, db0 = ops.linear_bwd_weight(dh0, feat, want_bias=True)
+        dwk, db0 = ops.linear_bwd_weight(dh0, feat, want_bias=True, mode="f16x3s" if feat_split else None, x_split=feat_split)
         dw0_keep[:, cols[:klay.width]] = dwk[:, :klay.width]
         if fork.on:
             db0.record_stream(fork.main)
     with fork.stream(fork.keep):
         gfeat = arena.get("kept_grad", tuple(feat.shape), torch.float32, feat.device) if arena is not None else torch.empty_like(feat)
-        ops.linear_bwd_data(dh0, w0k, out=gfeat)
+        ops.linear_bwd_data(dh0, w0k, out=gfeat, panel=FC0_DX_PANEL)
         if fork.on:
             fork.dx0_done = torch.cuda.Event()
             fork.dx0_done.record(fork.keep)
@@ -454,8 +456,10 @@
             rows_out = None
             if keep and arena is not None:
                 rows_out = arena.get("kept_rows", (B * pts.shape[1], ctx.klay.row_stride), torch.float32, x.device)
+            ctx.feat_split = bool(keep) and FC0_ROWS_SPLIT and ops.BACKWARD_GEMM == "f16x3s" and B * pts.shape[1] > 0
             out, feat = ops.gather_fc0_fwd(levels, pts, ext._layout, ext._disp, ext._align, w0p.detach(), b0.detach(), relu=True,
-                                           keep_levels=keep, keep_layout=ctx.klay, rows_out=rows_out, arena=arena)
+                                           keep_levels=keep, keep_layout=ctx.klay, rows_out=rows_out, arena=arena,
+                                           rows_split=ctx.feat_split)
             ctx.feat = feat
         else:
             out = feat = ops.gather_fwd(levels, pts, ext._layout, ext._disp, ext._align)
@@ -494,7 +498,7 @@
         dw0 = db0 = None
         if ctx.fused:
             dh0, feat, ctx.feat = gfeat, ctx.feat, None
-            dw0, db0, gfeat = _fc0_kept_bwd(fork, dh0, feat, ctx.w0p, klay, arena)
+            dw0, db0, gfeat = _fc0_kept_bwd(fork, dh0, feat, ctx.w0p, klay, arena, ctx.feat_split)
             if link is not None:
                 link.dh0 = dh0
         if link is not None and link.dh0 is None:
diff --git a/single-view-3d-reconstruction_amd/ops.py b/single-view-3d-reconstruction_amd/ops.py
--- a/single-view-3d-reconstruction_amd/ops.py
+++ b/single-view-3d-reconstruction_amd/ops.py
@@ -305,7 +305,8 @@
             self.kc = (C.c_int32 * len(self.vols))(*[int(c) for c in keep_layout.col])
 
 
-def gather_fc0_prepare(vols, layout, displacement, align_corners, w, B, N, keep_levels=(), keep_layout=None, arena=None):
+def gather_fc0_prepare(vols, layout, displacement, align_corners, w, B, N, keep_levels=(), keep_layout=None, arena=None,
+                       rows_split=False):
     _f32(w)
     d = make_gather_desc(vols, None, layout, B, N, displacement, align_corners)
     l = _lib.lib()
@@ -316,12 +317,15 @@
         raise RuntimeError("gather_fc0: unsupported level shapes (see svr_gather_fc0_supported)")
     ws = _alloc(arena, "fc0_ws", (ws_bytes,), torch.uint8, w.device)
     prep = Fc0Prepared(vols, layout, displacement, align_corners, n_out, ws, keep_levels, keep_layout, B, N)
+    prep.rows_split = bool(rows_split)
     check(l.svr_gather_fc0_prepare(C.byref(d), _rp(w), w.stride(0), n_out, C.c_void_p(256) if prep.mask else None,
                                    prep.stride if prep.mask else 0, prep.kc, prep.mask, _p(ws), _stream()), "gather_fc0_prepare")
     return prep
 
 
-def gather_fc0_run(prep, points, bias, relu=True, rows_out=None):
+def gather_fc0_run(prep, points, bias, relu=True, rows_out=None, rows_split=None):
+    if rows_split is None:
+        rows_split = getattr(prep, "rows_split", False)
     B, N, _ = points.shape
     _f32(points, bias)
     if prep.B is not None and (B != prep.B or N > prep.N):
@@ -341,15 +345,16 @@
             rows = torch.empty(B * N, prep.stride, device=points.device, dtype=torch.float32)
         ldf = prep.stride
     epi = EPI_NONE if bias is None else (EPI_BIAS_RELU if relu else EPI_BIAS)
-    check(_lib.lib().svr_gather_fc0_run(C.byref(d), _p(points), _p(bias), _p(out), out.stride(0), prep.n_out, _p(rows), ldf,
-                                        prep.kc, prep.mask, epi, _p(prep.ws), _stream()), "gather_fc0_run")
+    run = _lib.lib().svr_gather_fc0_run_split if rows_split else _lib.lib().svr_gather_fc0_run
+    check(run(C.byref(d), _p(points), _p(bias), _p(out), out.stride(0), prep.n_out, _p(rows), ldf,
+              prep.kc, prep.mask, epi, _p(prep.ws), _stream()), "gather_fc0_run")
     return out, rows
 
 
 def gather_fc0_fwd(vols, points, layout, displacement, align_corners, w, bias, relu=True, keep_levels=(), keep_layout=None,
-                   rows_out=None, arena=None):
+                   rows_out=None, arena=None, rows_split=False):
     B, N, _ = points.shape
-    prep = gather_fc0_prepare(vols, layout, displacement, align_corners, w, B, N, keep_levels, keep_layout, arena)
+    prep = gather_fc0_prepare(vols, layout, displacement, align_corners, w, B, N, keep_levels, keep_layout, arena, rows_split)
     return gather_fc0_run(prep, points, bias, relu, rows_out)
 
 
@@ -760,7 +765,7 @@
     return a
 
 
-def linear_bwd_data(dy, w, mask=None, out=None, mode=None):
+def linear_bwd_data(dy, w, mask=None, out=None, mode=None, panel=False):
     _f32(dy, w, mask)
     M, N = dy.shape
     K = w.shape[1]
@@ -769,6 +774,16 @@
     epi = EPI_MASK if mask is not None else EPI_NONE
     op = _linear_bwd_data_op(mode, N, operand_layout(dy), operand_layout(out), operand_layout(mask))
     amax_forget(out)
+    if panel and op == "bwd_data_f16x3s" and mask is None and N <= 256 and N % 32 == 0 and K % 4 == 0 and w.stride(1) == 1:
+        l = _lib.lib()
+        ws = torch.empty(l.svr_linear_bwd_data_f16x3_panel_workspace(N, K), device=dy.device, dtype=torch.uint8)
+        amax_dy = amax_of(dy)
+        amax_dx = amax_slot(dy.device)
+        check(l.svr_linear_bwd_data_f16x3_panel(C.c_void_p(dy.data_ptr()), dy.stride(0), C.c_void_p(w.data_ptr()), w.stride(0),
+                                                C.c_void_p(out.data_ptr()), out.stride(0), M, N, K, EPI_NONE, None, 0,
+                                                _p(amax_dy), _p(amax_dx), _p(ws), _stream()), "linear_bwd_data_f16x3_panel")
+        amax_remember(out, amax_dx)
+        return out
     if op == "bwd_data_f16x3s":
         l = _lib.lib()
         ws = _lookup("lbh", w, mode, "f16x3s") if (w.stride(0) == K and w.stride(1) == 1) else None
@@ -801,7 +816,7 @@
     return out
 
 
-def linear_bwd_weight(dy, x, want_bias=True, mode=None):
+def linear_bwd_weight(dy, x, want_bias=True, mode=None, x_split=False):
     _f32(dy, x)
     M, N = dy.shape
     K = x.shape[1]
@@ -809,9 +824,12 @@
     dw = torch.empty(N, K, device=dy.device, dtype=torch.float32)
     db = torch.empty(N, device=dy.device, dtype=torch.float32) if want_bias else None
     op = _linear_bwd_weight_op(mode, M, N, K, operand_layout(dy), operand_layout(x))
+    if x_split and op != "bwd_weight_f16x3s":
+        raise RuntimeError(f"linear_bwd_weight: x_split needs the f16x3s product, this call would run {op}")
     if op == "bwd_weight_f16x3s":
         ws = torch.empty(l.svr_linear_bwd_weight_f16x3_workspace(M, N, K), device=dy.device, dtype=torch.uint8)
-        check(l.svr_linear_bwd_weight_f16x3(C.c_void_p(dy.data_ptr()), dy.stride(0), C.c_void_p(x.data_ptr()), x.stride(0),
+        fn = l.svr_linear_bwd_weight_f16x3_xsplit if x_split else l.svr_linear_bwd_weight_f16x3
+        check(fn(C.c_void_p(dy.data_ptr()), dy.stride(0), C.c_void_p(x.data_ptr()), x.stride(0),
                                             _p(dw), dw.stride(0), _p(db), M, N, K, _p(amax_of(dy)), _p(ws), _stream()),
               "linear_bwd_weight_f16x3")
         return dw, db
```

New measurement: 26.45 million (median of 6 runs). No clear change (+0.4%).
